# torognes/vsearch

Measured on AMD Instinct MI355X. Metric: GCUPS (useful DP cells/s of the search16 global-alignment path: DP + traceback + CIGAR), higher is better.
Workload: dtype int16

## Files before the change

include/vsx.h:

```cpp
#ifndef VSX_H
#define VSX_H

#include <stddef.h>
#include <stdint.h>

#ifdef __cplusplus
extern "C" {
#endif

#define VSX_API_VERSION 1000
#define VSX_SCORE_SENTINEL 32767

#define VSX_OK         0
#define VSX_EINVAL    -1
#define VSX_ENODEVICE -2
#define VSX_ENOMEM    -3
#define VSX_EHIP      -4

typedef struct vsx_ctx vsx_ctx;
typedef struct vsx_seqset vsx_seqset;
typedef struct vsx_plan vsx_plan;

typedef struct vsx_scoring {
  int64_t match;
  int64_t mismatch;
  int64_t gap_open_query_left;
  int64_t gap_open_target_left;
  int64_t gap_open_query_interior;
  int64_t gap_open_target_interior;
  int64_t gap_open_query_right;
  int64_t gap_open_target_right;
  int64_t gap_ext_query_left;
  int64_t gap_ext_target_left;
  int64_t gap_ext_query_interior;
  int64_t gap_ext_target_interior;
  int64_t gap_ext_query_right;
  int64_t gap_ext_target_right;
  int32_t n_mismatch;
} vsx_scoring;

typedef struct vsx_results {
  uint64_t   n_pairs;
  int16_t  * score;
  uint16_t * aligned;
  uint16_t * matches;
  uint16_t * mismatches;
  uint16_t * gaps;
  uint64_t * cigar_off;
  char     * cigar_blob;
  uint64_t   cigar_bytes;
  uint8_t  * verdict;
} vsx_results;

#define VSX_VERDICT_UNDECIDED 0
#define VSX_VERDICT_ACCEPTED  1
#define VSX_VERDICT_WEAK      2
#define VSX_VERDICT_REJECTED  3
typedef struct vsx_filter {
  int32_t iddef;
  int32_t leftjust, rightjust;
  int32_t pad;
  double  id, weak_id, maxid, mid, query_cov, target_cov;
  int64_t maxsubs, maxgaps, mincols, maxdiffs;
} vsx_filter;
int vsx_plan_set_filter(vsx_plan * plan, const vsx_filter * f);

typedef struct vsx_timing {
  float    forward_ms;
  float    traceback_ms;
  float    total_ms;
  uint32_t forward_launches;
  uint32_t traceback_launches;
  uint64_t cells;
  uint64_t dir_bytes;
} vsx_timing;

typedef struct vsx_plan_info {
  uint64_t tasks;
  uint64_t tasks_tilted;
  uint64_t tasks_tracked;
  uint32_t rows_dominant;
  uint32_t chunks;
  uint64_t tasks_max3;
  uint64_t tasks_sparse;
  uint64_t waves;
  uint64_t tasks_pair;
} vsx_plan_info;

const char * vsx_version_string(void);
int vsx_device_count(void);
const char * vsx_last_error(void);

int vsx_create(vsx_ctx ** out, const vsx_scoring * scoring, int device);
void vsx_destroy(vsx_ctx * ctx);


int vsx_seqset_create(vsx_ctx * ctx, vsx_seqset ** out, uint64_t n,
                      const char * blob, uint64_t blob_bytes,
                      const uint64_t * offsets, const uint32_t * lengths);
int vsx_seqset_create_from_device(vsx_ctx * ctx, vsx_seqset ** out, uint64_t n,
                                  const void * d_blob, uint64_t blob_bytes,
                                  const uint64_t * offsets, const uint32_t * lengths);
int vsx_seqset_create_both_strands(vsx_ctx * ctx, vsx_seqset ** out, uint64_t n,
                                   const char * blob, uint64_t blob_bytes,
                                   const uint64_t * offsets, const uint32_t * lengths);
void vsx_seqset_destroy(vsx_seqset * s);
uint64_t vsx_seqset_count(const vsx_seqset * s);

int vsx_plan_create(vsx_ctx * ctx, vsx_plan ** out,
                    const vsx_seqset * queries, const vsx_seqset * targets,
                    uint64_t n_pairs, const uint32_t * qidx, const uint32_t * tidx,
                    uint64_t dir_budget_bytes);
int vsx_plan_run(vsx_plan * plan);
int vsx_plan_sync(vsx_plan * plan, vsx_timing * timing );
int vsx_plan_fetch(vsx_plan * plan, vsx_results * out);
int vsx_plan_describe(const vsx_plan * plan, vsx_plan_info * info);
#define VSX_HIT_RECORD_BYTES 24
int vsx_plan_export_hits(vsx_plan * plan, void * d_dst, uint64_t dst_bytes);
int vsx_plan_export_runs(vsx_plan * plan, void * d_dst, uint64_t dst_bytes, uint64_t * n_runs);
int64_t vsx_cigar_from_runs(const uint32_t * runs, uint32_t n, char * dst, uint64_t cap);
void vsx_plan_destroy(vsx_plan * plan);

int vsx_align_pairs_filtered(vsx_ctx * ctx, const vsx_seqset * queries, const vsx_seqset * targets,
                             uint64_t n_pairs, const uint32_t * qidx, const uint32_t * tidx,
                             const vsx_filter * filter, vsx_results * out);
int vsx_align_pairs(vsx_ctx * ctx, const vsx_seqset * queries, const vsx_seqset * targets,
                    uint64_t n_pairs, const uint32_t * qidx, const uint32_t * tidx,
                    vsx_results * out);
void vsx_results_free(vsx_results * r);

typedef struct vsx_ranked {
  uint64_t   n_pairs, n_hits;
  uint32_t * pair;
  int16_t  * score;
  uint16_t * aligned, * matches, * mismatches, * gaps;
  uint8_t  * verdict;
  double   * id;
  uint64_t * cigar_off;
  char     * cigar_blob;
  uint64_t   cigar_bytes;
  uint64_t   n_undecided;
  uint32_t * undecided;
} vsx_ranked;
int vsx_align_pairs_ranked(vsx_ctx * ctx, const vsx_seqset * queries, const vsx_seqset * targets,
                           uint64_t n_pairs, const uint32_t * qidx, const uint32_t * tidx,
                           const vsx_filter * filter, int keep_weak, vsx_ranked * out);
void vsx_ranked_free(vsx_ranked * r);

#ifdef __cplusplus
}
#endif
#endif
```

profiles/valu_budget.py:

```python
#!/usr/bin/env python3
import argparse
import collections
import os
import re
import shutil
import subprocess
import sys
import tempfile

LLVM = "/opt/rocm/llvm/bin"
ROOT = os.path.dirname(os.path.dirname(os.path.abspath(__file__)))


def mangled(args):
    a = [x.strip() for x in args.split(",")]
    enc = "".join(("Li%sE" % x) if x.lstrip("-").isdigit() else ("Lb%dE" % (x == "true")) for x in a)
    return "_Z18vsx_forward_kernelI" + enc + "Ev12VsxDevParamsPK7VsxTaskPKhS5_PjP15HIP_vector_typeIjLj2EEP10VsxSlotOutj"


def extract(lib, sym, tmp):
    shutil.copy(lib, os.path.join(tmp, "lib.so"))
    subprocess.run([LLVM + "/llvm-objdump", "--offloading", "lib.so"], cwd=tmp, capture_output=True, check=True)
    for f in sorted(os.listdir(tmp)):
        if "gfx950" not in f:
            continue
        p = os.path.join(tmp, f)
        syms = subprocess.run([LLVM + "/llvm-readelf", "-s", "--wide", p], capture_output=True, text=True).stdout
        if (" " + sym + "\n") in syms:
            return p, syms
    sys.exit("kernel %s not found in %s" % (sym, lib))


def meta(syms, sym):
    out = {}
    for k in ("num_vgpr", "numbered_sgpr", "private_seg_size"):
        m = re.search(r"\s([0-9a-f]+)\s+0\s+NOTYPE\s+LOCAL\s+DEFAULT\s+ABS\s+" + re.escape(sym) + r"\." + k + r"\n", syms)
        out[k] = int(m.group(1), 16) if m else None
    m = re.search(r"\s([0-9a-f]+)\s+(\d+)\s+FUNC\s+\S+\s+\S+\s+\S+\s+" + re.escape(sym) + r"\n", syms)
    out["start"], out["size"] = int(m.group(1), 16), int(m.group(2))
    return out


def disasm(co, sym, start):
    txt = subprocess.run([LLVM + "/llvm-objdump", "-d", "--mcpu=gfx950", "--disassemble-symbols=" + sym, co],
                         capture_output=True, text=True, check=True).stdout
    ins = []
    for line in txt.splitlines():
        m = re.match(r"\s+(\S+)\s*(.*?)\s*//\s*([0-9A-F]+):", line)
        if not m:
            continue
        op, rest, addr = m.group(1), m.group(2), int(m.group(3), 16) - start
        t = re.search(r"<" + re.escape(sym) + r"\+0x([0-9a-f]+)>", line)
        ins.append((addr, op, rest, int(t.group(1), 16) if t else None))
    return ins


def is_valu(op):
    return op.startswith("v_")


def category(op, rest):
    if op in ("v_pk_maximum3_f16", "v_pk_max_u16", "v_subrev_u32_e32", "v_sub_u32_e32", "v_subrev_u32_e64", "v_sub_u32_e64"):
        return "row body"
    if op == "v_mov_b32_dpp":
        return "DPP hand-overs (feed, H, F)"
    if op == "v_add_u32_sdwa":
        return "profile row addresses"
    if op in ("v_pk_ashrrev_i16", "v_bfi_b32"):
        return "leave-column tracking"
    if op in ("v_lshl_add_u32", "v_lshlrev_b32_e32", "v_or_b32_e32", "v_and_or_b32") and "s" in rest.split(",")[1]:
        return "feed-slot addresses"
    if op in ("v_lshl_add_u64", "v_add_co_u32_e32", "v_addc_co_u32_e32", "v_mad_u64_u32"):
        return "checkpoint addresses"
    if op == "v_mov_b32_e32":
        return "register copies"
    return None


def budget(body, R, S):
    c = collections.Counter()
    quota = {"v_perm_b32": R * S, "v_add_u32_e32": R * S}
    npk = sum(1 for op, _ in body if op == "v_pk_sub_i16")
    nashr = sum(1 for op, _ in body if op == "v_pk_ashrrev_i16")
    pk = [("row body", S), ("last row's own e / hf subtractions", 2 * S), ("leave-column tracking", nashr)]
    for op, rest in body:
        if not is_valu(op):
            continue
        k = category(op, rest)
        if k is None and op in quota:
            if op == "v_add_u32_e32" and re.search(r"0x(1|2)000(1|2)\b", rest):
                k = "leave-column tracking"
            elif quota[op] > 0:
                quota[op] -= 1
                k = "row body"
            else:
                k = "checkpoint pack" if op == "v_perm_b32" else "other"
        if k is None and op == "v_pk_sub_i16":
            for i, (name, n) in enumerate(pk):
                if n > 0:
                    pk[i] = (name, n - 1)
                    k = name
                    break
            else:
                k = "checkpoint pack"
        c[k or "other"] += 1
    return c, npk


def main():
    ap = argparse.ArgumentParser()
    ap.add_argument("--lib", default=os.path.join(ROOT, "vsearch_amd", "libvsx.so"))
    ap.add_argument("--kernel", default="16,false,true,true,1,false,true", help="template arguments of vsx_forward_kernel")
    ap.add_argument("--rows", type=int, default=None, help="R (default: the first template argument)")
    ap.add_argument("--loop", type=int, default=None, help="loop index to budget (default: most v_pk_maximum3_f16)")
    ap.add_argument("--ops", action="store_true", help="print the opcode histogram of the loop too")
    a = ap.parse_args()
    R = a.rows or int(a.kernel.split(",")[0])
    sym = mangled(a.kernel)
    tmp = tempfile.mkdtemp(prefix="vsx_budget_")
    try:
        co, syms = extract(a.lib, sym, tmp)
        md = meta(syms, sym)
        ins = disasm(co, sym, md["start"])
    finally:
        shutil.rmtree(tmp, ignore_errors=True)
    print("vsx_forward_kernel<%s>  (%s)" % (a.kernel, os.path.relpath(a.lib, ROOT) if a.lib.startswith(ROOT) else a.lib))
    print("  code %d B, %d instructions, %d VALU;  VGPR %s  SGPR %s  scratch %s B" % (
        md["size"], len(ins), sum(is_valu(op) for _, op, _, _ in ins), md["num_vgpr"], md["numbered_sgpr"], md["private_seg_size"]))
    idx = {addr: k for k, (addr, _, _, _) in enumerate(ins)}
    heads = collections.OrderedDict()
    for k, (addr, op, _, tgt) in enumerate(ins):
        if op.startswith("s_branch") or op.startswith("s_cbranch"):
            if tgt is not None and tgt <= addr and tgt in idx:
                h = idx[tgt]
                heads.setdefault(h, []).append(k)
    loops = []
    for h, bs in heads.items():
        first_back, last = min(bs), max(bs)
        main_path = set(range(h, first_back + 1))
        for k in range(h, first_back + 1):
            addr, op, _, tgt = ins[k]
            if op.startswith("s_cbranch") and tgt is not None and tgt > addr and tgt in idx and idx[tgt] <= first_back + 1:
                for j in range(k + 1, idx[tgt]):
                    main_path.discard(j)
        cond = [j for j in range(h, last + 1) if j not in main_path]
        mp = sorted(main_path)
        loops.append(dict(head=h, end=last, main=mp, cond=cond,
                          max3=sum(1 for j in mp if ins[j][1] == "v_pk_maximum3_f16"),
                          valu_main=sum(1 for j in mp if is_valu(ins[j][1])), valu_cond=sum(1 for j in cond if is_valu(ins[j][1]))))
    print("  loops (offset range: VALU on the always-taken path + in branch-guarded regions, v_pk_maximum3_f16):")
    for n, L in enumerate(loops):
        print("    [%d] +0x%04x..+0x%04x: %4d + %4d VALU, %3d max3" % (n, ins[L["head"]][0], ins[L["end"]][0], L["valu_main"], L["valu_cond"], L["max3"]))
    if not loops:
        return
    n = a.loop if a.loop is not None else max(range(len(loops)), key=lambda i: (loops[i]["max3"], -i))
    L = loops[n]
    S = max(1, round(L["max3"] / R))
    body = [(ins[j][1], ins[j][2]) for j in L["main"]]
    cond = [(ins[j][1], ins[j][2]) for j in L["cond"]]
    cm, _ = budget(body, R, S)
    per_step = L["valu_main"] / S + L["valu_cond"] / 16.0
    print("  loop [%d]: %d steps per iteration (R = %d)" % (n, S, R))
    print("    VALU per two steps, always-taken path: %.1f" % (2.0 * L["valu_main"] / S))
    print("    VALU in branch-guarded regions (once per 16 steps): %d" % L["valu_cond"])
    print("    VALU per 16-step block: %.0f   per step: %.2f   (row body %d per step = %.1f %%)" % (
        16 * per_step, per_step, 6 * R, 100.0 * 6 * R / per_step))
    print("    per step, by category (always-taken path / S, + branch-guarded / 16):")
    order = ["row body", "DPP hand-overs (feed, H, F)", "profile row addresses", "feed-slot addresses", "last row's own e / hf subtractions",
             "leave-column tracking", "checkpoint pack", "checkpoint addresses", "register copies", "other"]
    for k in order:
        v = cm.get(k, 0) / S
        if v:
            print("      %-38s %6.2f" % (k, v))
    if L["valu_cond"]:
        print("      %-38s %6.2f  (%d VALU / 16)" % ("16-step block boundary (guarded)", L["valu_cond"] / 16.0, L["valu_cond"]))
    if a.ops:
        for name, lst in (("always-taken path", body), ("branch-guarded", cond)):
            h = collections.Counter(op for op, _ in lst if is_valu(op))
            print("    %s opcodes: %s" % (name, ", ".join("%s %d" % kv for kv in h.most_common())))


if __name__ == "__main__":
    main()
```

vsearch_amd/_lib.py:

```python
import ctypes as C
import os

HERE = os.path.dirname(os.path.abspath(__file__))
LIB_PATH = os.environ.get("VSX_LIBRARY") or os.path.join(HERE, "libvsx.so")

VSX_OK, VSX_EINVAL, VSX_ENODEVICE, VSX_ENOMEM, VSX_EHIP = 0, -1, -2, -3, -4
SENTINEL = 32767

SYMBOLS = [
    "vsx_version_string", "vsx_device_count", "vsx_last_error", "vsx_create", "vsx_destroy",
    "vsx_seqset_create", "vsx_seqset_create_both_strands", "vsx_seqset_create_from_device", "vsx_seqset_destroy", "vsx_seqset_count",
    "vsx_plan_create", "vsx_plan_run", "vsx_plan_sync", "vsx_plan_fetch", "vsx_plan_export_hits", "vsx_plan_export_runs",
    "vsx_cigar_from_runs", "vsx_plan_destroy",
    "vsx_align_pairs", "vsx_align_pairs_filtered", "vsx_align_pairs_ranked", "vsx_ranked_free", "vsx_plan_set_filter", "vsx_results_free", "vsx_plan_describe",
]
SEARCH_SYMBOLS = ["vsx_search_opts_default", "vsx_searcher_create", "vsx_searcher_destroy", "vsx_searcher_db_text", "vsx_search_batch",
                  "vsx_search_batch_meta", "vsx_searcher_set_meta",
                  "vsx_hits_free", "vsx_search_candidates", "vsx_search_candidates_batch", "vsx_candidates_free", "vsx_lma_align", "vsx_allpairs_block", "vsx_allpairs_rows", "vsx_allpairs_stream", "vsx_cluster_fast", "vsx_cluster_out_free", "vsx_msa", "vsx_msa_out_free",
                  "vsx_msa_device", "vsx_msa_device_batch", "vsx_dust_mask", "vsx_abundance_ratio_cmp",
                  "vsx_multi_searcher_create", "vsx_multi_searcher_destroy", "vsx_multi_searcher_devices", "vsx_multi_searcher_replica",
                  "vsx_multi_search_batch", "vsx_multi_allpairs",
                  "vsx_chimera_opts_default", "vsx_uchime_ref", "vsx_chimera_last_stats",
                  "vsx_chimera_denovo_opts_default", "vsx_uchime_denovo", "vsx_chimera_denovo_last_stats"]


class Candidates(C.Structure):
    _fields_ = [("n_queries", C.c_uint64), ("start", C.POINTER(C.c_uint64)), ("target", C.POINTER(C.c_uint32)),
                ("count", C.POINTER(C.c_uint32)), ("seconds", C.c_double), ("kernel_ms", C.c_double),
                ("index_build_ms", C.c_double), ("index_postings", C.c_uint64), ("postings_streamed", C.c_uint64),
                ("bytes_streamed", C.c_uint64)]


class SearchOpts(C.Structure):
    _fields_ = [("id", C.c_double), ("weak_id", C.c_double), ("maxaccepts", C.c_int64), ("maxrejects", C.c_int64),
                ("wordlength", C.c_int64), ("minwordmatches", C.c_int64), ("iddef", C.c_int32), ("soft_mask", C.c_int32),
                ("maxsubs", C.c_int64), ("maxgaps", C.c_int64), ("mincols", C.c_int64), ("maxdiffs", C.c_int64),
                ("query_cov", C.c_double), ("target_cov", C.c_double), ("maxid", C.c_double), ("mid", C.c_double),
                ("leftjust", C.c_int32), ("rightjust", C.c_int32),
                ("minqt", C.c_double), ("maxqt", C.c_double), ("minsl", C.c_double), ("maxsl", C.c_double),
                ("idprefix", C.c_int64), ("idsuffix", C.c_int64), ("selfid", C.c_int32), ("threads", C.c_int32),
                ("window", C.c_int64), ("gap_infinite", C.c_uint32), ("strand_both", C.c_uint32),
                ("maxqsize", C.c_int64), ("mintsize", C.c_int64), ("minsizeratio", C.c_double), ("maxsizeratio", C.c_double),
                ("self", C.c_int32), ("sizeorder", C.c_int32), ("cluster_unoise", C.c_int32), ("qmask", C.c_int32),
                ("unoise_alpha", C.c_double), ("hardmask", C.c_int32)]


class ChimeraOpts(C.Structure):
    _fields_ = [("search", SearchOpts), ("minh", C.c_double), ("mindiv", C.c_double), ("mindiffs", C.c_int64),
                ("xn", C.c_double), ("dn", C.c_double), ("window", C.c_int64)]


class ChimeraResult(C.Structure):
    _fields_ = [("score", C.c_double), ("parent_a", C.c_uint32), ("parent_b", C.c_uint32), ("closest", C.c_uint32),
                ("status", C.c_int32), ("id_query_model", C.c_double), ("id_query_a", C.c_double), ("id_query_b", C.c_double),
                ("id_a_b", C.c_double), ("id_query_top", C.c_double), ("left_yes", C.c_int32), ("left_no", C.c_int32),
                ("left_abstain", C.c_int32), ("right_yes", C.c_int32), ("right_no", C.c_int32), ("right_abstain", C.c_int32),
                ("divergence", C.c_double), ("flag", C.c_char), ("pad", C.c_char * 7)]


class ChimeraStats(C.Structure):
    _fields_ = [("seconds_search", C.c_double), ("seconds_align", C.c_double), ("seconds_eval", C.c_double),
                ("seconds_total", C.c_double), ("windows", C.c_uint64), ("parts", C.c_uint64), ("pairs_aligned", C.c_uint64),
                ("sentinel_pairs", C.c_uint64), ("queries_kernel", C.c_uint64), ("queries_host", C.c_uint64)]


class ChimeraDenovoOpts(C.Structure):
    _fields_ = [("base", ChimeraOpts), ("variant", C.c_int32), ("abskew", C.c_double)]


class ChimeraDenovoStats(C.Structure):
    _fields_ = [("seconds_rank", C.c_double), ("seconds_members", C.c_double), ("seconds_search", C.c_double),
                ("seconds_align", C.c_double), ("seconds_eval", C.c_double), ("seconds_reconcile", C.c_double),
                ("seconds_total", C.c_double), ("windows", C.c_uint64), ("passes", C.c_uint64), ("passes_max", C.c_uint64),
                ("queries_reevaluated", C.c_uint64), ("parts", C.c_uint64), ("pairs_searched", C.c_uint64),
                ("pairs_aligned", C.c_uint64), ("sentinel_pairs", C.c_uint64), ("queries_kernel", C.c_uint64),
                ("queries_host", C.c_uint64)]


class SeqMeta(C.Structure):
    _fields_ = [("abundance", C.POINTER(C.c_uint64)), ("label", C.POINTER(C.c_char_p))]


class Hit(C.Structure):
    _fields_ = [("query", C.c_uint32), ("target", C.c_uint32), ("count", C.c_uint32),
                ("accepted", C.c_uint8), ("weak", C.c_uint8), ("used_fallback", C.c_uint8), ("strand", C.c_uint8),
                ("nwscore", C.c_int32), ("nwdiff", C.c_int32), ("nwgaps", C.c_int32), ("nwindels", C.c_int32),
                ("nwalignmentlength", C.c_int32), ("matches", C.c_int32), ("mismatches", C.c_int32),
                ("internal_alignmentlength", C.c_int32), ("internal_gaps", C.c_int32), ("internal_indels", C.c_int32),
                ("trim_q_left", C.c_int32), ("trim_q_right", C.c_int32), ("trim_t_left", C.c_int32), ("trim_t_right", C.c_int32),
                ("shortest", C.c_int32), ("longest", C.c_int32),
                ("nwid", C.c_double), ("id", C.c_double), ("id0", C.c_double), ("id1", C.c_double), ("id2", C.c_double),
                ("id3", C.c_double), ("id4", C.c_double), ("cigar_off", C.c_uint64)]


class Hits(C.Structure):
    _fields_ = [("n_queries", C.c_uint64), ("n_hits", C.c_uint64), ("first", C.POINTER(C.c_uint64)),
                ("hit", C.POINTER(Hit)), ("cigar_blob", C.POINTER(C.c_char)), ("cigar_bytes", C.c_uint64),
                ("pairs_aligned", C.c_uint64), ("cells_aligned", C.c_uint64), ("stages", C.c_uint64),
                ("sentinel_pairs", C.c_uint64), ("seconds_kmer", C.c_double), ("seconds_align", C.c_double),
                ("seconds_total", C.c_double)]


class Scoring(C.Structure):
    _fields_ = [(n, C.c_int64) for n in (
        "match", "mismatch", "gap_open_query_left", "gap_open_target_left", "gap_open_query_interior",
        "gap_open_target_interior", "gap_open_query_right", "gap_open_target_right",
        "gap_ext_query_left", "gap_ext_target_left", "gap_ext_query_interior", "gap_ext_target_interior",
        "gap_ext_query_right", "gap_ext_target_right")] + [("n_mismatch", C.c_int32)]


class Results(C.Structure):
    _fields_ = [("n_pairs", C.c_uint64), ("score", C.POINTER(C.c_int16)), ("aligned", C.POINTER(C.c_uint16)),
                ("matches", C.POINTER(C.c_uint16)), ("mismatches", C.POINTER(C.c_uint16)),
                ("gaps", C.POINTER(C.c_uint16)), ("cigar_off", C.POINTER(C.c_uint64)),
                ("cigar_blob", C.POINTER(C.c_char)), ("cigar_bytes", C.c_uint64), ("verdict", C.POINTER(C.c_uint8))]


class Ranked(C.Structure):
    _fields_ = [("n_pairs", C.c_uint64), ("n_hits", C.c_uint64), ("pair", C.POINTER(C.c_uint32)), ("score", C.POINTER(C.c_int16)),
                ("aligned", C.POINTER(C.c_uint16)), ("matches", C.POINTER(C.c_uint16)), ("mismatches", C.POINTER(C.c_uint16)),
                ("gaps", C.POINTER(C.c_uint16)), ("verdict", C.POINTER(C.c_uint8)), ("id", C.POINTER(C.c_double)),
                ("cigar_off", C.POINTER(C.c_uint64)), ("cigar_blob", C.POINTER(C.c_char)), ("cigar_bytes", C.c_uint64),
                ("n_undecided", C.c_uint64), ("undecided", C.POINTER(C.c_uint32))]


class Filter(C.Structure):
    _fields_ = [("iddef", C.c_int32), ("leftjust", C.c_int32), ("rightjust", C.c_int32), ("pad", C.c_int32),
                ("id", C.c_double), ("weak_id", C.c_double), ("maxid", C.c_double), ("mid", C.c_double),
                ("query_cov", C.c_double), ("target_cov", C.c_double),
                ("maxsubs", C.c_int64), ("maxgaps", C.c_int64), ("mincols", C.c_int64), ("maxdiffs", C.c_int64)]


class PlanInfo(C.Structure):
    _fields_ = [("tasks", C.c_uint64), ("tasks_tilted", C.c_uint64), ("tasks_tracked", C.c_uint64),
                ("rows_dominant", C.c_uint32), ("chunks", C.c_uint32), ("tasks_max3", C.c_uint64),
                ("tasks_sparse", C.c_uint64), ("waves", C.c_uint64), ("tasks_pair", C.c_uint64)]


class Timing(C.Structure):
    _fields_ = [("forward_ms", C.c_float), ("traceback_ms", C.c_float), ("total_ms", C.c_float),
                ("forward_launches", C.c_uint32), ("traceback_launches", C.c_uint32),
                ("cells", C.c_uint64), ("dir_bytes", C.c_uint64)]


class ClusterOut(C.Structure):
    _fields_ = [("n", C.c_uint64), ("n_clusters", C.c_uint64), ("clusterno", C.POINTER(C.c_uint32)), ("hits", Hits)]


class MsaOut(C.Structure):
    _fields_ = [("alnlen", C.c_uint64), ("n_rows", C.c_uint64), ("conslen", C.c_uint64), ("rows", C.POINTER(C.c_char)),
                ("consensus", C.POINTER(C.c_char)), ("profile", C.POINTER(C.c_uint64))]


_lib = None


def load():
    global _lib
    if _lib is not None:
        return _lib
    if not os.path.exists(LIB_PATH):
        raise ImportError(
            f"{LIB_PATH} not found: build the HIP extension first (python -c 'import __graft_entry__ as g; "
            "g.build()' or make -C vsearch_amd/csrc). vsearch_amd has no CPU fallback.")
    lib = C.CDLL(LIB_PATH)
    vp = C.c_void_p
    lib.vsx_version_string.restype = C.c_char_p
    lib.vsx_last_error.restype = C.c_char_p
    lib.vsx_device_count.restype = C.c_int
    lib.vsx_create.argtypes = [C.POINTER(vp), C.POINTER(Scoring), C.c_int]
    lib.vsx_destroy.argtypes = [vp]
    lib.vsx_destroy.restype = None
    lib.vsx_seqset_create.argtypes = [vp, C.POINTER(vp), C.c_uint64, vp, C.c_uint64, vp, vp]
    lib.vsx_seqset_create_both_strands.argtypes = [vp, C.POINTER(vp), C.c_uint64, vp, C.c_uint64, vp, vp]
    lib.vsx_seqset_create_from_device.argtypes = [vp, C.POINTER(vp), C.c_uint64, vp, C.c_uint64, vp, vp]
    lib.vsx_seqset_destroy.argtypes = [vp]
    lib.vsx_seqset_destroy.restype = None
    lib.vsx_seqset_count.argtypes = [vp]
    lib.vsx_seqset_count.restype = C.c_uint64
    lib.vsx_plan_create.argtypes = [vp, C.POINTER(vp), vp, vp, C.c_uint64, vp, vp, C.c_uint64]
    lib.vsx_plan_run.argtypes = [vp]
    lib.vsx_plan_sync.argtypes = [vp, C.POINTER(Timing)]
    lib.vsx_plan_fetch.argtypes = [vp, C.POINTER(Results)]
    lib.vsx_plan_export_hits.argtypes = [vp, vp, C.c_uint64]
    lib.vsx_plan_export_runs.argtypes = [vp, vp, C.c_uint64, C.POINTER(C.c_uint64)]
    lib.vsx_cigar_from_runs.argtypes = [vp, C.c_uint32, vp, C.c_uint64]
    lib.vsx_cigar_from_runs.restype = C.c_int64
    lib.vsx_plan_destroy.argtypes = [vp]
    lib.vsx_plan_destroy.restype = None
    lib.vsx_plan_describe.argtypes = [vp, C.POINTER(PlanInfo)]
    lib.vsx_align_pairs.argtypes = [vp, vp, vp, C.c_uint64, vp, vp, C.POINTER(Results)]
    lib.vsx_align_pairs_filtered.argtypes = [vp, vp, vp, C.c_uint64, vp, vp, C.POINTER(Filter), C.POINTER(Results)]
    lib.vsx_align_pairs_ranked.argtypes = [vp, vp, vp, C.c_uint64, vp, vp, C.POINTER(Filter), C.c_int, C.POINTER(Ranked)]
    lib.vsx_ranked_free.argtypes = [C.POINTER(Ranked)]
    lib.vsx_ranked_free.restype = None
    lib.vsx_plan_set_filter.argtypes = [vp, C.POINTER(Filter)]
    lib.vsx_results_free.argtypes = [C.POINTER(Results)]
    lib.vsx_results_free.restype = None
    lib.vsx_search_opts_default.argtypes = [C.POINTER(SearchOpts)]
    lib.vsx_search_opts_default.restype = None
    lib.vsx_searcher_create.argtypes = [vp, C.POINTER(vp), C.POINTER(SearchOpts), C.c_uint64, vp, C.c_uint64, vp, vp]
    lib.vsx_searcher_destroy.argtypes = [vp]
    lib.vsx_searcher_destroy.restype = None
    lib.vsx_search_batch.argtypes = [vp, C.c_uint64, vp, C.c_uint64, vp, vp, C.POINTER(Hits)]
    lib.vsx_search_batch_meta.argtypes = [vp, C.c_uint64, vp, C.c_uint64, vp, vp, C.POINTER(SeqMeta), C.POINTER(Hits)]
    lib.vsx_searcher_set_meta.argtypes = [vp, C.POINTER(SeqMeta)]
    lib.vsx_hits_free.argtypes = [C.POINTER(Hits)]
    lib.vsx_hits_free.restype = None
    lib.vsx_search_candidates.argtypes = [vp, C.c_char_p, C.c_uint32, vp, vp, C.c_uint64]
    lib.vsx_search_candidates.restype = C.c_int64
    lib.vsx_search_candidates_batch.argtypes = [vp, C.c_int32, C.c_uint64, vp, C.c_uint64, vp, vp, C.POINTER(Candidates)]
    lib.vsx_candidates_free.argtypes = [C.POINTER(Candidates)]
    lib.vsx_candidates_free.restype = None
    lib.vsx_allpairs_block.argtypes = [vp, C.c_int32, C.c_uint64, C.c_uint64, C.POINTER(Hits)]
    lib.vsx_allpairs_rows.argtypes = [vp, C.c_int32, vp, C.c_uint64, C.POINTER(Hits)]
    lib.vsx_allpairs_stream.argtypes = [vp, C.c_int32, C.c_uint64, C.c_uint64, C.c_uint64, vp, vp]
    lib.vsx_dust_mask.argtypes = [vp, C.c_uint64, vp, vp, C.c_int32]
    lib.vsx_multi_searcher_create.argtypes = [C.POINTER(vp), vp, vp, C.c_int32, vp, C.c_uint64, vp, C.c_uint64, vp, vp, vp]
    lib.vsx_multi_searcher_destroy.argtypes = [vp]
    lib.vsx_multi_searcher_destroy.restype = None
    lib.vsx_multi_searcher_devices.argtypes = [vp]
    lib.vsx_multi_searcher_devices.restype = C.c_int32
    lib.vsx_multi_searcher_replica.argtypes = [vp, C.c_int32]
    lib.vsx_multi_searcher_replica.restype = vp
    lib.vsx_multi_search_batch.argtypes = [vp, C.c_uint64, vp, C.c_uint64, vp, vp, vp, C.POINTER(Hits)]
    lib.vsx_multi_allpairs.argtypes = [vp, C.c_int32, C.c_uint64, C.c_uint64, C.POINTER(Hits)]
    lib.vsx_abundance_ratio_cmp.argtypes = [C.c_int64, C.c_double, C.c_int64]
    lib.vsx_abundance_ratio_cmp.restype = C.c_int
    lib.vsx_cluster_fast.argtypes = [vp, C.c_uint64, C.POINTER(ClusterOut)]
    lib.vsx_cluster_out_free.argtypes = [C.POINTER(ClusterOut)]
    lib.vsx_cluster_out_free.restype = None
    lib.vsx_msa.argtypes = [C.c_uint32, vp, vp, vp, vp, C.POINTER(MsaOut)]
    lib.vsx_msa_device.argtypes = [vp, C.c_uint32, vp, vp, vp, vp, C.POINTER(MsaOut)]
    lib.vsx_msa_device_batch.argtypes = [vp, C.c_uint32, vp, vp, vp, vp, vp, C.POINTER(MsaOut)]
    lib.vsx_msa_out_free.argtypes = [C.POINTER(MsaOut)]
    lib.vsx_msa_out_free.restype = None
    lib.vsx_lma_align.argtypes = [C.POINTER(Scoring), C.c_char_p, C.c_uint64, C.c_char_p, C.c_uint64] + \
        [C.POINTER(C.c_int64)] * 5 + [C.POINTER(vp)]
    _lib = lib
    return lib


class VsxError(RuntimeError):
    def __init__(self, code, where):
        msg = load().vsx_last_error().decode(errors="replace")
        super().__init__(f"{where}: error {code}: {msg}")
        self.code = code


def check(code, where):
    if code != VSX_OK:
        raise VsxError(code, where)
```

vsearch_amd/csrc/ubench_d16.hip:

```cpp
#include <hip/hip_runtime.h>
#include <cstdio>
#include <cstdlib>

#define CK(x) do { hipError_t e = (x); if (e != hipSuccess) { fprintf(stderr, "%s:%d %s\n", __FILE__, __LINE__, hipGetErrorString(e)); exit(1); } } while (0)

__global__ void k_semantics(unsigned * out)
{
  __shared__ unsigned short tab[256];
  tab[threadIdx.x] = (unsigned short) (0x1100u + threadIdx.x);
  tab[threadIdx.x + 64] = (unsigned short) (0x2200u + threadIdx.x);
  __syncthreads();
  const unsigned addr = (unsigned) (size_t) tab + threadIdx.x * 2u;
  unsigned hi = 0xDEADBEEFu, lo = 0xDEADBEEFu, u16 = 0xDEADBEEFu;
  asm volatile("ds_read_u16_d16_hi %0, %3 offset:128\n"
               "ds_read_u16_d16 %1, %3\n"
               "ds_read_u16 %2, %3\n"
               "s_waitcnt lgkmcnt(0)\n" : "+v"(hi), "+v"(lo), "+v"(u16) : "v"(addr));
  out[threadIdx.x * 3 + 0] = hi;
  out[threadIdx.x * 3 + 1] = lo;
  out[threadIdx.x * 3 + 2] = u16;
}

typedef _Float16 f16x2 __attribute__((ext_vector_type(2)));
typedef unsigned short us2 __attribute__((ext_vector_type(2)));
__device__ __forceinline__ unsigned max3(unsigned a, unsigned b, unsigned c)
{
  const f16x2 x = __builtin_bit_cast(f16x2, a), y = __builtin_bit_cast(f16x2, b), z = __builtin_bit_cast(f16x2, c);
  return __builtin_bit_cast(unsigned, __builtin_elementwise_maximum(__builtin_elementwise_maximum(x, y), z));
}
__device__ __forceinline__ unsigned pmaxu(unsigned a, unsigned b)
{
  return __builtin_bit_cast(unsigned, __builtin_elementwise_max(__builtin_bit_cast(us2, a), __builtin_bit_cast(us2, b)));
}

#define R 16
template <int MODE>
__global__ void __launch_bounds__(64) __attribute__((amdgpu_waves_per_eu(MODE == 2 ? 2 : 4, 8))) k_rows(int steps, unsigned * out, unsigned seed)
{
  __shared__ __attribute__((aligned(16))) short QP[(MODE == 2 ? 2 : 1) * 16 * 16 * R];
  for (int i = threadIdx.x; i < (MODE == 2 ? 2 : 1) * 16 * 16 * R; i += 64) QP[i] = (short) ((i * 7 + (int) seed) & 0xff);
  __syncthreads();
  const int l = threadIdx.x & 15;
  unsigned H[R], H2[R], E[R];
  for (int r = 0; r < R; ++r) { H[r] = 0x3E003E00u + (unsigned) (r * 3 + (int) threadIdx.x); H2[r] = H[r]; E[r] = 0x3E003E00u - (unsigned) (r + (int) seed); }
  unsigned F = 0x3E003E00u, diag = 0x3E003E00u, sym = threadIdx.x * 2654435761u + seed;
  const unsigned go = 0x00120012u;
  auto step = [&](unsigned (&hin)[R], unsigned (&hout)[R]) __attribute__((always_inline)) {
    sym = sym * 1664525u + 1013904223u;
    const unsigned ca = (sym >> 8) & 15u, cb = (sym >> 20) & 15u;
    unsigned Hd = diag;
    if (MODE == 0)
      {
        const short * qa = QP + ca * (16 * R) + l * R;
        const short * qb = QP + cb * (16 * R) + l * R;
        unsigned pa = 0, pb = 0, pa2 = 0, pb2 = 0;
#pragma unroll
        for (int r = 0; r < R; ++r)
          {
            if ((r & 3) == 0)
              {
                const uint2 va = *reinterpret_cast<const uint2 *>(qa + r), vb = *reinterpret_cast<const uint2 *>(qb + r);
                pa = va.x; pb = vb.x; pa2 = va.y; pb2 = vb.y;
              }
            else if ((r & 3) == 2) { pa = pa2; pb = pb2; }
            const unsigned V = (r & 1) ? __builtin_amdgcn_perm(pb, pa, 0x07060302u) : __builtin_amdgcn_perm(pb, pa, 0x05040100u);
            const unsigned h0 = Hd + V;
            const unsigned h2 = max3(h0, F, E[r]);
            Hd = hin[r];
            hout[r] = h2;
            const unsigned he = h2 - go;
            F = pmaxu(F, he);
            E[r] = pmaxu(E[r], he);
          }
      }
    else if (MODE == 2)
      {
        const uint4 * q4 = reinterpret_cast<const uint4 *>(QP) + (((ca & 3u) * 4u + (cb & 3u)) * 16u + (unsigned) l) * (R / 4);
        uint4 v4 = make_uint4(0, 0, 0, 0);
#pragma unroll
        for (int r = 0; r < R; ++r)
          {
            if ((r & 3) == 0) v4 = q4[r >> 2];
            const unsigned V = (r & 3) == 0 ? v4.x : ((r & 3) == 1 ? v4.y : ((r & 3) == 2 ? v4.z : v4.w));
            const unsigned h0 = Hd + V;
            const unsigned h2 = max3(h0, F, E[r]);
            Hd = hin[r];
            hout[r] = h2;
            const unsigned he = h2 - go;
            F = pmaxu(F, he);
            E[r] = pmaxu(E[r], he);
          }
      }
    else
      {
        const unsigned aA = (unsigned) (size_t) QP + (ca * (16 * R) + (unsigned) l * R) * 2u;
        const unsigned aB = (unsigned) (size_t) QP + (cb * (16 * R) + (unsigned) l * R) * 2u;
        unsigned lo[R], hi[R];
#define LOAD2(k) asm volatile("ds_read_u16 %0, %4 offset:%6\n ds_read_u16_d16_hi %1, %5 offset:%6\n ds_read_u16 %2, %4 offset:%7\n ds_read_u16_d16_hi %3, %5 offset:%7\n" \
                              : "=&v"(lo[2 * (k)]), "=&v"(hi[2 * (k)]), "=&v"(lo[2 * (k) + 1]), "=&v"(hi[2 * (k) + 1]) : "v"(aA), "v"(aB), "n"(4 * (k)), "n"(4 * (k) + 2))
#define WAIT2(k, n) asm volatile("s_waitcnt lgkmcnt(" #n ")" : "+v"(lo[2 * (k)]), "+v"(hi[2 * (k)]), "+v"(lo[2 * (k) + 1]), "+v"(hi[2 * (k) + 1]))
        LOAD2(0); LOAD2(1);
#pragma unroll
        for (int k = 0; k < R / 2; ++k)
          {
            if (k + 1 < R / 2) { WAIT2(k, 4); } else { WAIT2(k, 0); }
#pragma unroll
            for (int rr = 0; rr < 2; ++rr)
              {
                const int r = 2 * k + rr;
                const unsigned h0 = Hd + lo[r] + hi[r];
                const unsigned h2 = max3(h0, F, E[r]);
                Hd = hin[r];
                hout[r] = h2;
                const unsigned he = h2 - go;
                F = pmaxu(F, he);
                E[r] = pmaxu(E[r], he);
              }
            if (k + 2 < R / 2)
              {
                switch (k + 2) { case 2: LOAD2(2); break; case 3: LOAD2(3); break; case 4: LOAD2(4); break; case 5: LOAD2(5); break; case 6: LOAD2(6); break; case 7: LOAD2(7); break; }
              }
          }
      }
    diag = hout[R - 1] ^ sym;
  };
  for (int t = 0; t < steps; t += 2) { step(H, H2); step(H2, H); }
  unsigned acc = F;
  for (int r = 0; r < R; ++r) acc ^= H[r] ^ E[r];
  out[blockIdx.x * 64 + threadIdx.x] = acc;
}

template <int MODE> static void run(int waves_per_simd)
{
  const int blocks = 1024 * waves_per_simd, steps = 2000;
  unsigned * out; CK(hipMalloc(&out, (size_t) blocks * 64 * 4));
  hipEvent_t e0, e1; CK(hipEventCreate(&e0)); CK(hipEventCreate(&e1));
  hipLaunchKernelGGL(k_rows<MODE>, dim3(blocks), dim3(64), 0, 0, 20, out, 1u);
  CK(hipDeviceSynchronize());
  CK(hipEventRecord(e0));
  hipLaunchKernelGGL(k_rows<MODE>, dim3(blocks), dim3(64), 0, 0, steps, out, 1u);
  CK(hipEventRecord(e1));
  CK(hipEventSynchronize(e1));
  float ms; CK(hipEventElapsedTime(&ms, e0, e1));
  unsigned h0 = 0;
  CK(hipMemcpy(&h0, out, 4, hipMemcpyDeviceToHost));
  const double cycles = ms * 1e-3 * 2.4e9;
  printf("mode %d (%s) waves/SIMD %d: %8.3f ms, %.1f cycles per lane-row and wave   [check %08x]\n", MODE,
         MODE == 0 ? "b64 loads + perm, 6 VALU per row" : (MODE == 1 ? "u16 loads, add3, 5 VALU per row" : "pair profile, b128 loads, 5 VALU per row"), waves_per_simd, ms,
         cycles / ((double) steps * R * waves_per_simd), h0);
  CK(hipFree(out));
}

int main()
{
  hipDeviceProp_t p; CK(hipGetDeviceProperties(&p, 0));
  printf("device %s  CUs %d  arch %s\n", p.name, p.multiProcessorCount, p.gcnArchName);
  unsigned * out; CK(hipMalloc(&out, 64 * 3 * 4));
  hipLaunchKernelGGL(k_semantics, dim3(1), dim3(64), 0, 0, out);
  unsigned h[12]; CK(hipMemcpy(h, out, sizeof h, hipMemcpyDeviceToHost));
  printf("lane 0: d16_hi into 0xDEADBEEF -> %08x, d16 -> %08x, u16 -> %08x;  lane 1: %08x %08x %08x\n", h[0], h[1], h[2], h[3], h[4], h[5]);
  printf("  (table: lane x holds 0x1100 + x at its address, 0x2200 + x at +128)  d16_hi zeroes the low half: %s\n", (h[0] & 0xffffu) == 0 ? "YES" : "no");
  for (int w = 1; w <= 4; w *= 2) { run<0>(w); run<1>(w); if (w <= 2) run<2>(w); }
  run<0>(3);
  return 0;
}
```

vsearch_amd/csrc/vsx_device.hip:

```cpp
#include <hip/hip_runtime.h>
#include <type_traits>
#include <cstdlib>
#include <atomic>
#include "vsx_internal.h"

typedef unsigned int u32;
typedef unsigned int u32x4 __attribute__((ext_vector_type(4)));
typedef unsigned int u32x3 __attribute__((ext_vector_type(3)));
typedef short s2 __attribute__((ext_vector_type(2)));
typedef unsigned short us2 __attribute__((ext_vector_type(2)));

#define DEV __device__ __forceinline__
struct __attribute__((aligned(4))) Pair2 { unsigned int x, y; };

#define SIGN2 0x80008000u

DEV s2 S2(u32 x) { return __builtin_bit_cast(s2, x); }
DEV us2 U2(u32 x) { return __builtin_bit_cast(us2, x); }
DEV u32 UI(s2 x) { return __builtin_bit_cast(u32, x); }
DEV u32 UI(us2 x) { return __builtin_bit_cast(u32, x); }

DEV u32 sadd(u32 a, u32 b) { return UI(__builtin_elementwise_add_sat(S2(a), S2(b))); }
DEV u32 ssub(u32 a, u32 b) { return UI(__builtin_elementwise_sub_sat(S2(a), S2(b))); }
DEV u32 pmax(u32 a, u32 b) { return UI(__builtin_elementwise_max(S2(a), S2(b))); }
DEV u32 pmin(u32 a, u32 b) { return UI(__builtin_elementwise_min(S2(a), S2(b))); }
DEV u32 pminu(u32 a, u32 b) { return UI(__builtin_elementwise_min(U2(a), U2(b))); }
DEV u32 pmaxu(u32 a, u32 b) { return UI(__builtin_elementwise_max(U2(a), U2(b))); }
DEV u32 psubw(u32 a, u32 b) { return UI((us2) (U2(a) - U2(b))); }
DEV u32 pmad(u32 a, u32 b, u32 c) { return UI((us2) (U2(a) * U2(b) + U2(c))); }
DEV u32 pashr15(u32 a) { return UI((s2) (S2(a) >> (s2){15, 15})); }
DEV u32 bfi(u32 mask, u32 a, u32 b) { return (a & mask) | (b & ~mask); }
DEV u32 a_bfi(u32 mask, u32 a, u32 b) { u32 r; asm("v_bfi_b32 %0, %1, %2, %3" : "=v"(r) : "s"(mask), "v"(a), "v"(b)); return r; }
DEV u32 a_bfi_v(u32 mask, u32 a, u32 b) { u32 r; asm("v_bfi_b32 %0, %1, %2, %3" : "=v"(r) : "v"(mask), "v"(a), "v"(b)); return r; }
DEV u32 a_bfi_vs(u32 mask, u32 a, u32 b) { u32 r; asm("v_bfi_b32 %0, %1, %2, %3" : "=v"(r) : "v"(mask), "v"(a), "s"(b)); return r; }
DEV u32 a_lshr1(u32 a) { u32 r; asm("v_lshrrev_b32 %0, 1, %1" : "=v"(r) : "v"(a)); return r; }
DEV u32 a_pk_ashr15(u32 a) { u32 r; asm("v_pk_ashrrev_i16 %0, 15, %1 op_sel_hi:[0,1]" : "=v"(r) : "v"(a)); return r; }
DEV u32 funnel(u32 acc, u32 d) { return a_bfi(SIGN2, d, a_lshr1(acc)); }
DEV u32 pack16(int v) { const u32 x = (u32) v & 0xffffu; return x | (x << 16); }

DEV u32 dpp_shr1(u32 feed, u32 src) { return (u32) __builtin_amdgcn_update_dpp((int) feed, (int) src, 0x111, 0xF, 0xF, false); }
DEV u32 dpp_rol1(u32 src) { return (u32) __builtin_amdgcn_update_dpp((int) src, (int) src, 0x12F, 0xF, 0xF, false); }


#define VSX_COLCK_G 64
#define VSX_COLCK_DW(R_, lane_, block_) ((((size_t) ((lane_) / VSX_COLCK_G) * (size_t) ((2 * (R_)) / 4) + (size_t) (block_)) * VSX_COLCK_G + (size_t) ((lane_) % VSX_COLCK_G)) * 4)
#define VSX_RB 1
#define VSX_ROWCK_PAIR_DW(TILT_) ((TILT_) ? 192 : 256)
#define VSX_COLCK_NBH(RT_) (((RT_) + ((RT_) + 1) / 2 + 3) / 4)
#define VSX_COLCK_NB(R_, TILT_) ((TILT_) ? (VSX_MID(R_, true) ? 2 * VSX_COLCK_NBH((R_) / 2) : ((R_) + ((R_) + 1) / 2 + 3) / 4) : (2 * (R_)) / 4)
#define VSX_CK_SLOT(TILT_, g_, l_) ((TILT_) ? ((l_) * 4 + (g_)) : ((g_) * 16 + (l_)))
#ifndef VSX_COLCK_CG
#define VSX_COLCK_CG 64
#endif
#define VSX_COLCK_CDW(NB_, lane_, block_) ((((size_t) ((lane_) / VSX_COLCK_CG) * (size_t) (NB_) + (size_t) (block_)) * VSX_COLCK_CG + (size_t) ((lane_) % VSX_COLCK_CG)) * 4)
#ifndef VSX_FWD_WAVES
#define VSX_FWD_WAVES(R_, TILT_) ((R_) <= 16 ? 4 : ((R_) <= 24 ? 3 : 2))
#endif
#ifndef VSX_FWD_WAVES_ONE
#define VSX_FWD_WAVES_ONE(R_, TILT_) ((R_) == 26 ? 3 : VSX_FWD_WAVES(R_, TILT_))
#endif
typedef _Float16 f16x2 __attribute__((ext_vector_type(2)));
DEV u32 pk_max3_bits(u32 a, u32 b, u32 c)
{
  const f16x2 x = __builtin_bit_cast(f16x2, a), y = __builtin_bit_cast(f16x2, b), z = __builtin_bit_cast(f16x2, c);
  return __builtin_bit_cast(u32, __builtin_elementwise_maximum(__builtin_elementwise_maximum(x, y), z));
}
#ifndef VSX_FWD_WAVES_NQ
#define VSX_FWD_WAVES_NQ(R_, NQ_) ((NQ_) == 4 ? 2 : ((R_) <= 24 ? 3 : 2))
#endif
template <int R, bool TRACK, bool TILT = false, bool MAX3 = false, int NQ = 1, bool PAIR = false, bool ONE = false>
__global__ void __launch_bounds__(PAIR ? 256 : 64) __attribute__((amdgpu_waves_per_eu(NQ == 1 ? (ONE ? VSX_FWD_WAVES_ONE(R, TILT) : VSX_FWD_WAVES(R, TILT)) : VSX_FWD_WAVES_NQ(R, NQ), 8)))
vsx_forward_kernel(const VsxDevParams P, const VsxTask * __restrict__ tasks,
                   const uint8_t * __restrict__ qc, const uint8_t * __restrict__ tc,
                   u32 * __restrict__ dir, uint2 * strip, VsxSlotOut * __restrict__ slot_out, const u32 ntasks)
{
  constexpr bool TOPPAD = !TRACK;
  static_assert(!TILT || TOPPAD, "tilted coordinates exist for the TOPPAD class only");
  const int tl = TILT ? P.tilt : 0;
  static_assert(!MAX3 || TILT, "the MAX3 arithmetic is a sub-class of TILT");
  constexpr u32 BIAS16 = MAX3 ? 0x3E00u : (TILT ? 0x8000u : 0u);
  constexpr u32 BIAS = BIAS16 * 0x10001u;
  constexpr u32 CK_REBIAS = 0u;
  auto bpack = [](int v) -> u32 { return pack16(v + (int) BIAS16); };
  auto vadd = [](u32 a, u32 b) -> u32 { return TILT ? a + b : sadd(a, b); };
  auto vsubk = [](u32 a, u32 b) -> u32 { return TILT ? a - b : ssub(a, b); };
  auto vsub = [](u32 a, u32 b) -> u32 { return TILT ? psubw(a, b) : ssub(a, b); };
  auto vmax = [](u32 a, u32 b) -> u32 { return TILT ? pmaxu(a, b) : pmax(a, b); };
  constexpr bool MIDCK = VSX_MID(R, TILT);
  constexpr int RT = MIDCK ? R / 2 : R;
  constexpr bool QPL = TILT;
  constexpr int RP = (R + 3) & ~3;
  static_assert(NQ == 1 || NQ == 2 || NQ == 4, "tasks per wave");
  static_assert(NQ == 1 || TILT, "the sparse-task classes exist for the look-ahead TILT kernels only");
  static_assert(!PAIR || (NQ == 1 && TILT), "the pair-profile classes extend the FEED2 look-ahead kernels");
  constexpr int WPB = PAIR ? 4 : 1;
  constexpr int QPBYTES = 16 * 16 * RP;
  constexpr int RPP = ((RP / 4) & 1) ? RP : RP + 4;
  __shared__ __attribute__((aligned(16))) u32 PPf[PAIR ? 16 * 16 * RPP : 4];
  __shared__ __attribute__((aligned(16))) int16_t QP[!PAIR ? (QPL ? (NQ * QPBYTES) / 2 : 16 * 16 * R) : 8];
  constexpr int FSZ = (TILT ? 2 : 1) * 4 * 16;
  __shared__ uint4 FEED4a[FSZ * WPB];
  __shared__ u32 FEEDFa[FSZ * WPB];
  constexpr bool FEED2 = TILT;
  __shared__ uint2 FEEDBa[FEED2 ? 2 * 4 * 16 * WPB : 1];

  const int wv = PAIR ? __builtin_amdgcn_readfirstlane((int) (threadIdx.x >> 6)) : 0;
  uint4 * const FEED4 = FEED4a + wv * FSZ;
  u32 * const FEEDF = FEEDFa + wv * FSZ;
  uint2 * const FEEDB = FEEDBa + (FEED2 ? wv * FSZ : 0);
  const int lane = PAIR ? (int) (threadIdx.x & 63) : (int) threadIdx.x;
  const int gw = lane >> 4;
  constexpr int GPT = 4 / NQ;
  const int sq = (NQ == 1) ? 0 : gw / GPT;
  const int g = (NQ == 1) ? gw : gw % GPT;
  const int l = lane & 15;
  const u32 tix = PAIR ? blockIdx.x * 4u + (u32) wv : ((NQ == 1) ? blockIdx.x : blockIdx.x * (u32) NQ + (u32) sq);
  const bool sub_on = (NQ == 1 && !PAIR) ? true : (tix < ntasks);
  const VsxTask & T = tasks[sub_on ? tix : ntasks - 1];
  uint8_t * const QPl = reinterpret_cast<uint8_t *>(QP) + ((NQ == 1) ? 0 : sq * QPBYTES);

  const int Q = (int) T.qlen;
  const int total_lanes = (Q + R - 1) / R;
  const int rcnt0 = Q - (total_lanes - 1) * R;
  const int rc0 = __builtin_amdgcn_readfirstlane(rcnt0);
  static_assert(!PAIR || ONE, "the pair-profile classes are planned for single-strip queries only");
  const int nstrips = (NQ == 1 && !ONE) ? (total_lanes + 15) >> 4 : 1;
  const int steps = (NQ == 1) ? (int) T.steps : __builtin_amdgcn_readfirstlane((int) T.steps);

  const int DA = sub_on ? (int) T.tlen[2 * g] : 0;
  const int DB = sub_on ? (int) T.tlen[2 * g + 1] : 0;
  const int DpA = (DA + 3) & ~3;
  const int DpB = (DB + 3) & ~3;
  const int Dpg = DpA > DpB ? DpA : DpB;
  const uint8_t * __restrict__ tA = tc + T.toff[2 * g];
  const uint8_t * __restrict__ tB = tc + T.toff[2 * g + 1];
  const uint8_t * __restrict__ qq = qc + T.qoff;

  const u32 qrt_i_pk = pack16(P.qrt_i);
  u32 hmin = 0, hmax = 0;
  u32 score = 0;
  u32 lv1 = 0xFFFFFFFFu, leave = 0;

  for (int s = 0; s < nstrips; ++s)
    {
      const int L = 16 * s + l;
      const bool lane_on = (L < total_lanes) && (Dpg > 0);
      const bool first = (L == 0);
      const int pad = TOPPAD ? R - rcnt0 : 0;
      const int i0 = first ? -pad : rcnt0 + (L - 1) * R;

        {
          __syncthreads();
          if (PAIR)
            {
              for (int idx = (int) threadIdx.x; idx < 16 * 16 * RP; idx += 256)
                {
                  const int pr = idx / (16 * RP), row = idx % (16 * RP);
                  const int Lr = 16 * s + row / RP, rr = row % RP;
                  int va = 0, vb = 0;
                  if (rr < R)
                    {
                      if (Lr == 0 && rr < pad) va = vb = -P.top_step + 2 * tl;
                      else if (Lr < total_lanes)
                        {
                          const int gi = (Lr == 0) ? rr - pad : rcnt0 + (Lr - 1) * R + rr;
                          const int qs = (int) qq[gi];
                          va = P.matrix[(1 << (pr >> 2)) * 16 + qs];
                          vb = P.matrix[(1 << (pr & 3)) * 16 + qs];
                        }
                    }
                  PPf[(pr * 16 + row / RP) * RPP + rr] = ((u32) va & 0xffu) | (((u32) vb & 0xffu) << 16);
                }
            }
          else if (QPL)
            {
              constexpr int LPT = 64 / NQ;
              for (int idx = (NQ == 1) ? lane : lane % LPT; idx < 16 * 16 * RP; idx += LPT)
                {
                  const int code = idx / (16 * RP), row = idx % (16 * RP);
                  const int Lr = 16 * s + row / RP, rr = row % RP;
                  int v = 0;
                  if (rr < R)
                    {
                      if (Lr == 0 && rr < pad) v = -P.top_step + 2 * tl;
                      else if (Lr < total_lanes)
                        {
                          const int gi = (Lr == 0) ? rr - pad : rcnt0 + (Lr - 1) * R + rr;
                          v = P.matrix[code * 16 + (int) qq[gi]];
                        }
                    }
                  QPl[idx] = (uint8_t) v;
                }
            }
          else
          for (int idx = lane; idx < 16 * 16 * R; idx += 64)
            {
              const int code = idx / (16 * R), row = idx % (16 * R);
              const int Lr = 16 * s + row / R, rr = row % R;
              int v = 0;
              if (TOPPAD && Lr == 0 && rr < pad) v = -P.top_step + 2 * tl;
              else if (Lr < total_lanes && (TOPPAD || !(Lr == 0 && rr >= rcnt0)))
                {
                  const int gi = (Lr == 0) ? rr - pad : rcnt0 + (Lr - 1) * R + rr;
                  v = P.matrix[code * 16 + (int) qq[gi]];
                }
              QP[idx] = (int16_t) v;
            }
          __syncthreads();
        }

      u32 hprev[R];
      u32 hnext[R];
      u32 E[R];
      u32 ac[R];
#pragma unroll
      for (int r = 0; r < R; ++r)
        {
          int i = i0 + r;
          const bool dummy = TOPPAD && first && r < pad;
          if (i > Q - 1) i = Q - 1;
          if (i < 0) i = 0;
          u32 hl = bpack(P.hleft[i]);
          u32 e0 = vsub(hl, (i < Q - 1) ? P.qrq_i_pk : P.qrq_r_pk);
          if (dummy)
            {
              const int sh = (r - pad - 1) * tl;
              hl = bpack(((r == pad - 1) ? 0 : -P.top_open) + sh);
              e0 = vsub(bpack(-P.top_open - P.top_step + sh), P.qrq_i_pk);
            }
          hprev[r] = hl;
          hnext[r] = hl;
          E[r] = e0;
        }
      u32 diag = first ? bpack(((TOPPAD && pad > 0) ? -P.top_open : 0) - (pad + 2) * tl) : bpack(P.hleft[i0 - 1]);
      const bool lastpos = (L == total_lanes - 1);
      const u32 qrq_last = lastpos ? P.qrq_r_pk : P.qrq_i_pk;
      const u32 rq_last = lastpos ? P.rq_r_pk : P.rq_i_pk;

      u32 sym = 0, qrt = 0, rt = 0;
      u32 symf = 0;
      u32 outH = 0, outF = 0;
      u32 f_sym = 0, f_qrt = 0, f_rt = 0, f_H = 0, f_F = 0;
      u32 rawA = 0, rawB = 0;
      int rawH = 0;
      uint2 rawS = make_uint2(0, 0);
      const uint2 * strip_in = strip + T.strip_off + (size_t) (((s + 1) & 1) * 4 + g) * (size_t) steps;
      uint2 * strip_outp = strip + T.strip_off + (size_t) ((s & 1) * 4 + g) * (size_t) steps;

      auto prefetch = [&](int blk) {
        const int c = 16 * blk + l;
        rawA = (c < DA) ? (u32) tA[c] : 0u;
        rawB = (c < DB) ? (u32) tB[c] : 0u;
        if (s == 0) rawH = P.htop[c];
        else if (c < Dpg) rawS = strip_in[c];
      };
      prefetch(0);

      auto build_feed = [&](int blk, auto lean_tag) __attribute__((always_inline)) {
              constexpr bool LEAN = FEED2 && decltype(lean_tag)::value;
              const int c = 16 * blk + l;
              if (LEAN)
                {
                  f_H = (s == 0) ? bpack(rawH - pad * tl) : rawS.x;
                  f_F = (s == 0) ? vsub(f_H, qrt_i_pk) : rawS.y;
                  const u32 f_off = PAIR ? (((rawA >> 1) - (rawA >> 3)) * 4u + ((rawB >> 1) - (rawB >> 3))) * (u32) (16 * RPP * 4)
                                         : (rawA * (u32) (16 * RP) | ((rawB * (u32) (16 * RP)) << 16));
                  FEED4[(blk & 1) * 64 + gw * 16 + l] = make_uint4(f_off, 0u, f_H, f_F);
                  prefetch(blk + 1);
                  return;
                }
              const u32 qA = (u32) ((c < DA - 1) ? P.qrt_i : P.qrt_r) & 0xffffu;
              const u32 qB = (u32) ((c < DB - 1) ? P.qrt_i : P.qrt_r) & 0xffffu;
              const u32 rA = (u32) ((c < DA - 1) ? P.rt_i : P.rt_r) & 0xffffu;
              const u32 rB = (u32) ((c < DB - 1) ? P.rt_i : P.rt_r) & 0xffffu;
              const u32 sA = rawA | ((c == DA - 1) ? 0x100u : 0u) | ((c < DpA) ? 0x200u : 0u);
              const u32 sB = rawB | ((c == DB - 1) ? 0x100u : 0u) | ((c < DpB) ? 0x200u : 0u);
              f_sym = sA | (sB << 16);
              f_qrt = qA | (qB << 16);
              f_rt = rA | (rB << 16);
              if (s == 0)
                {
                  f_H = bpack(rawH - pad * tl);
                  f_F = vsub(f_H, f_qrt);
                }
              else
                {
                  f_H = rawS.x;
                  f_F = rawS.y;
                }
              const int fo = QPL ? (blk & 1) * 64 : 0;
              if (FEED2)
                {
                  const u32 f_off = PAIR ? (((rawA >> 1) - (rawA >> 3)) * 4u + ((rawB >> 1) - (rawB >> 3))) * (u32) (16 * RPP * 4)
                                         : (rawA * (u32) (16 * RP) | ((rawB * (u32) (16 * RP)) << 16));
                  FEED4[fo + gw * 16 + l] = make_uint4(f_off, f_sym, f_H, f_F);
                  FEEDB[fo + gw * 16 + l] = make_uint2(f_qrt, f_rt);
                }
              else
                {
                  FEED4[fo + gw * 16 + l] = make_uint4(f_sym, f_qrt, f_rt, f_H);
                  FEEDF[fo + gw * 16 + l] = f_F;
                }
              prefetch(blk + 1);
      };
      constexpr int PD = RP / 4;
      u32 profA[2][(QPL && !PAIR) ? PD : 1], profB[2][(QPL && !PAIR) ? PD : 1];
      auto load_profile = [&](u32 (&buf)[2][(QPL && !PAIR) ? PD : 1], u32 sy) __attribute__((always_inline)) {
        if (PAIR) return;
        const u32 cd = sy & 0x000F000Fu;
        constexpr int QPA = (RP % 16 == 0) ? 16 : ((RP % 8 == 0) ? 8 : 4);
        if (FEED2)
          {
            const uint8_t * pa = QPl + l * RP + (sy & 0xFFFFu);
            const uint8_t * pb = QPl + l * RP + (sy >> 16);
            constexpr int PDN = (QPL && !PAIR) ? PD : 1;
            if constexpr (PAIR) { }
            else if constexpr (QPA == 16)
              {
#pragma unroll
                for (int k = 0; k < PDN; k += 4)
                  {
                    const uint4 va = *reinterpret_cast<const uint4 *>(pa + 4 * k), vb = *reinterpret_cast<const uint4 *>(pb + 4 * k);
                    buf[0][k] = va.x; buf[0][k + 1] = va.y; buf[0][k + 2] = va.z; buf[0][k + 3] = va.w;
                    buf[1][k] = vb.x; buf[1][k + 1] = vb.y; buf[1][k + 2] = vb.z; buf[1][k + 3] = vb.w;
                  }
              }
            else if constexpr (QPA == 8)
              {
#pragma unroll
                for (int k = 0; k < PDN; k += 2)
                  {
                    const uint2 va = *reinterpret_cast<const uint2 *>(pa + 4 * k), vb = *reinterpret_cast<const uint2 *>(pb + 4 * k);
                    buf[0][k] = va.x; buf[0][k + 1] = va.y;
                    buf[1][k] = vb.x; buf[1][k + 1] = vb.y;
                  }
              }
            else
              {
#pragma unroll
                for (int k = 0; k < PDN; ++k)
                  { buf[0][k] = reinterpret_cast<const u32 *>(pa)[k]; buf[1][k] = reinterpret_cast<const u32 *>(pb)[k]; }
              }
            return;
          }
        const u32 * a = reinterpret_cast<const u32 *>(QPl + (cd & 0xFu) * (16 * RP) + l * RP);
        const u32 * b = reinterpret_cast<const u32 *>(QPl + (cd >> 16) * (16 * RP) + l * RP);
#pragma unroll
        for (int k = 0; k < ((QPL && !PAIR) ? PD : 1); ++k) { buf[0][k] = a[k]; buf[1][k] = b[k]; }
      };
      if (QPL)
        {
          build_feed(0, std::false_type {});
          sym = dpp_shr1(FEED4[gw * 16].x, 0u);
          load_profile(profA, sym);
        }

      const uint4 * const feed4_g = FEED4 + gw * 16;
      const u32 * const feedf_g = FEEDF + gw * 16;
      u32 pendH = 0, pendF = 0;
      u32 pendMH = 0, pendMF = 0, curMH = 0, curMF = 0;
      bool pend_on = false;
      const size_t ck_rowdw = ((((size_t) nstrips * steps + 1) & ~(size_t) 1) >> 1) * VSX_ROWCK_PAIR_DW(TILT);
      const size_t ck_nblk = ((size_t) steps + 15) >> 4;
      constexpr int CK_LANE_DW = TILT ? 3 : 4;
      constexpr size_t CK_COL_DW = TILT ? (size_t) 64 * 4 * VSX_COLCK_NB(R, true) : (size_t) 64 * (2 * R);
      const int ck_slot = VSX_CK_SLOT(TILT, gw, l);
      u32 * const rck_base = dir + T.dir_off + ((((size_t) s * steps) >> 1) * 64 + ck_slot) * CK_LANE_DW;
      u32 * const cck_base = dir + T.dir_off + ck_rowdw + (size_t) s * ck_nblk * CK_COL_DW;
      u32 * const mck_base = dir + T.dir_off + ck_rowdw + (size_t) nstrips * ck_nblk * CK_COL_DW
                             + ((((size_t) s * steps) >> 1) * 64 + ck_slot) * CK_LANE_DW;

      auto step = [&](const int t, u32 (&hin)[R], u32 (&hout)[R], u32 (&pc)[2][(QPL && !PAIR) ? PD : 1], u32 (&pn)[2][(QPL && !PAIR) ? PD : 1],
                      auto interior_tag, auto odd_tag, auto steady_tag) __attribute__((always_inline)) {
          constexpr bool INTERIOR = decltype(interior_tag)::value;
          constexpr bool ODD = decltype(odd_tag)::value;
          constexpr bool STEADY = decltype(steady_tag)::value != 0;
          constexpr bool LEANFEED = decltype(steady_tag)::value == 2;
          u32 symn = 0;
          u32 pp[PAIR ? RP : 1];
          if (PAIR)
            {
              const u32 * ppa = PPf + (sym >> 2) + l * RPP;
#pragma unroll
              for (int k = 0; k < (PAIR ? RP : 0); k += 4)
                {
                  const uint4 v = *reinterpret_cast<const uint4 *>(ppa + k);
                  pp[k] = v.x; pp[k + 1] = v.y; pp[k + 2] = v.z; pp[k + 3] = v.w;
                }
            }
          if (QPL) { if ((t & 15) == 15) build_feed((t >> 4) + 1, std::integral_constant<bool, LEANFEED> {}); }
          else if ((t & 15) == 0) build_feed(t >> 4, std::false_type {});

          const int fo = QPL ? ((t >> 4) & 1) * 64 : 0;
          const u32 fslot = (u32) (fo + (t & 15));
          const uint4 fv = feed4_g[fslot];
          const u32 fF = FEED2 ? fv.w : feedf_g[fslot];
          if (QPL)
            {
              const int t1 = t + 1;
              symn = dpp_shr1(feed4_g[(u32) (((t1 >> 4) & 1) * 64 + (t1 & 15))].x, sym);
              load_profile(pn, symn);
            }
          else sym = dpp_shr1(fv.x, sym);
          if (!INTERIOR)
            {
              if (FEED2)
                {
                  const uint2 fb = FEEDB[fo + gw * 16 + (t & 15)];
                  qrt = dpp_shr1(fb.x, qrt); rt = dpp_shr1(fb.y, rt);
                  symf = dpp_shr1(fv.y, symf);
                }
              else { qrt = dpp_shr1(fv.y, qrt); rt = dpp_shr1(fv.z, rt); }
            }
          const u32 inH = dpp_shr1(FEED2 ? fv.z : fv.w, outH);
          const u32 inF = dpp_shr1(fF, outF);

          const int j = t - l;
          const bool active = STEADY ? true : (lane_on && j >= 0 && j < Dpg);
          if (active)
            {
              const u32 code = sym & 0x000F000Fu;
              const int16_t * qpA = QP + (code & 0xFu) * (16 * R) + l * R;
              const int16_t * qpB = QP + (code >> 16) * (16 * R) + l * R;
              u32 pa = 0, pb = 0;
              u32 Hd = diag;
              u32 F = inF;
              u32 smn = 0x7FFF7FFFu, smx = 0x80008000u;
              u32 h2 = 0;
              u32 capH = 0, capF = 0, capmn = 0, capmx = 0;
              u32 lastL = 0, lastEL = 0;
              u32 midH = 0, midF = 0;
              auto rows = [&](auto shared_tag) __attribute__((always_inline)) {
              constexpr bool SHARED = decltype(shared_tag)::value;
              constexpr bool LASTFAST = MAX3 && SHARED;
#pragma unroll
              for (int r = 0; r < R; ++r)
                {
                  u32 V;
                  if (PAIR) V = pp[r];
                  else if (QPL)
                    {
                      if ((r & 3) == 0) { pa = pc[0][r >> 2]; pb = pc[1][r >> 2]; }
                      V = __builtin_amdgcn_perm(pb, pa, 0x0C040C00u + 0x00010001u * (u32) (r & 3));
                    }
                  else
                    {
                      if (R % 2 == 0)
                        {
                          if ((r & 3) == 0 && r + 3 < R)
                            {
                              typedef typename std::conditional<R % 4 == 0, uint2, Pair2>::type Rows4;
                              const Rows4 va = *reinterpret_cast<const Rows4 *>(qpA + r);
                              const Rows4 vb = *reinterpret_cast<const Rows4 *>(qpB + r);
                              pa = va.x; pb = vb.x;
                              ac[r + 1] = va.y; ac[r + 2] = vb.y;
                            }
                          else if ((r & 3) == 0)
                            {
                              pa = *reinterpret_cast<const u32 *>(qpA + r);
                              pb = *reinterpret_cast<const u32 *>(qpB + r);
                            }
                          else if ((r & 3) == 2) { pa = ac[r - 1]; pb = ac[r]; }
                          V = (r & 1) ? __builtin_amdgcn_perm(pb, pa, 0x07060302u) : __builtin_amdgcn_perm(pb, pa, 0x05040100u);
                        }
                      else V = (u32) (uint16_t) qpA[r] | ((u32) (uint16_t) qpB[r] << 16);
                    }
                  const u32 h0 = vadd(Hd, V);
                  const bool ONE_MAX = MAX3 && (r < R - 1 || LASTFAST);
                  const u32 h1 = ONE_MAX ? 0u : vmax(h0, F);
                  h2 = ONE_MAX ? pk_max3_bits(h0, F, E[r]) : vmax(h1, E[r]);
                  if (TRACK) { smn = pmin(smn, h2); smx = pmax(smx, h2); }
                  Hd = hin[r];
                  hout[r] = h2;
                  const u32 qrq = (r == R - 1) ? qrq_last : P.qrq_i_pk;
                  const u32 rq = (r == R - 1) ? rq_last : P.rq_i_pk;
                  const u32 he = (r < R - 1) ? vsubk(h2, qrq) : vsub(h2, qrq);
                  const u32 hf = (SHARED && r < R - 1) ? he : vsub(h2, qrt);
                  const u32 f = (TILT && INTERIOR) ? F : vsub(F, rt);
                  const u32 e = (TILT && INTERIOR && r < R - 1) ? E[r] : vsub(E[r], rq);
                  if (r == R - 1) { lastL = LASTFAST ? 0u : vsub(h1, E[r]); lastEL = vsub(he, e); }
                  F = vmax(f, hf);
                  E[r] = vmax(e, he);
                  if (MIDCK && r == RT - 1) { midH = h2; midF = F; }
                  if (!TOPPAD && __builtin_expect(rc0 == r + 1, 0)) { capH = h2; capF = F; capmn = smn; capmx = smx; }
                }
              };
              if (INTERIOR) rows(std::true_type {});
              else rows(std::false_type {});
              const u32 hl = (!TOPPAD && first) ? capH : h2;
              F = (!TOPPAD && first) ? capF : F;
              smn = (!TOPPAD && first) ? capmn : smn;
              smx = (!TOPPAD && first) ? capmx : smx;
              outH = hl;
              outF = F;
              diag = inH;
              {
                const u32 jpk = (u32) j | ((u32) j << 16);
                if (!INTERIOR)
                  {
                    const u32 atlast = a_pk_ashr15((FEED2 ? symf : sym) << 7);
                    leave = a_bfi_v(atlast, a_bfi_v(a_pk_ashr15(lastL), lv1, jpk), leave);
                  }
                const u32 lmask = a_pk_ashr15((MAX3 && INTERIOR) ? lastEL : (lastL | lastEL));
                lv1 = STEADY ? a_bfi_vs(lmask, lv1, (u32) t * 0x00010001u) : a_bfi_v(lmask, lv1, jpk);
              }

              if (TRACK)
                {
                  const u32 vm = a_pk_ashr15(sym << 6);
                  hmin = pmin(hmin, a_bfi_v(vm, smn, 0x7FFF7FFFu));
                  hmax = pmax(hmax, a_bfi_v(vm, smx, 0x80008000u));
                }
              if (!INTERIOR)
                {
                  const u32 lm = a_pk_ashr15((FEED2 ? symf : sym) << 7);
                  score = a_bfi_v(lm, hl, score);
                }

              if (!ODD) { pendH = outH; pendF = outF; }
              if (MIDCK) { if (!ODD) { pendMH = midH; pendMF = midF; } else { curMH = midH; curMF = midF; } }
              if (l == 15 && s + 1 < nstrips) strip_outp[j] = make_uint2(outH, outF);
            }
          if (!ODD) pend_on = active;
          else if (pend_on || active)
            {
              if (TILT)
                {
                  const size_t ckp = LEANFEED ? (size_t) ((t & ~15) >> 1) * 192 + (size_t) (((t & 15) >> 1) * 192) : (size_t) (t >> 1) * 192;
                  const u32 dpk = __builtin_amdgcn_perm(psubw(outH, outF), psubw(pendH, pendF), 0x06040200u);
                  __builtin_nontemporal_store((u32x3) {pendH + CK_REBIAS, outH + CK_REBIAS, dpk}, reinterpret_cast<u32x3 *>(rck_base + ckp));
                  if (MIDCK)
                    {
                      const u32 dpm = __builtin_amdgcn_perm(psubw(curMH, curMF), psubw(pendMH, pendMF), 0x06040200u);
                      __builtin_nontemporal_store((u32x3) {pendMH + CK_REBIAS, curMH + CK_REBIAS, dpm}, reinterpret_cast<u32x3 *>(mck_base + ckp));
                    }
                }
              else
                __builtin_nontemporal_store((u32x4) {pendH, pendF, outH, outF}, reinterpret_cast<u32x4 *>(rck_base + (size_t) (t >> 1) * 256));
            }
          if ((t & 15) == 15)
            {
              u32 * cb = cck_base + (size_t) (t >> 4) * CK_COL_DW;
              if (TILT)
                {
                  constexpr int NF = R + (R + 1) / 2;
                  constexpr int NFH = RT + (RT + 1) / 2, ZH = 4 * VSX_COLCK_NBH(RT);
                  auto flatc = [&](int z) -> u32 {
                    if (MIDCK)
                      {
                        const int hh = z / ZH, zz = z % ZH, r00 = hh * RT;
                        if (zz < RT) return hout[r00 + zz] + CK_REBIAS;
                        if (zz < NFH)
                          {
                            const int r0 = r00 + 2 * (zz - RT), r1 = (r0 + 1 < r00 + RT) ? r0 + 1 : r0;
                            return __builtin_amdgcn_perm(psubw(hout[r1], E[r1]), psubw(hout[r0], E[r0]), 0x06040200u);
                          }
                        return 0u;
                      }
                    if (z < R) return hout[z] + CK_REBIAS;
                    if (z < NF)
                      {
                        const int r0 = 2 * (z - R), r1 = r0 + 1 < R ? r0 + 1 : r0;
                        return __builtin_amdgcn_perm(psubw(hout[r1], E[r1]), psubw(hout[r0], E[r0]), 0x06040200u);
                      }
                    return 0u;
                  };
#pragma unroll
                  for (int z = 0; z < 4 * VSX_COLCK_NB(R, true); z += 4)
                    __builtin_nontemporal_store((u32x4) {flatc(z), flatc(z + 1), flatc(z + 2), flatc(z + 3)}, reinterpret_cast<u32x4 *>(cb + VSX_COLCK_CDW(VSX_COLCK_NB(R, true), ck_slot, z >> 2)));
                }
              else if (R % 2 == 0)
                {
                  auto flat = [&](int z) -> u32 { return z < R ? hout[z] : E[z - R]; };
#pragma unroll
                  for (int z = 0; z < 2 * R; z += 4)
                    __builtin_nontemporal_store((u32x4) {flat(z), flat(z + 1), flat(z + 2), flat(z + 3)}, reinterpret_cast<u32x4 *>(cb + VSX_COLCK_DW(R, lane, z >> 2)));
                }
              else
                {
                  u32 * cp = cb + lane * (2 * R);
#pragma unroll
                  for (int x = 0; x < R; ++x) { cp[x] = hout[x]; cp[R + x] = E[x]; }
                }
            }
          if (QPL) sym = symn;
      };
      int t_switch = 0;
      if (P.share_sub)
        {
          int dmin = 0x7fffffff;
          if (DA > 0 && DA < dmin) dmin = DA;
          if (DB > 0 && DB < dmin) dmin = DB;
#pragma unroll
          for (int m = 32; m >= 1; m >>= 1) { const int o = __shfl_xor(dmin, m, 64); dmin = o < dmin ? o : dmin; }
          t_switch = __builtin_amdgcn_readfirstlane(dmin == 0x7fffffff ? 0 : dmin - 1) & ~1;
          if (t_switch > steps) t_switch = steps & ~1;
        }
      int t = 0;
      qrt = qrt_i_pk; rt = pack16(P.rt_i);
      for (; t < t_switch && (TRACK || t < 16); t += 2)
        {
          step(t, hprev, hnext, profA, profB, std::true_type {}, std::false_type {}, std::false_type {});
          step(t + 1, hnext, hprev, profB, profA, std::true_type {}, std::true_type {}, std::false_type {});
        }
      if (!TRACK)
        {
          const u32 lpk = (u32) l * 0x00010001u;
          lv1 = psubw(lv1, psubw(0u, lpk));
          for (; t + 32 <= t_switch; t += 16)
            {
              const int tb = t & ~15;
#pragma unroll
              for (int k = 0; k < 16; k += 2)
                {
                  step(tb + k, hprev, hnext, profA, profB, std::true_type {}, std::false_type {}, std::integral_constant<int, 2> {});
                  step(tb + k + 1, hnext, hprev, profB, profA, std::true_type {}, std::true_type {}, std::integral_constant<int, 2> {});
                }
            }
          for (; t < t_switch; t += 2)
            {
              step(t, hprev, hnext, profA, profB, std::true_type {}, std::false_type {}, std::true_type {});
              step(t + 1, hnext, hprev, profB, profA, std::true_type {}, std::true_type {}, std::true_type {});
            }
          lv1 = psubw(lv1, lpk);
        }
      for (; t < steps; t += 2)
        {
          step(t, hprev, hnext, profA, profB, std::false_type {}, std::false_type {}, std::false_type {});
          step(t + 1, hnext, hprev, profB, profA, std::false_type {}, std::true_type {}, std::false_type {});
        }

      if (s + 1 < nstrips)
        {
          __builtin_amdgcn_fence(__ATOMIC_RELEASE, "agent");
          __builtin_amdgcn_fence(__ATOMIC_ACQUIRE, "agent");
        }
    }

#pragma unroll
  for (int m = 8; m >= 1; m >>= 1)
    {
      hmin = pmin(hmin, (u32) __shfl_xor((int) hmin, m, 16));
      hmax = pmax(hmax, (u32) __shfl_xor((int) hmax, m, 16));
    }
  const int l_last = (total_lanes - 1) & 15;
  score = (u32) __shfl((int) score, l_last, 16);
  leave = (u32) __shfl((int) leave, l_last, 16);
  if (l == 0)
    {
      const int mnA = (int16_t) (hmin & 0xffff), mnB = (int16_t) (hmin >> 16);
      const int mxA = (int16_t) (hmax & 0xffff), mxB = (int16_t) (hmax >> 16);
      VsxSlotOut oA, oB;
      score = psubw(score, BIAS);
      oA.score = (int16_t) ((int) (int16_t) (score & 0xffff) - (DA > 0 ? (Q + DA - 2) * tl : 0));
      oB.score = (int16_t) ((int) (int16_t) (score >> 16) - (DB > 0 ? (Q + DB - 2) * tl : 0));
      oA.leave = (uint16_t) (leave & 0xffff); oB.leave = (uint16_t) (leave >> 16); oA.pad = 0; oB.pad = 0;
      oA.overflow = (mnA <= P.smin || mxA >= 32767) ? 1 : 0;
      oB.overflow = (mnB <= P.smin || mxB >= 32767) ? 1 : 0;
      if (sub_on)
        {
          slot_out[(size_t) tix * VSX_TASK_SLOTS + 2 * g] = oA;
          slot_out[(size_t) tix * VSX_TASK_SLOTS + 2 * g + 1] = oB;
        }
    }
}

DEV u32 half_lo(u32 w, bool hi) { return hi ? (w >> 16) : w; }
DEV int wave_max_i32(int v)
{
#pragma unroll
  for (int m = 32; m >= 1; m >>= 1) { const int o = __shfl_xor(v, m, 64); v = o > v ? o : v; }
  return v;
}

DEV void rank_note(const VsxFilterDev & FL, u32 pid, u32 verdict, int score, double idv)
{
  if (FL.rank_counts == nullptr) return;
  if (verdict == 1u || verdict == 2u)
    {
      const u32 pos = atomicAdd(FL.rank_counts, 1u);
      FL.kept_pair[pos] = pid;
      FL.kept_id[pos] = idv;
    }
  else if (verdict == 0u && score == 32767)
    FL.refused_pair[atomicAdd(FL.rank_counts + 1, 1u)] = pid;
}

template <bool FAST> struct TbOps;
template <> struct TbOps<false>
{
  static DEV u32 in(u32 lo16) { return lo16; }
  static DEV u32 score(int16_t v) { return (u32) (uint16_t) v; }
  static DEV u32 add(u32 a, u32 b) { return sadd(a, b); }
  static DEV u32 sub(u32 a, u32 b) { return ssub(a, b); }
  static DEV u32 max(u32 a, u32 b) { return pmax(a, b); }
  static DEV u32 dif(u32 a, u32 b) { return ssub(a, b); }
  static DEV u32 neg(u32 d) { return (d >> 15) & 1u; }
  static DEV u32 fun(u32 acc, u32 d) { return funnel(acc, d); }
  static DEV u32 one_row_word(u32 acc) { return acc >> 12; }
  static DEV u32 nibble(u32 w, int rows_in_group, int y) { return (w >> (16 - 4 * rows_in_group + 4 * y)) & 15u; }
  static constexpr u32 UP = 1, LEFT = 2, EXT_UP = 4, EXT_LEFT = 8;
};
template <> struct TbOps<true>
{
  static DEV u32 in(u32 lo16) { return (lo16 & 0xffffu) ^ 0x8000u; }
  static DEV u32 score(int16_t v) { return (u32) (int) v; }
  static DEV u32 add(u32 a, u32 b) { return a + b; }
  static DEV u32 sub(u32 a, u32 b) { return a - b; }
  static DEV u32 max(u32 a, u32 b) { return (u32) __builtin_elementwise_max((unsigned short) a, (unsigned short) b); }
  static DEV u32 dif(u32 a, u32 b) { return a - b; }
  static DEV u32 neg(u32 d) { return d >> 31; }
  static DEV u32 fun(u32 acc, u32 d) { return __builtin_amdgcn_alignbit(acc, d, 31); }
  static DEV u32 one_row_word(u32 acc) { return acc << 12; }
  static DEV u32 nibble(u32 w, int rows_in_group, int y) { return (w >> (4 * (rows_in_group - 1 - y))) & 15u; }
  static constexpr u32 UP = 8, LEFT = 4, EXT_UP = 2, EXT_LEFT = 1;
};

typedef u32 u32_unaligned __attribute__((aligned(1)));
typedef unsigned long long u64_unaligned __attribute__((aligned(1)));
struct __attribute__((aligned(4))) Quad { u32 x, y, z, w; };
struct __attribute__((aligned(4))) Trio { u32 x, y, z; };

#include "vsx_accept.h"

#ifndef VSX_TB_STATS
#define VSX_TB_STATS 0
#endif
#if VSX_TB_STATS
__device__ unsigned long long vsx_tb_stats_dev[16];
extern "C" hipError_t vsx_internal_tb_stats(unsigned long long * out8, int reset)
{
  hipError_t e = hipMemcpyFromSymbol(out8, HIP_SYMBOL(vsx_tb_stats_dev), sizeof(unsigned long long) * 16);
  if (e == hipSuccess && reset) { unsigned long long z[16] = {0}; e = hipMemcpyToSymbol(HIP_SYMBOL(vsx_tb_stats_dev), z, sizeof z); }
  return e;
}
#endif

#ifndef VSX_TB_WAVES
#define VSX_TB_WAVES(R_, MID_) ((MID_) ? ((R_) <= 24 ? 4 : 3) : ((R_) <= 12 ? 4 : ((R_) <= 16 ? 3 : 2)))
#endif
template <int R, bool FAST, bool CK8 = false, bool MID = false>
__global__ void __launch_bounds__(128) __attribute__((amdgpu_waves_per_eu(VSX_TB_WAVES(R, MID), 8)))
vsx_traceback_ck_kernel(const VsxDevParams P, const VsxFilterDev FL, const VsxTask * __restrict__ tasks,
                        const u32 * __restrict__ pair_slot, const u32 * __restrict__ pair_ids, u32 npairs,
                        const uint8_t * __restrict__ qc, const uint8_t * __restrict__ tc,
                        const u32 * __restrict__ ck, const VsxSlotOut * __restrict__ slot,
                        u32 * __restrict__ slab, const uint64_t * __restrict__ slab_off,
                        u32 * __restrict__ runs, uint64_t runs_capacity, unsigned long long * cursor,
                        VsxPairOut * __restrict__ out)
{
  typedef TbOps<FAST> A;
  static_assert(VSX_RB == 1, "the tile staging below reads row checkpoints as two-step (16-byte) pairs");
  static_assert(!CK8 || FAST, "compressed checkpoints belong to the TILT class");
  static_assert(!MID || (CK8 && R % 2 == 0), "half-height tiles belong to the TILT class");
  constexpr int RT = MID ? R / 2 : R;
  constexpr int ND = (RT + 3) / 4;
  constexpr bool TOPPAD = FAST;
  typedef typename std::conditional<CK8, uint8_t, int16_t>::type SshT;
  __shared__ SshT Ssh[512];
  __shared__ uint16_t bitsL_all[2 * 16 * ND * 64];
  __shared__ u32 tbL_all[2 * 17 * 64];
  __shared__ uint8_t symL_all[2 * 8 * 64];
  const int tid = (int) (threadIdx.x & 63);
  const int wv = (int) (threadIdx.x >> 6);
  uint16_t * const bitsL = bitsL_all + wv * (16 * ND * 64);
  u32 * const tbL = tbL_all + wv * (17 * 64) - 64;
  uint8_t * const symL = symL_all + wv * (8 * 64);
  for (int x = (int) threadIdx.x; x < 512; x += 128)
    Ssh[x] = (SshT) (((x & 31) < 16) ? P.matrix[(x >> 5) * 16 + (x & 15)] : (int16_t) (-P.top_step + 2 * P.tilt));
  __syncthreads();
// ... 824 lines not shown
                      const u32 h1 = pmax(h0, F);
                      const u32 dL = ssub(h1, ee[x]);
                      const u32 h2 = pmax(h1, ee[x]);
                      Hd = hp[x];
                      hp[x] = FIRST ? bfi(0x0000FFFFu, h2, hp[x]) : h2;
                      const u32 hf = pk_sub(h2, qrt_pk);
                      const u32 f = INT ? F : pk_sub(F, rt_pk);
                      const u32 dEU = ssub(hf, f);
                      F = pmax(f, hf);
                      const bool plain = INT && x != XL;
                      const u32 he = plain ? hf : pk_sub(h2, x == XL ? qrq_pk_x : qrq_pk_i);
                      const u32 e = plain ? ee[x] : pk_sub(ee[x], x == XL ? rq_pk_x : rq_pk_i);
                      const u32 dEL = ssub(he, e);
                      const u32 en = pmax(e, he);
                      ee[x] = FIRST ? bfi(0x0000FFFFu, en, ee[x]) : en;
                      acc = a_bfi(mA[x & 3], __builtin_amdgcn_perm(dL, dU, 0x0B0A0908u), acc);
                      acc = a_bfi(mB[x & 3], __builtin_amdgcn_perm(dEL, dEU, 0x0B0A0908u), acc);
                    }
                bitsL[(it * NG + g4) * 64 + tid] = acc;
              }
          Hd_end = Hd;
          F_end = F;
          tb_prev = tbv;
          cr_prev = cr;
        };
        auto sweep = [&](auto int_tag, auto fast_tag) __attribute__((always_inline)) {
          column(0, int_tag, fast_tag, std::true_type {});
          for (int it = 1; it <= cmax + 1; ++it) column(it, int_tag, fast_tag, std::false_type {});
        };
        if (tile_int) { if (fastV) sweep(std::true_type {}, std::true_type {}); else sweep(std::true_type {}, std::false_type {}); }
        else          { if (fastV) sweep(std::false_type {}, std::true_type {}); else sweep(std::false_type {}, std::false_type {}); }
      };
      auto walk = [&](const int cst) __attribute__((always_inline)) {
        while (r >= r0h && j >= cst && i >= 0)
          {
            const int cw = j - cst;
            const int rv = r - r0h;
            const bool up_half = rv >= HR;
            const int rx = up_half ? rv - HR : rv;
            const u32 w = bitsL[((cw + (up_half ? 1 : 0)) * NG + (rx >> 2)) * 64 + tid] >> ((rx & 3) + (up_half ? 8 : 0));
            ++al;
            const u32 inI = (op == 1) ? 1u : 0u, inD = (op == 2) ? 1u : 0u;
            const u32 c1 = inI & (w >> 20);
            const u32 c2 = (c1 ^ 1u) & inD & (w >> 4);
            const u32 c12 = c1 | c2;
            const u32 c3 = (c12 ^ 1u) & (w >> 16);
            const u32 c4 = ((c12 | c3) ^ 1u) & w;
            const u32 isI = (c1 | c3) & 1u, isD = (c2 | c4) & 1u;
            const int newop = (int) (isI + 2u * isD);
            ga += ((c3 & (inI ^ 1u)) | (c4 & (inD ^ 1u))) & 1u;
            j -= (int) (isD ^ 1u);
            const int di = (int) (isI ^ 1u);
            i -= di; r -= di;
            if (newop != op)
              {
                if (op >= 0) my[nruns++] = (runlen << 2) | (u32) op;
                op = newop;
                runlen = 0;
              }
            ++runlen;
#if VSX_TB_STATS & 1
            atomicAdd(&vsx_tb_stats_dev[3], 1ull);
#endif
          }
      };

#if VSX_TB_STATS & 2
#define TBMARK(k_) do { __builtin_amdgcn_s_waitcnt(0); const unsigned long long now_ = __builtin_readcyclecounter(); tphase[k_] += now_ - tmark; tmark = now_; } while (0)
      unsigned long long tmark = __builtin_readcyclecounter();
#else
#define TBMARK(k_) do { } while (0)
#endif
#pragma unroll 1
      for (int tno = 0; tno < 2; ++tno)
        {
          const bool need = (tno == 0) ? busy : (busy && (m >= 1) && (r >= r0h) && (i >= 0) && (j >= 0) && (j < c0));
          if (tno == 1 && !__any(need)) break;
          const int cst = tno ? c0b : c0;
          TileIn in;
          load_tile(in, cst, tno ? m - 2 : m - 1);
          TBMARK(3 * tno);
          const int rmax_raw = __builtin_amdgcn_readfirstlane(wave_max_i32(need ? r - r0h : 0));
          const int cmax = __builtin_amdgcn_readfirstlane(wave_max_i32(need ? j - cst : 0));
          const bool tile_int = tno ? true : !__any(busy && (c0 + cmax >= D - 1));
          recompute(in, tno ? (m <= 1) : (m == 0), cst, rmax_raw, cmax, tile_int);
          TBMARK(3 * tno + 1);
          if (need) walk(cst);
          TBMARK(3 * tno + 2);
        }
      if (busy && r < 0 && L > 0) { --L; r = R - 1; }
    }
#if VSX_TB_STATS
  if (valid) atomicAdd(&vsx_tb_stats_dev[5], 1ull);
  if (tid == 0)
    {
      atomicAdd(&vsx_tb_stats_dev[15], __builtin_readcyclecounter() - t_kernel0); atomicAdd(&vsx_tb_stats_dev[0], (unsigned long long) n_iter);
      for (int k2 = 0; k2 < 6; ++k2) atomicAdd(&vsx_tb_stats_dev[8 + k2], tphase[k2]);
    }
#endif
  if (!valid) return;

  VsxPairOut o;
  o.pad = 0; o.nruns = 0; o.run_off = 0;
  if (so.overflow)
    {
      o.score = 32767; o.aligned = 0; o.matches = 0; o.mismatches = 0; o.gaps = 0;
      out[pair_ids[k]] = o;
      rank_note(FL, pair_ids[k], 0u, 32767, 0.0);
      return;
    }
  if (i >= 0) { al += (u32) (i + 1); if (op != 2) ++ga; push_n(2, (u32) (i + 1)); }
  if (j >= 0) { al += (u32) (j + 1); if (op != 1) ++ga; push_n(1, (u32) (j + 1)); }
  if (op >= 0) my[nruns++] = (runlen << 2) | (u32) op;

  u32 ma = 0, mi = 0;
  {
    int qi = Q - 1, tj = D - 1;
    for (u32 x = 0; x < nruns; ++x)
      {
        const u32 w = my[x];
        const int len = (int) (w >> 2);
        const u32 o2 = w & 3u;
        if (o2 == 0)
          {
            for (int b = 0; b < len; b += 8)
              {
                const int rem = (len - b < 8) ? len - b : 8;
                const unsigned long long aw = *reinterpret_cast<const u64_unaligned *>(q + (qi - b - 7));
                const unsigned long long cw = *reinterpret_cast<const u64_unaligned *>(d + (tj - b - 7));
                const unsigned long long ones = 0x0101010101010101ull;
                const unsigned long long x2 = aw & cw;
                unsigned long long t = (x2 | (x2 >> 1) | (x2 >> 2) | (x2 >> 3)) & ones;
                if (P.n_mismatch)
                  {
                    const unsigned long long a15 = aw & (aw >> 1) & (aw >> 2) & (aw >> 3);
                    const unsigned long long c15 = cw & (cw >> 1) & (cw >> 2) & (cw >> 3);
                    t &= ~(a15 | c15);
                  }
                t &= ~0ull << (8 * (8 - rem));
                const u32 m8 = (u32) __builtin_popcountll(t);
                ma += m8;
                mi += (u32) rem - m8;
              }
            qi -= len; tj -= len;
          }
        else if (o2 == 1) tj -= len;
        else qi -= len;
      }
  }

  u32 verdict = 0;
  double idv = 0.0;
  if (FL.enabled && nruns > 0) verdict = accept_verdict(FL, Q, D, (int) al, (int) ma, (int) mi, (int) ga, my[nruns - 1], my[0], &idv);
  if (verdict == 3u) nruns = 0;
  rank_note(FL, pair_ids[k], verdict, (int) so.score, idv);

  const unsigned long long base = atomicAdd(cursor, (unsigned long long) nruns);
  if (base + nruns <= runs_capacity)
    for (u32 x = 0; x < nruns; ++x) runs[base + x] = my[x];

  o.score = so.score;
  o.aligned = (uint16_t) al; o.matches = (uint16_t) ma; o.mismatches = (uint16_t) mi; o.gaps = (uint16_t) ga;
  o.pad = (uint16_t) verdict;
  o.nruns = nruns;
  o.run_off = base;
  out[pair_ids[k]] = o;
}

DEV u32 map4(u32 ch)
{
  const u32 c = ch | 0x20u;
  if (((ch | 0x20u) < 'a') || ((ch | 0x20u) > 'z') || ((ch & 0xC0u) != 0x40u)) return 0;
  switch (c)
    {
    case 'a': return 1;  case 'b': return 14; case 'c': return 2;  case 'd': return 13;
    case 'g': return 4;  case 'h': return 11; case 'k': return 12; case 'm': return 3;
    case 'n': return 15; case 'r': return 5;  case 's': return 6;  case 't': return 8;
    case 'u': return 8;  case 'v': return 7;  case 'w': return 9;  case 'y': return 10;
    default: return 0;
    }
}

__global__ void __launch_bounds__(256)
vsx_encode_kernel(const uint8_t * __restrict__ ascii, uint8_t * __restrict__ codes, uint64_t nbytes)
{
  __shared__ uint8_t lut[256];
  lut[threadIdx.x] = (uint8_t) map4(threadIdx.x);
  __syncthreads();
  const uint64_t nvec = nbytes >> 4;
  const uint64_t stride = (uint64_t) gridDim.x * blockDim.x;
  for (uint64_t v = (uint64_t) blockIdx.x * blockDim.x + threadIdx.x; v < nvec; v += stride)
    {
      const uint4 in = reinterpret_cast<const uint4 *>(ascii)[v];
      u32 w[4] = {in.x, in.y, in.z, in.w};
      u32 o[4];
#pragma unroll
      for (int x = 0; x < 4; ++x)
        o[x] = (u32) lut[w[x] & 0xff] | ((u32) lut[(w[x] >> 8) & 0xff] << 8) |
               ((u32) lut[(w[x] >> 16) & 0xff] << 16) | ((u32) lut[w[x] >> 24] << 24);
      reinterpret_cast<uint4 *>(codes)[v] = make_uint4(o[0], o[1], o[2], o[3]);
    }
  if (blockIdx.x == 0 && threadIdx.x < (nbytes & 15))
    {
      const uint64_t p = (nvec << 4) + threadIdx.x;
      codes[p] = lut[ascii[p]];
    }
}

__global__ void __launch_bounds__(256)
vsx_purity_kernel(const uint8_t * __restrict__ codes, const uint64_t * __restrict__ off,
                  const uint32_t * __restrict__ len, uint64_t nseq, uint8_t * __restrict__ impure)
{
  const uint64_t s = (uint64_t) blockIdx.x * 4 + (threadIdx.x >> 6);
  if (s >= nseq) return;
  const int lane = threadIdx.x & 63;
  const uint8_t * p = codes + off[s];
  const uint32_t n = len[s];
  int bad = 0;
  for (uint32_t x = lane; x < n; x += 64)
    {
      const u32 c = p[x];
      bad |= !((c != 0) && ((c & (c - 1)) == 0));
    }
  const unsigned long long any = __ballot(bad);
  if (lane == 0) impure[s] = any ? 1 : 0;
}

__global__ void __launch_bounds__(256)
vsx_max3_selftest_kernel(u32 * bad)
{
  const u32 x = blockIdx.x * 256u + threadIdx.x;
  if (x > 0x7BFFu) return;
  const u32 edge[8] = {0u, 1u, 0x03FFu, 0x0400u, 0x3C00u, 0x3E00u, 0x7BFEu, 0x7BFFu};
  u32 wrong = 0;
  for (u32 k = 0; k < 64; ++k)
    {
      const u32 h = (x * 2654435761u) ^ (k * 0x9E3779B9u);
      const u32 y = (k < 8) ? edge[k] : (h >> 7) % 0x7C00u;
      const u32 z = (k < 16) ? edge[(k + 3) & 7] : (h >> 17) % 0x7C00u;
      const u32 a = x | (y << 16), b = y | (z << 16), c = z | (x << 16);
      const u32 got = pk_max3_bits(a, b, c);
      const u32 m = x > y ? (x > z ? x : z) : (y > z ? y : z);
      if (got != (m | (m << 16))) ++wrong;
      const u32 pa = h ^ (x << 13), pb = (h * 0x85EBCA6Bu) ^ k;
      const u32 pg = __builtin_amdgcn_perm(pa, pb, 0x0B0A0908u);
      const u32 pe = ((pb >> 15) & 1u) * 0xFFu | (((pb >> 31) & 1u) * 0xFFu) << 8 | (((pa >> 15) & 1u) * 0xFFu) << 16 | (((pa >> 31) & 1u) * 0xFFu) << 24;
      if (pg != pe) atomicAdd(bad + 1, 1u);
    }
  if (wrong) atomicAdd(bad, wrong);
}
static std::atomic<int> g_tb_v1_dev[65];
extern "C" void vsx_internal_set_tb_v2(int device, int on) { g_tb_v1_dev[device < 0 || device > 64 ? 64 : device].store(on ? 0 : 1); }
extern "C" hipError_t vsx_launch_max3_selftest(u32 * d_bad, hipStream_t st)
{
  hipLaunchKernelGGL(vsx_max3_selftest_kernel, dim3((0x7C00 + 255) / 256), dim3(256), 0, st, d_bad);
  return hipGetLastError();
}

static const int kRows[] = {1, 4, 8, 10, 12, 14, 16, 18, 20, 22, 24, 26, 28, 32};

extern "C" const int * vsx_supported_rows(int * count)
{
  *count = (int) (sizeof(kRows) / sizeof(kRows[0]));
  return kRows;
}

extern "C" hipError_t vsx_launch_encode(const uint8_t * d_ascii, uint8_t * d_codes, uint64_t nbytes, hipStream_t st)
{
  if (nbytes == 0) return hipSuccess;
  uint64_t blocks = ((nbytes >> 4) + 255) / 256;
  if (blocks < 1) blocks = 1;
  if (blocks > 256 * 8) blocks = 256 * 8;
  hipLaunchKernelGGL(vsx_encode_kernel, dim3((unsigned) blocks), dim3(256), 0, st, d_ascii, d_codes, nbytes);
  return hipGetLastError();
}

extern "C" hipError_t vsx_launch_purity(const uint8_t * d_codes, const uint64_t * d_off, const uint32_t * d_len,
                                        uint64_t nseq, uint8_t * d_impure, hipStream_t st)
{
  if (nseq == 0) return hipSuccess;
  hipLaunchKernelGGL(vsx_purity_kernel, dim3((unsigned) ((nseq + 3) / 4)), dim3(256), 0, st,
                     d_codes, d_off, d_len, nseq, d_impure);
  return hipGetLastError();
}

#define VSX_FWD_GO(GRID_, ...) hipLaunchKernelGGL((vsx_forward_kernel<__VA_ARGS__>), dim3(GRID_), dim3(64), 0, st, P, d_tasks, q, t, dir, strip, slot, ntasks)
#define VSX_FWD_GO4(GRID_, ...) hipLaunchKernelGGL((vsx_forward_kernel<__VA_ARGS__>), dim3(GRID_), dim3(256), 0, st, P, d_tasks, q, t, dir, strip, slot, ntasks)
template <int R>
static hipError_t launch_fwd2(int track, int nq, int one, const VsxDevParams & P, const VsxTask * d_tasks, uint32_t ntasks,
                              const uint8_t * q, const uint8_t * t, uint32_t * dir, uint2 * strip,
                              VsxSlotOut * slot, hipStream_t st)
{
  if (nq == 8)
    {
      if (!(P.tilt != 0 && !track) || (ntasks & 3u)) return hipErrorInvalidValue;
      if constexpr (R >= 4)
        {
          if (!one) return hipErrorInvalidValue;
          if (P.max3) VSX_FWD_GO4(ntasks / 4, R, false, true, true, 1, true, true); else VSX_FWD_GO4(ntasks / 4, R, false, true, false, 1, true, true);
          return hipGetLastError();
        }
      else return hipErrorInvalidValue;
    }
  if (nq != 1)
    {
      if (!(P.tilt != 0 && !track && (nq == 2 || nq == 4))) return hipErrorInvalidValue;
      if constexpr (R >= 4)
        {
          const uint32_t grid = (ntasks + (uint32_t) nq - 1) / (uint32_t) nq;
          if (nq == 2) { if (P.max3) VSX_FWD_GO(grid, R, false, true, true, 2); else VSX_FWD_GO(grid, R, false, true, false, 2); }
          else         { if (P.max3) VSX_FWD_GO(grid, R, false, true, true, 4); else VSX_FWD_GO(grid, R, false, true, false, 4); }
          return hipGetLastError();
        }
      else return hipErrorInvalidValue;
    }
  if (P.tilt != 0)
    {
      if (track) return hipErrorInvalidValue;
      if constexpr (R >= 4)
        {
          if (one)
            {
              if (P.max3) VSX_FWD_GO(ntasks, R, false, true, true, 1, false, true);
              else VSX_FWD_GO(ntasks, R, false, true, false, 1, false, true);
              return hipGetLastError();
            }
        }
      if (P.max3) VSX_FWD_GO(ntasks, R, false, true, true);
      else VSX_FWD_GO(ntasks, R, false, true);
    }
  else if (track) VSX_FWD_GO(ntasks, R, true);
  else VSX_FWD_GO(ntasks, R, false);
  return hipGetLastError();
}
#undef VSX_FWD_GO
#undef VSX_FWD_GO4

extern "C" hipError_t vsx_launch_forward(int rows, int track, int nq, int one, VsxDevParams P, const VsxTask * d_tasks, uint32_t ntasks,
                                         const uint8_t * q, const uint8_t * t, uint32_t * dir, uint2 * strip,
                                         VsxSlotOut * slot, hipStream_t st)
{
  if (ntasks == 0) return hipSuccess;
#define FWDR(RR) case RR: return launch_fwd2<RR>(track, nq, one, P, d_tasks, ntasks, q, t, dir, strip, slot, st)
  switch (rows)
    {
    FWDR(1); FWDR(4); FWDR(8); FWDR(10); FWDR(12); FWDR(14); FWDR(16); FWDR(18); FWDR(20); FWDR(22); FWDR(24); FWDR(26); FWDR(28); FWDR(32);
    default: return hipErrorInvalidValue;
    }
#undef FWDR
}

template <int R, bool MID>
static hipError_t launch_tbtilt(const VsxDevParams & P, const VsxFilterDev & F, const VsxTask * d_tasks, const uint32_t * d_pair_slot,
                                const uint32_t * d_pair_ids, uint32_t npairs, const uint8_t * q, const uint8_t * t,
                                const uint32_t * ck, const VsxSlotOut * slot, uint32_t * slab, const uint64_t * slab_off,
                                uint32_t * runs, uint64_t cap, unsigned long long * cursor, VsxPairOut * out, hipStream_t st)
{
  if constexpr (R >= 4)
    hipLaunchKernelGGL((vsx_traceback_tilt_kernel<R, MID>), dim3((npairs + 63) / 64), dim3(64), 0, st,
                       P, F, d_tasks, d_pair_slot, d_pair_ids, npairs, q, t, ck, slot, slab, slab_off, runs, cap, cursor, out);
  return hipGetLastError();
}

template <int R, bool FAST, bool CK8 = false, bool MID = false>
static hipError_t launch_tbck(const VsxDevParams & P, const VsxFilterDev & F, const VsxTask * d_tasks, const uint32_t * d_pair_slot,
                              const uint32_t * d_pair_ids, uint32_t npairs, const uint8_t * q, const uint8_t * t,
                              const uint32_t * ck, const VsxSlotOut * slot, uint32_t * slab, const uint64_t * slab_off,
                              uint32_t * runs, uint64_t cap, unsigned long long * cursor, VsxPairOut * out, hipStream_t st)
{
  hipLaunchKernelGGL((vsx_traceback_ck_kernel<R, FAST, CK8, MID>), dim3((npairs + 127) / 128), dim3(128), 0, st,
                     P, F, d_tasks, d_pair_slot, d_pair_ids, npairs, q, t, ck, slot, slab, slab_off, runs, cap, cursor, out);
  return hipGetLastError();
}

extern "C" hipError_t vsx_launch_traceback_ck(int rows, int fast16, VsxDevParams P, VsxFilterDev F, const VsxTask * d_tasks, const uint32_t * d_pair_slot,
                                              const uint32_t * d_pair_ids, uint32_t npairs,
                                              const uint8_t * q, const uint8_t * t,
                                              const uint32_t * ck, const VsxSlotOut * slot,
                                              uint32_t * slab, const uint64_t * slab_off,
                                              uint32_t * runs, uint64_t runs_capacity, unsigned long long * cursor,
                                              VsxPairOut * out, hipStream_t st)
{
  if (npairs == 0) return hipSuccess;
  static const bool v1_env = std::getenv("VSX_TB_V1") != nullptr;
  int dev_now = 0;
  if (hipGetDevice(&dev_now) != hipSuccess) { (void) hipGetLastError(); dev_now = 64; }
  const bool v2 = g_tb_v1_dev[dev_now < 0 || dev_now > 64 ? 64 : dev_now].load(std::memory_order_relaxed) == 0 && !v1_env;
#define TBCK(RR) case RR: return (fast16 && P.tilt != 0 && v2 && RR >= 4) ? launch_tbtilt<RR, VSX_MID(RR, true)>(P, F, d_tasks, d_pair_slot, d_pair_ids, npairs, q, t, ck, slot, slab, slab_off, runs, runs_capacity, cursor, out, st) \
                                 : (fast16 && P.tilt != 0) ? launch_tbck<RR, true, true, VSX_MID(RR, true)>(P, F, d_tasks, d_pair_slot, d_pair_ids, npairs, q, t, ck, slot, slab, slab_off, runs, runs_capacity, cursor, out, st) \
                                 : fast16 ? launch_tbck<RR, true>(P, F, d_tasks, d_pair_slot, d_pair_ids, npairs, q, t, ck, slot, slab, slab_off, runs, runs_capacity, cursor, out, st) \
                                        : launch_tbck<RR, false>(P, F, d_tasks, d_pair_slot, d_pair_ids, npairs, q, t, ck, slot, slab, slab_off, runs, runs_capacity, cursor, out, st)
  switch (rows)
    {
    TBCK(1); TBCK(4); TBCK(8); TBCK(10); TBCK(12); TBCK(14); TBCK(16); TBCK(18); TBCK(20); TBCK(22); TBCK(24); TBCK(26); TBCK(28); TBCK(32);
    default: return hipErrorInvalidValue;
    }
#undef TBCK
}

extern "C" uint64_t vsx_ckpt_dwords(uint64_t nstrips, uint64_t steps, uint64_t rows, int tilt)
{
  const uint64_t nblk = (steps + 15) >> 4;
  const uint64_t rowck = (((nstrips * steps) + 1) >> 1) * VSX_ROWCK_PAIR_DW(tilt != 0);
  if (tilt)
    {
      const bool mid = VSX_MID(rows, true);
      const uint64_t rt = mid ? rows / 2 : rows;
      const uint64_t nbh = (rt + (rt + 1) / 2 + 3) / 4;
      const uint64_t nb = mid ? 2 * nbh : nbh;
      return rowck + nstrips * nblk * 64 * 4 * nb + (mid ? rowck : 0);
    }
  return rowck + nstrips * nblk * 64 * 2 * rows;
}
```

vsearch_amd/csrc/vsx_host.cpp:

```cpp
#include "../../include/vsx.h"
#include "vsx_internal.h"

#include <hip/hip_runtime.h>
#include <cstdlib>
extern "C" uint64_t vsx_internal_memory_pressure(int device);
extern "C" void vsx_internal_poison(void * p, size_t bytes)
{
  static const bool on = std::getenv("VSX_POISON") != nullptr;
  if (on && p && bytes) { (void) hipMemset(p, 0xA5, bytes); (void) hipDeviceSynchronize(); }
}

#include <algorithm>
#include <cinttypes>
#include <cstdarg>
#include <cstdio>
#include <cstdlib>
#include <cstring>
#include <sched.h>
#include <thread>
#include <atomic>
#include <condition_variable>
#include <mutex>
#include <chrono>
#include <deque>
// ... 817 lines not shown
                                   const uint64_t * offsets, const uint32_t * lengths)
{
  return seqset_common(ctx, out, n, blob, false, blob_bytes, offsets, lengths, true);
}

int vsx_internal_seqset_create_cased(vsx_ctx * ctx, vsx_seqset ** out, uint64_t n, const char * blob, uint64_t blob_bytes,
                                     const uint64_t * offsets, const uint32_t * lengths, int mode)
{
  if (mode != 1 && mode != 2) return fail(VSX_EINVAL, "vsx_internal_seqset_create_cased: mode must be 1 (soft) or 2 (dust)");
  return seqset_common(ctx, out, n, blob, false, blob_bytes, offsets, lengths, false, mode);
}
const uint8_t * vsx_internal_seqset_lower(const vsx_seqset * s) { return s ? s->d_lower.p : nullptr; }
int vsx_internal_seqset_lower_download(const vsx_seqset * s, uint8_t * dst, uint64_t nbytes)
{
  if (!s || !s->d_lower.p || nbytes > s->lower_bytes) return fail(VSX_EINVAL, "vsx_internal_seqset_lower_download: no case bitmap of that size");
  HIPCHK(hipSetDevice(s->device));
  if (nbytes) HIPCHK(hipMemcpy(dst, s->d_lower.p, nbytes, hipMemcpyDeviceToHost));
  return VSX_OK;
}

int vsx_internal_mask_bits(vsx_ctx * ctx, uint64_t n, const char * blob, uint64_t blob_bytes, const uint64_t * offsets,
                           const uint32_t * lengths, int mode, uint8_t * bits_out)
{
  vsx_seqset * s = nullptr;
  int rc = vsx_internal_seqset_create_cased(ctx, &s, n, blob, blob_bytes, offsets, lengths, mode);
  if (rc != VSX_OK) return rc;
  rc = vsx_internal_seqset_lower_download(s, bits_out, (blob_bytes + 7) / 8);
  vsx_seqset_destroy(s);
  return rc;
}

int vsx_seqset_create_from_device(vsx_ctx * ctx, vsx_seqset ** out, uint64_t n, const void * d_blob,
                                  uint64_t blob_bytes, const uint64_t * offsets, const uint32_t * lengths)
{
  return seqset_common(ctx, out, n, d_blob, true, blob_bytes, offsets, lengths);
}

void vsx_seqset_destroy(vsx_seqset * s)
{
  if (!s) return;
  (void) hipSetDevice(s->device);
  delete s;
}

uint64_t vsx_seqset_count(const vsx_seqset * s) { return s ? s->n : 0; }

static int ensure_impure(const vsx_seqset * s)
{
  std::lock_guard<std::mutex> lk(s->impure_mu);
  if (s->have_impure) return VSX_OK;
  vsx_ctx * ctx = s->ctx;
  HIPCHK(hipSetDevice(ctx->device));
  PoolBuf<uint8_t> d_flags;
  HIPCHK(d_flags.alloc(s->pool_ref ? s->pool_ref.get() : nullptr, s->n));
  HIPCHK(vsx_launch_purity(s->codes(), s->d_off.p, s->d_len.p, s->n, d_flags.p, ctx->stream));
  s->impure.assign(s->n, 0);
  if (s->n) HIPCHK(hipMemcpyAsync(s->impure.data(), d_flags.p, s->n, hipMemcpyDeviceToHost, ctx->stream));
  HIPCHK(hipStreamSynchronize(ctx->stream));
  s->have_impure = true;
  return VSX_OK;
}

static bool no_overflow_possible(const vsx_ctx * ctx, int64_t Q, int64_t D)
{
  int64_t B = std::max<int64_t>(std::llabs(ctx->P.match), std::llabs(ctx->P.mismatch));
  int64_t G = 0;
  for (int k = 0; k < 12; ++k)
    {
      if (ctx->pen[k] < 0) return false;
      if (k < 6) G = std::max<int64_t>(G, ctx->pen[k]); else B = std::max<int64_t>(B, ctx->pen[k]);
    }
  if (ctx->pen[2] + ctx->pen[8] < ctx->pen[6] || ctx->pen[8] < ctx->pen[6]) return false;
  const int64_t Dp = (D + 3) & ~3ll;
  return 4 * G + (Q + Dp + 16) * B < 32000;
}

static int tilt_possible(const vsx_ctx * ctx, int64_t Q, int64_t D)
{
  if (ctx->Pt.tilt == 0) return 0;
  static const bool max3_off = std::getenv("VSX_MAX3") && std::strcmp(std::getenv("VSX_MAX3"), "0") == 0;
  int64_t B = std::max<int64_t>(std::llabs(ctx->P.match), std::llabs(ctx->P.mismatch));
  int64_t G = 0;
  for (int k = 0; k < 12; ++k)
    if (k < 6) G = std::max<int64_t>(G, ctx->pen[k]); else B = std::max<int64_t>(B, ctx->pen[k]);
  const int64_t Dp = (D + 3) & ~3ll;
  const int64_t reach = 4 * G + 2 * (Q + Dp + 64) * B;
  if (reach < 15800 && !max3_off && ctx->pen[4] > 0 &&
      ctx->device < 64 && g_max3_state[ctx->device].load(std::memory_order_relaxed) == 1) return 2;
  return reach < 32000 ? 1 : 0;
}

static int pick_rows(int Q)
{
  static const int forced = std::getenv("VSX_ROWS") ? std::atoi(std::getenv("VSX_ROWS")) : 0;
  if (forced > 0 && Q >= forced) return forced;
  int cnt = 0;
  const int * rows = vsx_supported_rows(&cnt);
  int idx = cnt - 1;
  for (int k = 0; k < cnt; ++k)
    if (16 * rows[k] >= Q) { idx = k; break; }
  while (idx > 0 && Q < rows[idx]) --idx;
  return rows[idx];
}

int vsx_plan_create(vsx_ctx * ctx, vsx_plan ** out, const vsx_seqset * queries, const vsx_seqset * targets,
                    uint64_t n_pairs, const uint32_t * qidx, const uint32_t * tidx, uint64_t dir_budget_bytes)
{
  if (!ctx || !out || !queries || !targets || (n_pairs && (!qidx || !tidx)))
    return fail(VSX_EINVAL, "vsx_plan_create: null argument");
  *out = nullptr;
  if (queries->device != ctx->device || targets->device != ctx->device)
    return fail(VSX_EINVAL, "vsx_plan_create: seqset lives on another device");
  if (n_pairs > 0xffffffffull / 8) return fail(VSX_EINVAL, "vsx_plan_create: too many pairs for one plan");
  static const bool timing = std::getenv("VSX_DEBUG_TIMING") != nullptr;
  auto now = []() { return std::chrono::duration<double>(std::chrono::steady_clock::now().time_since_epoch()).count(); };
  const double tc0 = now();
  const int nthc = (int) std::max<uint64_t>(1, std::min<uint64_t>((uint64_t) vsx_internal_usable_cpus(), n_pairs / 32768));
  {
    std::vector<uint64_t> bad((size_t) nthc, UINT64_MAX);
    auto check = [&](int t) {
      const uint64_t lo = n_pairs * (uint64_t) t / (uint64_t) nthc, hi = n_pairs * (uint64_t) (t + 1) / (uint64_t) nthc;
      for (uint64_t k = lo; k < hi; ++k)
        if (qidx[k] >= queries->n || tidx[k] >= targets->n) { bad[(size_t) t] = k; return; }
    };
    run_threads(nthc, check);
    for (int t = 0; t < nthc; ++t)
      if (bad[(size_t) t] != UINT64_MAX)
        return fail(VSX_EINVAL, "vsx_plan_create: pair %" PRIu64 " references a sequence out of range", bad[(size_t) t]);
  }
  HIPCHK(hipSetDevice(ctx->device));
  static const bool pair_env = std::getenv("VSX_PAIRPROF") ? std::strcmp(std::getenv("VSX_PAIRPROF"), "0") != 0 : (VSX_PAIRPROF_DEFAULT != 0);
  const bool pair_try = pair_env && n_pairs >= 32;

  std::unique_ptr<vsx_plan> pl(new vsx_plan);
  pl->ctx = ctx; pl->Q = queries; pl->T = targets; pl->n_pairs = n_pairs;
  {
    std::lock_guard<std::mutex> lk(ctx->slot_mu);
    const unsigned seq = ctx->plan_seq.fetch_add(1);
    int pick = -1;
    for (int k = 0; k < 3; ++k)
      if (ctx->slot_refs[k] == 0 && (pick < 0 || ctx->shared_dir[k].bytes() > ctx->shared_dir[pick].bytes())) pick = k;
    if (pick < 0)
      for (int k = 0; k < 3; ++k)
        if (pick < 0 || (int) (seq - ctx->slot_stamp[k]) > (int) (seq - ctx->slot_stamp[pick])) pick = k;
    ++ctx->slot_refs[pick];
    ctx->slot_stamp[pick] = seq;
    pl->dir_slot = pick;
    pl->slot_held = true;
  }

  std::vector<uint32_t> gpu_pairs;
  {
    std::vector<std::vector<uint32_t>> gp((size_t) nthc), special((size_t) nthc);
    std::vector<uint64_t> pcells((size_t) nthc, 0);
    auto classify = [&](int t) {
      const uint64_t lo = n_pairs * (uint64_t) t / (uint64_t) nthc, hi = n_pairs * (uint64_t) (t + 1) / (uint64_t) nthc;
      gp[(size_t) t].reserve(hi - lo);
      uint64_t cells = 0;
      for (uint64_t k = lo; k < hi; ++k)
        {
          const int64_t Q = queries->len[qidx[k]], D = targets->len[tidx[k]];
          if (ctx->force_fallback || Q == 0 || D == 0 || !fits(Q, D)) { special[(size_t) t].push_back((uint32_t) k); continue; }
          gp[(size_t) t].push_back((uint32_t) k);
          cells += (uint64_t) Q * (uint64_t) D;
        }
      pcells[(size_t) t] = cells;
    };
    run_threads(nthc, classify);
    size_t total = 0;
    for (auto & v : gp) total += v.size();
    gpu_pairs.resize(total);
    {
      std::vector<size_t> base((size_t) nthc);
      size_t acc = 0;
      for (int t = 0; t < nthc; ++t) { base[(size_t) t] = acc; acc += gp[(size_t) t].size(); pl->cells += pcells[(size_t) t]; }
      auto place = [&](int t) { if (!gp[(size_t) t].empty()) std::memcpy(gpu_pairs.data() + base[(size_t) t], gp[(size_t) t].data(), gp[(size_t) t].size() * 4); };
      run_threads(nthc, place);
    }
    for (int t = 0; t < nthc; ++t)
      for (uint32_t k : special[(size_t) t])
        {
          const int64_t Q = queries->len[qidx[k]], D = targets->len[tidx[k]];
          pl->host_pairs.push_back(k);
          pl->host_out.emplace_back();
          VsxPairOut & o = pl->host_out.back();
          auto sentinel = [&]() { o = VsxPairOut {}; o.score = 32767; };
          if (ctx->force_fallback) { sentinel(); continue; }
          if (Q == 0)
            {
              if (!fits(0, D)) { sentinel(); continue; }
              o = VsxPairOut {};
              o.aligned = (uint16_t) D; o.gaps = (uint16_t) D;
              if (D > 0)
                {
                  const int64_t a = -(int64_t) ctx->pen[1] - D * (int64_t) ctx->pen[7];
                  const int64_t b = -(int64_t) ctx->pen[5] - D * (int64_t) ctx->pen[11];
                  o.score = (int16_t) (uint16_t) (std::max(a, b) & 0xffff);
                  pl->host_cigar.push_back(std::to_string(D) + "I");
                  pl->host_cigar_pair.push_back(k);
                  pl->host_cigar_run.push_back(((uint32_t) D << 2) | 1u);
                }
              continue;
            }
          sentinel();
        }
  }
  const double tc1 = now();

  auto by_query = [&](uint32_t a, uint32_t b) { return qidx[a] < qidx[b]; };
  if (!std::is_sorted(gpu_pairs.begin(), gpu_pairs.end(), by_query)) std::stable_sort(gpu_pairs.begin(), gpu_pairs.end(), by_query);
  struct ProtoTask { uint32_t q; int rows; int track; int tilt; int nq; uint32_t n; uint32_t pair[8]; };
  static const bool sparse_on = !(std::getenv("VSX_SPARSE") && std::strcmp(std::getenv("VSX_SPARSE"), "0") == 0);
  std::vector<size_t> group_begin;
  for (size_t b = 0; b < gpu_pairs.size();)
    {
      group_begin.push_back(b);
      const uint32_t q = qidx[gpu_pairs[b]];
      size_t e = b;
      while (e < gpu_pairs.size() && qidx[gpu_pairs[e]] == q) ++e;
      b = e;
    }
  group_begin.push_back(gpu_pairs.size());
  const size_t ngroups = group_begin.size() - 1;
  const int nth = (int) std::max<size_t>(1, std::min<size_t>((size_t) vsx_internal_usable_cpus(), gpu_pairs.size() / 16384));
  std::vector<std::vector<ProtoTask>> part((size_t) nth);
  std::vector<std::vector<std::pair<size_t, size_t>>> pair_cand((size_t) nth);
  auto work = [&](int t) {
    const size_t p_lo = gpu_pairs.size() * (size_t) t / (size_t) nth, p_hi = gpu_pairs.size() * (size_t) (t + 1) / (size_t) nth;
    const size_t g_lo = (size_t) (std::lower_bound(group_begin.begin(), group_begin.end() - 1, p_lo) - group_begin.begin());
    const size_t g_hi = (t == nth - 1) ? ngroups : (size_t) (std::lower_bound(group_begin.begin(), group_begin.end() - 1, p_hi) - group_begin.begin());
    std::vector<ProtoTask> & outp = part[(size_t) t];
    for (size_t g = g_lo; g < g_hi; ++g)
      {
        const size_t b = group_begin[g], e = group_begin[g + 1];
        const uint32_t q = qidx[gpu_pairs[b]];
        std::stable_sort(gpu_pairs.begin() + (long) b, gpu_pairs.begin() + (long) e,
                         [&](uint32_t x, uint32_t y) { return targets->len[tidx[x]] > targets->len[tidx[y]]; });
        const int rows = pick_rows((int) queries->len[q]);
        const size_t first_of_query = outp.size();
        for (size_t x = b; x < e; x += VSX_TASK_SLOTS)
          {
            ProtoTask pt {};
            pt.q = q; pt.rows = rows;
            pt.n = (uint32_t) std::min<size_t>(VSX_TASK_SLOTS, e - x);
            uint32_t dmax = 0;
            for (uint32_t sidx = 0; sidx < pt.n; ++sidx)
              {
                pt.pair[sidx] = gpu_pairs[x + sidx];
                dmax = std::max(dmax, targets->len[tidx[pt.pair[sidx]]]);
              }
            pt.track = (!ctx->tb_packed && no_overflow_possible(ctx, queries->len[q], dmax)) ? 0 : 1;
            pt.tilt = (pt.track == 0) ? tilt_possible(ctx, queries->len[q], dmax) : 0;
            pt.nq = 1;
            if (sparse_on && pt.tilt && rows >= 4 && pt.n <= 4 && (int64_t) queries->len[q] <= 16ll * rows)
              pt.nq = pt.n <= 2 ? 4 : 2;
            outp.push_back(pt);
          }
        if (pair_try && rows >= 4 && outp.size() - first_of_query >= 4 && (int64_t) queries->len[q] <= 16ll * rows)
          {
            size_t eligible = 0;
            for (size_t k = first_of_query; k < outp.size(); ++k) eligible += (outp[k].nq == 1 && outp[k].tilt) ? 1 : 0;
            if (eligible >= 4) pair_cand[(size_t) t].emplace_back(first_of_query, outp.size());
          }
      }
  };
  run_threads(nth, work);
  bool any_pair_cand = false;
  for (const auto & v : pair_cand) any_pair_cand = any_pair_cand || !v.empty();
  if (any_pair_cand)
    {
      int rc = ensure_impure(queries);
      if (rc == VSX_OK) rc = ensure_impure(targets);
      if (rc != VSX_OK) return rc;
    }
  auto mark_pairs = [&](int t) {
    std::vector<ProtoTask> & outp = part[(size_t) t];
    for (const std::pair<size_t, size_t> & range : pair_cand[(size_t) t])
      {
        const size_t first_of_query = range.first, end_of_query = range.second;
        if (queries->impure[outp[first_of_query].q]) continue;
          {
            std::vector<size_t> ok;
            for (size_t k = first_of_query; k < end_of_query; ++k)
              {
                ProtoTask & pt = outp[k];
                if (pt.nq != 1 || !pt.tilt) continue;
                bool pure = true;
                for (uint32_t sidx = 0; sidx < pt.n && pure; ++sidx) pure = !targets->impure[tidx[pt.pair[sidx]]];
                if (pure) ok.push_back(k);
              }
            size_t i0 = 0;
            while (i0 < ok.size())
              {
                size_t i1 = i0;
                while (i1 < ok.size() && outp[ok[i1]].tilt == outp[ok[i0]].tilt) ++i1;
                const size_t whole = (i1 - i0) / 4 * 4;
                for (size_t k = i0; k < i0 + whole; ++k) outp[ok[k]].nq = 8;
                i0 = i1;
              }
          }
      }
  };
  if (any_pair_cand) run_threads(nth, mark_pairs);
  std::vector<ProtoTask> protos;
  {
    size_t total = 0;
    for (auto & v : part) total += v.size();
    protos.reserve(total);
    for (auto & v : part) protos.insert(protos.end(), v.begin(), v.end());
  }
  {
    static const bool no_promote = std::getenv("VSX_NO_PROMOTE") != nullptr;
    struct Cls { int rows, track, tilt, nq; size_t count; };
    std::vector<Cls> cls;
    for (const ProtoTask & pt : protos)
      {
        bool found = false;
        for (Cls & c : cls) if (c.rows == pt.rows && c.track == pt.track && c.tilt == pt.tilt && c.nq == pt.nq) { ++c.count; found = true; break; }
        if (!found) cls.push_back(Cls {pt.rows, pt.track, pt.tilt, pt.nq, 1});
      }
    std::vector<std::pair<size_t, int>> move;
    for (size_t a = 0; a < cls.size() && !no_promote; ++a)
      {
        int best = 0;
        for (const Cls & c : cls)
          if (c.track == cls[a].track && c.tilt == cls[a].tilt && c.nq == cls[a].nq && c.rows > cls[a].rows &&
              c.count >= 32 * cls[a].count && (best == 0 || c.rows < best))
            best = c.rows;
        if (best && cls[a].count < 4096) move.emplace_back(a, best);
      }
    for (auto & mv : move)
      for (int hop = 0; hop < 4; ++hop)
        for (const auto & other : move)
          {
            const Cls & a = cls[mv.first], & o = cls[other.first];
            if (o.rows == mv.second && o.track == a.track && o.tilt == a.tilt && o.nq == a.nq) { mv.second = other.second; break; }
          }
    if (!move.empty())
      for (ProtoTask & pt : protos)
        for (const auto & mv : move)
          {
            const Cls & c = cls[mv.first];
            if (pt.rows == c.rows && pt.track == c.track && pt.tilt == c.tilt && pt.nq == c.nq)
              {
                if ((int) queries->len[pt.q] > mv.second) pt.rows = mv.second;
                break;
              }
          }
  }
  if (sparse_on)
    {
      static const size_t sparse_min = std::getenv("VSX_SPARSE_MIN") ? (size_t) std::atoll(std::getenv("VSX_SPARSE_MIN")) : 4096;
      struct Key { int rows, track, tilt, nq; size_t count; };
      std::vector<Key> ks;
      for (const ProtoTask & pt : protos)
        {
          if (pt.nq != 2 && pt.nq != 4) continue;
          bool found = false;
          for (Key & c : ks) if (c.rows == pt.rows && c.track == pt.track && c.tilt == pt.tilt && c.nq == pt.nq) { ++c.count; found = true; break; }
          if (!found) ks.push_back(Key {pt.rows, pt.track, pt.tilt, pt.nq, 1});
        }
      bool any = false;
      for (const Key & c : ks) any = any || c.count < sparse_min;
      if (any)
        for (ProtoTask & pt : protos)
          if (pt.nq == 2 || pt.nq == 4)
            for (const Key & c : ks)
              if (c.count < sparse_min && pt.nq == c.nq && pt.rows == c.rows && pt.track == c.track && pt.tilt == c.tilt) { pt.nq = 1; break; }
    }
  auto by_class = [](const ProtoTask & a, const ProtoTask & b) {
    if (a.rows != b.rows) return a.rows < b.rows;
    if (a.track != b.track) return a.track < b.track;
    if (a.tilt != b.tilt) return a.tilt < b.tilt;
    return a.nq < b.nq;
  };
  if (!std::is_sorted(protos.begin(), protos.end(), by_class)) std::stable_sort(protos.begin(), protos.end(), by_class);

  double t_budget = 0;
  if (dir_budget_bytes == 0)
    {
      size_t free_b = 0, total_b = 0;
      const double tb0 = now();
      HIPCHK(hipMemGetInfo(&free_b, &total_b));
      t_budget = now() - tb0;
      free_b += ctx->pool.idle_bytes() + ctx->shared_dir[pl->dir_slot].bytes();
      dir_budget_bytes = std::min<uint64_t>((uint64_t) (free_b * 0.4), 128ull << 30);
      const uint64_t have = ctx->shared_dir[pl->dir_slot].bytes();
      if (have >= dir_budget_bytes / 2) dir_budget_bytes = have;
    }
  const uint64_t budget_dwords = std::max<uint64_t>(dir_budget_bytes / 4, 1);

  const double tc2 = now();
  const size_t NT = protos.size();
  pl->tasks.resize(NT);
  pl->pair_slot.resize(gpu_pairs.size());
  pl->pair_ids.resize(gpu_pairs.size());
  pl->slab_off.resize(gpu_pairs.size());
  std::vector<uint64_t> t_dwords(NT), t_slab(NT), t_pair0(NT);
  const int ntt = (int) std::max<size_t>(1, std::min<size_t>((size_t) vsx_internal_usable_cpus(), NT / 4096));
  run_threads(ntt, [&](int th) {
    const size_t lo = NT * (size_t) th / (size_t) ntt, hi = NT * (size_t) (th + 1) / (size_t) ntt;
    for (size_t x = lo; x < hi; ++x)
      {
        const ProtoTask & pt = protos[x];
        VsxTask t {};
        t.qoff = queries->off[pt.q];
        t.qlen = queries->len[pt.q];
        t.rows = (uint32_t) pt.rows;
        uint32_t dmax = 0;
        uint64_t slab = 0;
        for (uint32_t sl = 0; sl < pt.n; ++sl)
          {
            const uint32_t ti = tidx[pt.pair[sl]];
            t.toff[sl] = targets->off[ti];
            t.tlen[sl] = targets->len[ti];
            dmax = std::max(dmax, (targets->len[ti] + 3u) & ~3u);
            slab += (uint64_t) t.qlen + t.tlen[sl] + 1;
          }
        t.steps = dmax + 16;
        const uint64_t total_lanes = (t.qlen + pt.rows - 1) / pt.rows;
        const uint64_t nstrips = (total_lanes + 15) / 16;
        t_dwords[x] = vsx_ckpt_dwords(nstrips, t.steps, (uint64_t) pt.rows, pt.tilt);
        t.strip_off = nstrips > 1 ? 2ull * 4 * t.steps : 0;
        t_slab[x] = slab;
        pl->tasks[x] = t;
      }
  });
  size_t np_out = 0;
  Chunk cur;
  auto close_chunk = [&]() {
    if (cur.task_count) pl->chunks.push_back(cur);
    Chunk nc;
    nc.task_first = cur.task_first + cur.task_count;
    nc.pair_first = cur.pair_first + cur.pair_count;
    cur = nc;
  };
  uint32_t wave_left = 0, wave_steps = 0, wave_group = 0, pair_left = 0;
  uint64_t wave_off = 0;
  auto same_class = [&](size_t a, size_t b) {
    return protos[a].rows == protos[b].rows && protos[a].track == protos[b].track &&
           protos[a].tilt == protos[b].tilt && protos[a].nq == protos[b].nq;
  };
  for (size_t x = 0; x < NT; ++x)
    {
      const ProtoTask & pt = protos[x];
      VsxTask & t = pl->tasks[x];
      uint64_t dwords = t_dwords[x];
      const uint64_t strip = t.strip_off;
      const bool sparse_task = pt.nq == 2 || pt.nq == 4;
      if (pt.nq == 8)
        {
          if (pair_left == 0)
            {
              pair_left = 4;
              uint64_t gsum = 0;
              for (size_t y = x; y < std::min(NT, x + 4); ++y) gsum += t_dwords[y];
              if (cur.task_count && cur.dir_dwords + gsum + VSX_CK_SLACK_DW > budget_dwords) close_chunk();
            }
          --pair_left;
        }
      else if (sparse_task && wave_left == 0)
        {
          uint32_t smax = t.steps, members = 1;
          while (members < (uint32_t) pt.nq && x + members < NT && same_class(x, x + members)) { smax = std::max(smax, pl->tasks[x + members].steps); ++members; }
          wave_left = members; wave_steps = smax; wave_group = 0;
          dwords = vsx_ckpt_dwords(1, smax, (uint64_t) pt.rows, pt.tilt);
          if (cur.task_count && cur.dir_dwords + dwords + VSX_CK_SLACK_DW > budget_dwords) close_chunk();
          wave_off = cur.dir_dwords;
        }
      else if (sparse_task) dwords = 0;
      else if (cur.task_count && cur.dir_dwords + dwords + VSX_CK_SLACK_DW > budget_dwords) close_chunk();
      if (sparse_task)
        {
          t.dir_off = wave_off;
          t.steps = wave_steps;
          t.group0 = wave_group;
          wave_group += 4u / (uint32_t) pt.nq;
          --wave_left;
        }
      else t.dir_off = cur.dir_dwords;
      t.strip_off = cur.strip_elems;
      cur.dir_dwords += dwords;
      cur.strip_elems += strip;
      pl->dir_bytes_total += dwords * 4;
      if (cur.launches.empty() || cur.launches.back().rows != pt.rows ||
          cur.launches.back().track != pt.track || cur.launches.back().tilt != pt.tilt || cur.launches.back().nq != pt.nq)
        cur.launches.push_back(Launch {pt.rows, pt.track, pt.tilt, pt.nq, (uint32_t) x, 0, cur.pair_first + cur.pair_count, 0});
      cur.launches.back().count++;
      if (strip != 0) cur.launches.back().multi = true;
      cur.launches.back().pair_count += pt.n;
      t_pair0[x] = np_out;
      np_out += pt.n;
      const uint64_t slab = t_slab[x];
      t_slab[x] = cur.slab_words;
      cur.slab_words += slab;
      cur.pair_count += pt.n;
      cur.task_count++;
    }
  run_threads(ntt, [&](int th) {
    const size_t lo = NT * (size_t) th / (size_t) ntt, hi = NT * (size_t) (th + 1) / (size_t) ntt;
    for (size_t x = lo; x < hi; ++x)
      {
        const ProtoTask & pt = protos[x];
        const VsxTask & t = pl->tasks[x];
        uint64_t slab = t_slab[x];
        for (uint32_t sl = 0; sl < pt.n; ++sl)
          {
            const size_t o = (size_t) t_pair0[x] + sl;
            pl->pair_slot[o] = (uint32_t) x * VSX_TASK_SLOTS + sl;
            pl->pair_ids[o] = pt.pair[sl];
            pl->slab_off[o] = slab;
            slab += (uint64_t) t.qlen + t.tlen[sl] + 1;
          }
      }
  });
  close_chunk();
  const double tc3 = now();

  uint64_t max_dir = 1, max_strip = 1, max_slab = 1, worst_runs = 0;
  for (const Chunk & c : pl->chunks)
    {
      max_dir = std::max(max_dir, c.dir_dwords + VSX_CK_SLACK_DW);
      max_strip = std::max(max_strip, c.strip_elems);
      max_slab = std::max(max_slab, c.slab_words);
      worst_runs += c.slab_words;
    }
  const size_t ngp = pl->pair_ids.size();
  pl->runs_capacity = std::min<uint64_t>(worst_runs, std::max<uint64_t>(16ull << 20, 48ull * ngp)) + 1;
  HIPCHK(pl->d_tasks.alloc(&ctx->pool, pl->tasks.size()));
  HIPCHK(pl->d_pair_slot.alloc(&ctx->pool, ngp));
  HIPCHK(pl->d_pair_ids.alloc(&ctx->pool, ngp));
  HIPCHK(pl->d_slab_off.alloc(&ctx->pool, ngp));
  HIPCHK(pl->d_slot.alloc(&ctx->pool, pl->tasks.size() * VSX_TASK_SLOTS));
  HIPCHK(pl->d_out.alloc(&ctx->pool, n_pairs));
  HIPCHK(pl->d_cursor.alloc(&ctx->pool, 2));
  {
    const uint64_t np = std::max<uint64_t>(n_pairs, 1);
    const uint64_t width[7] = {2, 2, 2, 2, 2, 1, 8};
    uint64_t at = 0;
    for (int x = 0; x < 7; ++x) { pl->soa_off[x] = at; at += (np * width[x] + 15) & ~15ull; }
    pl->soa_bytes = at;
    HIPCHK(pl->d_soa.alloc(&ctx->pool, at));
    uint8_t * b = pl->d_soa.p;
    pl->soa.score = reinterpret_cast<int16_t *>(b + pl->soa_off[0]);
    pl->soa.aligned = reinterpret_cast<uint16_t *>(b + pl->soa_off[1]);
    pl->soa.matches = reinterpret_cast<uint16_t *>(b + pl->soa_off[2]);
    pl->soa.mismatches = reinterpret_cast<uint16_t *>(b + pl->soa_off[3]);
    pl->soa.gaps = reinterpret_cast<uint16_t *>(b + pl->soa_off[4]);
    pl->soa.verdict = b + pl->soa_off[5];
    pl->soa.text_off = reinterpret_cast<uint64_t *>(b + pl->soa_off[6]);
  }
  {
    std::lock_guard<std::mutex> lk(ctx->stage_mu);
    if (!ctx->cursor_slots.empty()) { pl->h_cursor = ctx->cursor_slots.back(); ctx->cursor_slots.pop_back(); }
  }
  if (!pl->h_cursor) HIPCHK(hipHostMalloc(reinterpret_cast<void **>(&pl->h_cursor), 64, hipHostMallocDefault));
  for (int k = 0; k < 2; ++k)
    {
      const uint64_t need = (k == 0 ? max_dir : max_slab) * 4;
      uint64_t seen = ctx->req_hwm[k].load();
      while (need > seen && !ctx->req_hwm[k].compare_exchange_weak(seen, need)) { }
    }
  HIPCHK(pl->d_dir[0].alloc(ctx->shared_dir[pl->dir_slot], &ctx->pool, max_dir));
  HIPCHK(pl->d_strip.alloc(&ctx->pool, max_strip));
  HIPCHK(pl->d_slab.alloc(ctx->shared_slab, &ctx->pool, max_slab));
  HIPCHK(pl->d_runs.alloc(&ctx->pool, pl->runs_capacity));
  pl->text_capacity = std::min<uint64_t>(6 * worst_runs + 8 * (uint64_t) ngp, std::max<uint64_t>(32ull << 20, 128ull * ngp)) + 16;
  HIPCHK(pl->d_text.alloc(&ctx->pool, pl->text_capacity));
  if (!pl->tasks.empty())
    HIPCHK(hipMemcpyAsync(pl->d_tasks.p, pl->tasks.data(), pl->tasks.size() * sizeof(VsxTask), hipMemcpyHostToDevice, ctx->stream_up));
  if (ngp)
    {
      HIPCHK(hipMemcpyAsync(pl->d_pair_slot.p, pl->pair_slot.data(), ngp * 4, hipMemcpyHostToDevice, ctx->stream_up));
      HIPCHK(hipMemcpyAsync(pl->d_pair_ids.p, pl->pair_ids.data(), ngp * 4, hipMemcpyHostToDevice, ctx->stream_up));
      HIPCHK(hipMemcpyAsync(pl->d_slab_off.p, pl->slab_off.data(), ngp * 8, hipMemcpyHostToDevice, ctx->stream_up));
    }
  HIPCHK(hipEventCreate(&pl->ev_begin));
  HIPCHK(hipEventCreate(&pl->ev_end));
  for (Chunk & c : pl->chunks)
    {
      HIPCHK(hipEventCreate(&c.e0));
      HIPCHK(hipEventCreate(&c.e1));
      HIPCHK(hipEventCreate(&c.e1b));
      HIPCHK(hipEventCreate(&c.e2));
    }
  HIPCHK(hipStreamSynchronize(ctx->stream_up));
  if (timing)
    std::fprintf(stderr, "vsx_plan_create: %llu pairs, %zu tasks: classify %.2f ms, group %.2f ms (budget query %.2f), tasks %.2f ms, device buffers + upload %.2f ms\n",
                 (unsigned long long) n_pairs, pl->tasks.size(), (tc1 - tc0) * 1e3, (tc2 - tc1) * 1e3, t_budget * 1e3, (tc3 - tc2) * 1e3, (now() - tc3) * 1e3);
  *out = pl.release();
  return VSX_OK;
}

int vsx_plan_set_filter(vsx_plan * pl, const vsx_filter * f)
{
  if (!pl) return fail(VSX_EINVAL, "vsx_plan_set_filter: null plan");
  pl->filter = VsxFilterDev {};
  if (!f) return VSX_OK;
  if (f->iddef < 0 || f->iddef > 4) return fail(VSX_EINVAL, "vsx_plan_set_filter: iddef must be 0..4");
  VsxFilterDev & d = pl->filter;
  d.enabled = 1; d.iddef = f->iddef; d.leftjust = f->leftjust; d.rightjust = f->rightjust;
  d.id = f->id; d.weak_id = f->weak_id; d.maxid = f->maxid; d.mid = f->mid; d.query_cov = f->query_cov; d.target_cov = f->target_cov;
  d.maxsubs = f->maxsubs; d.maxgaps = f->maxgaps; d.mincols = f->mincols; d.maxdiffs = f->maxdiffs;
  pl->ran = false;
  return VSX_OK;
}

static int plan_set_ranked(vsx_plan * pl)
{
  if (!pl->filter.enabled) return VSX_OK;
  vsx_ctx * ctx = pl->ctx;
  const size_t n = (size_t) pl->n_pairs;
  HIPCHK(hipSetDevice(ctx->device));
  HIPCHK(pl->d_rank_counts.alloc(&ctx->pool, 2));
  HIPCHK(pl->d_kept_pair.alloc(&ctx->pool, n + 1));
  HIPCHK(pl->d_kept_id.alloc(&ctx->pool, n + 1));
  HIPCHK(pl->d_refused_pair.alloc(&ctx->pool, n + 1));
  pl->filter.rank_counts = pl->d_rank_counts.p;
  pl->filter.kept_pair = pl->d_kept_pair.p;
  pl->filter.kept_id = pl->d_kept_id.p;
  pl->filter.refused_pair = pl->d_refused_pair.p;
  return VSX_OK;
}

int vsx_plan_run(vsx_plan * pl)
{
  if (!pl) return fail(VSX_EINVAL, "vsx_plan_run: null plan");
  vsx_ctx * ctx = pl->ctx;
  HIPCHK(hipSetDevice(ctx->device));
  hipStream_t st = pl->alt_fwd ? ctx->stream_b : ctx->stream, st2 = ctx->stream2;
  const int slot = pl->dir_slot;
  HIPCHK(hipMemsetAsync(pl->d_cursor.p, 0, 2 * sizeof(unsigned long long), st));
  if (pl->filter.rank_counts) HIPCHK(hipMemsetAsync(pl->d_rank_counts.p, 0, 2 * sizeof(uint32_t), st));
  HIPCHK(hipEventRecord(pl->ev_begin, st));
  for (size_t k = 0; k < pl->chunks.size(); ++k)
    {
      Chunk & c = pl->chunks[k];
      uint32_t * dir = pl->d_dir[0].p;
      if (k >= 1) HIPCHK(hipStreamWaitEvent(st, pl->chunks[k - 1].e2, 0));
      else if (ctx->ev_tb_used[slot]) HIPCHK(hipStreamWaitEvent(st, ctx->ev_tb[slot], 0));
      HIPCHK(hipEventRecord(c.e0, st));
      for (const Launch & L : c.launches)
        {
          VsxDevParams Pf = L.tilt ? ctx->Pt : ctx->P;
          Pf.max3 = (L.tilt == 2) ? 1 : 0;
          static const bool one_off = std::getenv("VSX_ONESTRIP") && std::strcmp(std::getenv("VSX_ONESTRIP"), "0") == 0;
          HIPCHK(vsx_launch_forward(L.rows, L.track, L.nq, (L.multi || (one_off && L.nq != 8)) ? 0 : 1, Pf, pl->d_tasks.p + L.first, L.count,
                                    pl->Q->codes(), pl->T->codes(), dir, pl->d_strip.p,
                                    pl->d_slot.p + (size_t) L.first * VSX_TASK_SLOTS, st));
        }
      HIPCHK(hipEventRecord(c.e1, st));
      HIPCHK(hipStreamWaitEvent(st2, c.e1, 0));
      HIPCHK(hipEventRecord(c.e1b, st2));
      for (size_t li = 0; li < c.launches.size();)
        {
          const Launch & L = c.launches[li];
          uint32_t pair_count = L.pair_count;
          size_t lj = li + 1;
          while (lj < c.launches.size() && c.launches[lj].rows == L.rows &&
                 c.launches[lj].track == L.track && c.launches[lj].tilt == L.tilt) { pair_count += c.launches[lj].pair_count; ++lj; }
          VsxDevParams Pb = L.tilt ? ctx->Pt : ctx->P;
          Pb.max3 = (L.tilt == 2) ? 1 : 0;
          HIPCHK(vsx_launch_traceback_ck(L.rows, L.track == 0 ? 1 : 0, Pb, pl->filter, pl->d_tasks.p, pl->d_pair_slot.p + L.pair_first,
                                         pl->d_pair_ids.p + L.pair_first, pair_count, pl->Q->codes(), pl->T->codes(),
                                         dir, pl->d_slot.p, pl->d_slab.p, pl->d_slab_off.p + L.pair_first,
                                         pl->d_runs.p, pl->runs_capacity, pl->d_cursor.p, pl->d_out.p, st2));
          li = lj;
        }
      HIPCHK(hipEventRecord(c.e2, st2));
    }
  if (pl->chunks.empty()) HIPCHK(hipStreamWaitEvent(st2, pl->ev_begin, 0));
  HIPCHK(hipEventRecord(ctx->ev_tb[slot], st2));
  ctx->ev_tb_used[slot] = true;
  HIPCHK(vsx_launch_cigar_text(pl->d_out.p, pl->d_pair_ids.p, (uint32_t) pl->pair_ids.size(), pl->d_runs.p, pl->runs_capacity,
                               pl->d_text.p, pl->text_capacity, pl->d_cursor.p + 1, pl->soa, st2));
  HIPCHK(hipMemcpyAsync(pl->h_cursor, pl->d_cursor.p, 2 * sizeof(unsigned long long), hipMemcpyDeviceToHost, st2));
  HIPCHK(hipEventRecord(pl->ev_end, st2));
  pl->ran = true;
  pl->host_patched = false;
  return VSX_OK;
}

int vsx_plan_sync(vsx_plan * pl, vsx_timing * tm)
{
  if (!pl) return fail(VSX_EINVAL, "vsx_plan_sync: null plan");
  if (!pl->ran) return fail(VSX_EINVAL, "vsx_plan_sync: plan has not been run");
  HIPCHK(hipSetDevice(pl->ctx->device));
  HIPCHK(hipEventSynchronize(pl->ev_end));
  if (tm)
    {
      *tm = vsx_timing {};
      for (Chunk & c : pl->chunks)
        {
          float a = 0, b = 0;
          HIPCHK(hipEventElapsedTime(&a, c.e0, c.e1));
          HIPCHK(hipEventElapsedTime(&b, c.e1b, c.e2));
          tm->forward_ms += a;
          tm->traceback_ms += b;
          tm->forward_launches += (uint32_t) c.launches.size();
          tm->traceback_launches += 1;
        }
      HIPCHK(hipEventElapsedTime(&tm->total_ms, pl->ev_begin, pl->ev_end));
      tm->cells = pl->cells;
      tm->dir_bytes = pl->dir_bytes_total;
    }
  return VSX_OK;
}

int vsx_plan_describe(const vsx_plan * pl, vsx_plan_info * info)
{
  if (!pl || !info) return fail(VSX_EINVAL, "vsx_plan_describe: null argument");
  *info = vsx_plan_info {};
  info->tasks = pl->tasks.size();
  info->chunks = (uint32_t) pl->chunks.size();
  uint64_t best = 0;
  for (const Chunk & c : pl->chunks)
    for (const Launch & L : c.launches)
      {
        if (L.nq == 2 || L.nq == 4) info->tasks_sparse += L.count;
        if (L.nq == 8) info->tasks_pair += L.count;
        info->waves += (L.nq == 2 || L.nq == 4) ? (L.count + (uint32_t) L.nq - 1) / (uint32_t) L.nq : L.count;
        if (L.tilt) info->tasks_tilted += L.count;
        if (L.tilt == 2) info->tasks_max3 += L.count;
        if (L.track) info->tasks_tracked += L.count;
        if (L.count > best) { best = L.count; info->rows_dominant = (uint32_t) L.rows; }
      }
  return VSX_OK;
}

static void append_cigar(std::string & s, const uint32_t * runs, uint32_t n)
{
  static const char ops[4] = {'M', 'I', 'D', '?'};
  char buf[16];
  for (uint32_t k = n; k-- > 0;)
    {
      const uint32_t len = runs[k] >> 2;
      if (len > 1) { int w = snprintf(buf, sizeof buf, "%u", len); s.append(buf, (size_t) w); }
      s.push_back(ops[runs[k] & 3]);
    }
}

struct FetchDest {
  int16_t * score; uint16_t * aligned, * matches, * mismatches, * gaps; uint64_t * cigar_off; uint8_t * verdict;
  char ** blob; uint64_t * blob_used;
};

static int settle(vsx_plan * pl, unsigned long long & used, unsigned long long & text_used)
{
  vsx_ctx * ctx = pl->ctx;
  if (!pl->ran) { int rc = vsx_plan_run(pl); if (rc != VSX_OK) return rc; }
  int rc = vsx_plan_sync(pl, nullptr);
  if (rc != VSX_OK) return rc;
  HIPCHK(hipSetDevice(ctx->device));
  hipStream_t st = ctx->stream;
  used = pl->h_cursor[0]; text_used = pl->h_cursor[1];
  if (used > pl->runs_capacity)
    {
      pl->runs_capacity = used + 1;
      HIPCHK(pl->d_runs.alloc(&pl->ctx->pool, pl->runs_capacity));
      if ((rc = vsx_plan_run(pl)) != VSX_OK) return rc;
      if ((rc = vsx_plan_sync(pl, nullptr)) != VSX_OK) return rc;
      used = pl->h_cursor[0]; text_used = pl->h_cursor[1];
      if (used > pl->runs_capacity) return fail(VSX_EHIP, "vsx_plan_fetch: run buffer overflow after resize");
    }
  if (text_used > pl->text_capacity)
    {
      pl->text_capacity = text_used + 16;
      HIPCHK(pl->d_text.alloc(&pl->ctx->pool, pl->text_capacity));
      HIPCHK(hipMemsetAsync(pl->d_cursor.p + 1, 0, sizeof(unsigned long long), st));
      HIPCHK(vsx_launch_cigar_text(pl->d_out.p, pl->d_pair_ids.p, (uint32_t) pl->pair_ids.size(), pl->d_runs.p, pl->runs_capacity,
                                   pl->d_text.p, pl->text_capacity, pl->d_cursor.p + 1, pl->soa, st));
      HIPCHK(hipMemcpyAsync(pl->h_cursor, pl->d_cursor.p, 2 * sizeof(unsigned long long), hipMemcpyDeviceToHost, st));
      HIPCHK(hipStreamSynchronize(st));
      text_used = pl->h_cursor[1];
      if (text_used > pl->text_capacity) return fail(VSX_EHIP, "vsx_plan_fetch: text buffer overflow after resize");
    }
  return VSX_OK;
}

static int stage_reserve(vsx_ctx * ctx, uint64_t need)
{
  if (need <= ctx->stage_bytes) return VSX_OK;
  if (ctx->stage) { (void) hipHostFree(ctx->stage); ctx->stage = nullptr; ctx->stage_bytes = 0; }
  const uint64_t want = need + need / 4 + (1u << 20);
  if (hipHostMalloc(reinterpret_cast<void **>(&ctx->stage), want, hipHostMallocDefault) != hipSuccess)
    { (void) hipGetLastError(); return fail(VSX_ENOMEM, "vsx_plan_fetch: pinned staging allocation failed"); }
  ctx->stage_bytes = want;
  return VSX_OK;
}

static int fetch_core(vsx_plan * pl, const FetchDest & D)
{
  vsx_ctx * ctx = pl->ctx;
  unsigned long long used = 0, text_used = 0;
  int rc = settle(pl, used, text_used);
  if (rc != VSX_OK) return rc;

  const uint64_t n = pl->n_pairs;
  uint64_t tail = 0;
  for (size_t h = 0, hc = 0; h < pl->host_pairs.size(); ++h)
    {
      ++tail;
      if (hc < pl->host_cigar_pair.size() && pl->host_cigar_pair[hc] == pl->host_pairs[h]) tail += pl->host_cigar[hc++].size();
    }
  const uint64_t base = *D.blob_used;
  {
    char * nb = (char *) std::realloc(*D.blob, std::max<uint64_t>(base + text_used + tail, 1));
    if (!nb) return fail(VSX_ENOMEM, "vsx_plan_fetch: host allocation failed");
    *D.blob = nb;
  }
  char * const blob = *D.blob;

  {
    std::lock_guard<std::mutex> lk(ctx->stage_mu);
    if ((rc = stage_reserve(ctx, pl->soa_bytes + ((text_used + 15) & ~15ull))) != VSX_OK) return rc;
    hipError_t e = hipSuccess;
    if (n) e = hipMemcpyAsync(ctx->stage, pl->d_soa.p, pl->soa_bytes, hipMemcpyDeviceToHost, ctx->stream_dn);
    if (e == hipSuccess && text_used) e = hipMemcpyAsync(ctx->stage + pl->soa_bytes, pl->d_text.p, text_used, hipMemcpyDeviceToHost, ctx->stream_dn);
    if (e == hipSuccess) e = hipStreamSynchronize(ctx->stream_dn);
    if (e != hipSuccess) return fail(VSX_EHIP, "vsx_plan_fetch: %s", hipGetErrorString(e));
    const uint8_t * sg = ctx->stage;
    const int nth = copy_threads(n * 19 + text_used);
    run_threads(nth, [&](int t) {
      const uint64_t lo = n * (uint64_t) t / (uint64_t) nth, hi = n * (uint64_t) (t + 1) / (uint64_t) nth;
      if (hi > lo)
        {
          std::memcpy(D.score + lo, sg + pl->soa_off[0] + 2 * lo, 2 * (hi - lo));
          std::memcpy(D.aligned + lo, sg + pl->soa_off[1] + 2 * lo, 2 * (hi - lo));
          std::memcpy(D.matches + lo, sg + pl->soa_off[2] + 2 * lo, 2 * (hi - lo));
          std::memcpy(D.mismatches + lo, sg + pl->soa_off[3] + 2 * lo, 2 * (hi - lo));
          std::memcpy(D.gaps + lo, sg + pl->soa_off[4] + 2 * lo, 2 * (hi - lo));
          if (D.verdict) std::memcpy(D.verdict + lo, sg + pl->soa_off[5] + lo, hi - lo);
          const uint64_t * so = reinterpret_cast<const uint64_t *>(sg + pl->soa_off[6]);
          for (uint64_t k = lo; k < hi; ++k) D.cigar_off[k] = so[k] + base;
        }
      const uint64_t blo = text_used * (uint64_t) t / (uint64_t) nth, bhi = text_used * (uint64_t) (t + 1) / (uint64_t) nth;
      if (bhi > blo) std::memcpy(blob + base + blo, sg + pl->soa_bytes + blo, bhi - blo);
    });
  }
  uint64_t at = base + text_used;
  for (size_t h = 0, hc = 0; h < pl->host_pairs.size(); ++h)
    {
      const uint32_t k = pl->host_pairs[h];
      const VsxPairOut & o = pl->host_out[h];
      D.score[k] = o.score; D.aligned[k] = o.aligned; D.matches[k] = o.matches;
      D.mismatches[k] = o.mismatches; D.gaps[k] = o.gaps;
      if (D.verdict) D.verdict[k] = (uint8_t) VSX_VERDICT_UNDECIDED;
      D.cigar_off[k] = at;
      if (hc < pl->host_cigar_pair.size() && pl->host_cigar_pair[hc] == k)
        {
          std::memcpy(blob + at, pl->host_cigar[hc].data(), pl->host_cigar[hc].size());
          at += pl->host_cigar[hc++].size();
        }
      blob[at++] = '\0';
    }
  *D.blob_used = at;
  return VSX_OK;
}

struct RankedSink {
  std::vector<uint32_t> pair, undecided;
  std::vector<int16_t> score;
  std::vector<uint16_t> aligned, matches, mismatches, gaps;
  std::vector<uint8_t> verdict;
  std::vector<double> id;
  std::vector<uint64_t> cigar_off;
  char * blob = nullptr;
  uint64_t blob_used = 0;
  int keep_weak = 0;
  ~RankedSink() { std::free(blob); }
};

static int fetch_ranked_lists(vsx_plan * pl, uint64_t first, const uint32_t * qkey, RankedSink & S, unsigned long long text_used)
{
  vsx_ctx * ctx = pl->ctx;
  hipStream_t st = ctx->stream_dn;
  const uint64_t n = pl->n_pairs;
  uint32_t counts[2] = {0, 0};
  HIPCHK(hipMemcpyAsync(counts, pl->d_rank_counts.p, sizeof counts, hipMemcpyDeviceToHost, st));
  HIPCHK(hipStreamSynchronize(st));
  const uint32_t kept = counts[0], n_refused = counts[1];
  if (kept > n || n_refused > n) return fail(VSX_EHIP, "vsx_align_pairs_ranked: the kept / refused lists are corrupt");
  if (n_refused)
    {
      std::vector<uint32_t> rf(n_refused);
      HIPCHK(hipMemcpy(rf.data(), pl->d_refused_pair.p, (size_t) n_refused * 4, hipMemcpyDeviceToHost));
      std::sort(rf.begin(), rf.end());
      for (uint32_t k : rf) S.undecided.push_back((uint32_t) (first + k));
    }
  if (!kept) return VSX_OK;
  const uint64_t width[9] = {4, 8, 8, 2, 2, 2, 2, 2, 1};
  uint64_t off[9], at = 0;
  for (int x = 0; x < 9; ++x) { off[x] = at; at += ((uint64_t) kept * width[x] + 15) & ~15ull; }
  const uint64_t rank_bytes = at;
  PoolBuf<uint8_t> d_rank;
  HIPCHK(d_rank.alloc(&ctx->pool, rank_bytes));
  VsxRankedOut R;
  R.pair = reinterpret_cast<uint32_t *>(d_rank.p + off[0]);
  R.id = reinterpret_cast<double *>(d_rank.p + off[1]);
  R.text_off = reinterpret_cast<uint64_t *>(d_rank.p + off[2]);
  R.score = reinterpret_cast<int16_t *>(d_rank.p + off[3]);
  R.aligned = reinterpret_cast<uint16_t *>(d_rank.p + off[4]);
  R.matches = reinterpret_cast<uint16_t *>(d_rank.p + off[5]);
  R.mismatches = reinterpret_cast<uint16_t *>(d_rank.p + off[6]);
  R.gaps = reinterpret_cast<uint16_t *>(d_rank.p + off[7]);
  R.verdict = d_rank.p + off[8];
  HIPCHK(vsx_rank_gather_list(pl->d_kept_pair.p, pl->d_kept_id.p, kept, pl->d_out.p, pl->soa.text_off, R, st));
  std::lock_guard<std::mutex> lk(ctx->stage_mu);
  int rc = stage_reserve(ctx, rank_bytes + ((text_used + 15) & ~15ull));
  if (rc != VSX_OK) return rc;
  HIPCHK(hipMemcpyAsync(ctx->stage, d_rank.p, rank_bytes, hipMemcpyDeviceToHost, st));
  if (text_used) HIPCHK(hipMemcpyAsync(ctx->stage + rank_bytes, pl->d_text.p, text_used, hipMemcpyDeviceToHost, st));
  HIPCHK(hipStreamSynchronize(st));
  const uint8_t * sg = ctx->stage;
  const char * text = reinterpret_cast<const char *>(sg + rank_bytes);
  const uint32_t * h_pair = reinterpret_cast<const uint32_t *>(sg + off[0]);
  const double * h_id = reinterpret_cast<const double *>(sg + off[1]);
  const uint64_t * h_toff = reinterpret_cast<const uint64_t *>(sg + off[2]);
  const int16_t * h_score = reinterpret_cast<const int16_t *>(sg + off[3]);
  const uint16_t * h_al = reinterpret_cast<const uint16_t *>(sg + off[4]), * h_ma = reinterpret_cast<const uint16_t *>(sg + off[5]);
  const uint16_t * h_mi = reinterpret_cast<const uint16_t *>(sg + off[6]), * h_ga = reinterpret_cast<const uint16_t *>(sg + off[7]);
  const uint8_t * h_vd = sg + off[8];
  std::vector<uint32_t> order;
  order.reserve(kept);
  for (uint32_t j = 0; j < kept; ++j)
    {
      if (h_pair[j] >= n) return fail(VSX_EHIP, "vsx_align_pairs_ranked: a kept pair is out of range");
      if (h_vd[j] == 1u || (S.keep_weak && h_vd[j] == 2u)) order.push_back(j);
    }
  std::vector<uint32_t> seg((size_t) n);
  for (uint64_t k = 1; k < n; ++k) seg[k] = seg[k - 1] + (qkey[k] != qkey[k - 1] ? 1u : 0u);
  std::sort(order.begin(), order.end(), [&](uint32_t a, uint32_t b) {
    const uint32_t pa = h_pair[a], pb = h_pair[b];
    if (seg[pa] != seg[pb]) return seg[pa] < seg[pb];
    if (h_id[a] != h_id[b]) return h_id[a] > h_id[b];
    return pa < pb;
  });
  const size_t m = order.size(), base = S.pair.size();
  S.pair.resize(base + m); S.id.resize(base + m); S.cigar_off.resize(base + m);
  S.score.resize(base + m); S.aligned.resize(base + m); S.matches.resize(base + m);
  S.mismatches.resize(base + m); S.gaps.resize(base + m); S.verdict.resize(base + m);
  uint64_t need = 0;
  std::vector<uint32_t> slen(m);
  for (size_t x = 0; x < m; ++x) { slen[x] = (uint32_t) std::strlen(text + h_toff[order[x]]) + 1; need += slen[x]; }
  char * nb = (char *) std::realloc(S.blob, std::max<uint64_t>(S.blob_used + need, 1));
  if (!nb) return fail(VSX_ENOMEM, "vsx_align_pairs_ranked: host allocation failed");
  S.blob = nb;
  for (size_t x = 0; x < m; ++x)
    {
      const uint32_t j = order[x];
      S.pair[base + x] = (uint32_t) (first + h_pair[j]);
      S.id[base + x] = h_id[j];
      S.score[base + x] = h_score[j]; S.aligned[base + x] = h_al[j]; S.matches[base + x] = h_ma[j];
      S.mismatches[base + x] = h_mi[j]; S.gaps[base + x] = h_ga[j]; S.verdict[base + x] = h_vd[j];
      S.cigar_off[base + x] = S.blob_used;
      std::memcpy(S.blob + S.blob_used, text + h_toff[j], slen[x]);
      S.blob_used += slen[x];
    }
  return VSX_OK;
}

static int fetch_ranked_core(vsx_plan * pl, uint64_t first, const uint32_t * qkey, RankedSink & S)
{
  unsigned long long used = 0, text_used = 0;
  int rc = settle(pl, used, text_used);
  if (rc != VSX_OK) return rc;
  const uint64_t n = pl->n_pairs;
  for (uint32_t k : pl->host_pairs) S.undecided.push_back((uint32_t) (first + k));
  if (n == 0) return VSX_OK;
  if (!pl->filter.rank_counts) return fail(VSX_EINVAL, "vsx_align_pairs_ranked: the plan has no ranking lists");
  return fetch_ranked_lists(pl, first, qkey, S, text_used);
}

static int results_alloc(vsx_results * out, uint64_t n, bool with_verdict)
{
  std::memset(out, 0, sizeof *out);
  const uint64_t n1 = std::max<uint64_t>(n, 1);
  out->n_pairs = n;
  out->score = (int16_t *) std::malloc(n1 * 2);
  out->aligned = (uint16_t *) std::malloc(n1 * 2);
  out->matches = (uint16_t *) std::malloc(n1 * 2);
  out->mismatches = (uint16_t *) std::malloc(n1 * 2);
  out->gaps = (uint16_t *) std::malloc(n1 * 2);
  out->cigar_off = (uint64_t *) std::malloc(n1 * 8);
  out->verdict = with_verdict ? (uint8_t *) std::malloc(n1) : nullptr;
  out->cigar_blob = (char *) std::malloc(1);
  if (!out->score || !out->aligned || !out->matches || !out->mismatches || !out->gaps || !out->cigar_off || !out->cigar_blob ||
      (with_verdict && !out->verdict))
    { vsx_results_free(out); return fail(VSX_ENOMEM, "vsx_plan_fetch: host allocation failed"); }
  return VSX_OK;
}

static FetchDest dest_at(vsx_results * out, uint64_t first)
{
  return FetchDest {out->score + first, out->aligned + first, out->matches + first, out->mismatches + first, out->gaps + first,
                    out->cigar_off + first, out->verdict ? out->verdict + first : nullptr, &out->cigar_blob, &out->cigar_bytes};
}

int vsx_plan_fetch(vsx_plan * pl, vsx_results * out)
{
  if (!pl || !out) return fail(VSX_EINVAL, "vsx_plan_fetch: null argument");
  int rc = results_alloc(out, pl->n_pairs, pl->filter.enabled != 0);
  if (rc != VSX_OK) return rc;
  rc = fetch_core(pl, dest_at(out, 0));
  if (rc != VSX_OK) { const std::string keep = g_err; vsx_results_free(out); g_err = keep; }
  return rc;
}

int vsx_plan_export_hits(vsx_plan * pl, void * d_dst, uint64_t dst_bytes)
{
  static_assert(sizeof(VsxPairOut) == VSX_HIT_RECORD_BYTES, "hit record layout");
  if (!pl || !d_dst) return fail(VSX_EINVAL, "vsx_plan_export_hits: null argument");
  if (!pl->ran) return fail(VSX_EINVAL, "vsx_plan_export_hits: plan has not been run");
  if (dst_bytes < pl->n_pairs * sizeof(VsxPairOut)) return fail(VSX_EINVAL, "vsx_plan_export_hits: destination too small");
  HIPCHK(hipSetDevice(pl->ctx->device));
  hipStream_t st = pl->ctx->stream;
  HIPCHK(hipEventSynchronize(pl->ev_end));
  if (!pl->host_patched)
    {
      HIPCHK(hipEventSynchronize(pl->ev_end));
      const uint64_t used = pl->h_cursor[0];
      for (size_t h = 0, hc = 0; h < pl->host_pairs.size(); ++h)
        {
// ... 271 lines not shown
```

vsearch_amd/csrc/vsx_internal.h:

```cpp
#ifndef VSX_INTERNAL_H
#define VSX_INTERNAL_H

#include <stdint.h>
#include <hip/hip_runtime_api.h>

#define VSX_TASK_SLOTS 8
#define VSX_GROUP_LANES 16
#define VSX_MAX_SEQLEN_SUM 65535LL
#define VSX_MAX_SEQLEN_PRODUCT 25000000LL
#define VSX_TABLE_LEN (65536 + 64)
#define VSX_CODE_SLACK 64
#define VSX_CK_SLACK_DW 4096
#ifndef VSX_MID_MIN_ROWS
#define VSX_MID_MIN_ROWS 18
#endif
#define VSX_MID(R_, TILT_) ((TILT_) && (R_) >= VSX_MID_MIN_ROWS)

struct VsxDevParams {
  uint32_t match_pk;
  uint32_t qrq_i_pk, rq_i_pk;
  uint32_t qrq_r_pk, rq_r_pk;
  int32_t  qrt_i, rt_i;
  int32_t  qrt_r, rt_r;
  int32_t  match, mismatch;
  int32_t  smin;
  int32_t  n_mismatch;
  int32_t  share_sub;
  int32_t  top_open, top_step;
  int32_t  tilt;
  int32_t  max3;
  const int16_t * htop;
  const int16_t * hleft;
  const int16_t * matrix;
};

struct VsxTask {
  uint64_t qoff;
  uint64_t toff[VSX_TASK_SLOTS];
  uint64_t dir_off;
  uint64_t strip_off;
  uint32_t tlen[VSX_TASK_SLOTS];
  uint32_t qlen;
  uint32_t steps;
  uint32_t rows;
  uint32_t group0;
};

struct VsxFilterDev {
  int32_t enabled, iddef, leftjust, rightjust;
  double  id, weak_id, maxid, mid, query_cov, target_cov;
  int64_t maxsubs, maxgaps, mincols, maxdiffs;
  uint32_t * rank_counts;
  uint32_t * kept_pair;
  double   * kept_id;
  uint32_t * refused_pair;
};

struct VsxSlotOut {
  int16_t  score;
  uint16_t overflow;
  uint16_t leave;
  uint16_t pad;
};

struct VsxPairOut {
  int16_t  score;
  uint16_t aligned, matches, mismatches, gaps;
  uint16_t pad;
  uint32_t nruns;
  uint64_t run_off;
};

struct VsxSoaOut {
  int16_t  * score;
  uint16_t * aligned, * matches, * mismatches, * gaps;
  uint8_t  * verdict;
  uint64_t * text_off;
};

struct VsxRankedOut {
  uint32_t * pair;
  int16_t  * score;
  uint16_t * aligned, * matches, * mismatches, * gaps;
  uint8_t  * verdict;
  double   * id;
  uint64_t * text_off;
};

#define VSX_CHIM_MAXCAND 16
struct VsxChimItem {
  uint32_t q;
  uint32_t ncand;
  uint32_t pair0;
  uint32_t out;
  uint32_t cand[VSX_CHIM_MAXCAND];
};
struct VsxChimParams {
  double minh, mindiv, xn, dn;
  int64_t mindiffs;
  int32_t variant;
  int32_t pad;
};

#ifdef __cplusplus
extern "C" {
#endif

hipError_t vsx_launch_chimera_eval(const VsxChimItem * d_items, uint32_t nitems, const uint8_t * qcodes, const uint64_t * qoff,
                                   const uint32_t * qlen, const uint8_t * tcodes, const uint64_t * toff, const uint32_t * tlen,
                                   const VsxPairOut * d_hits, const uint32_t * d_runs, uint64_t n_runs, VsxChimParams P,
                                   void * d_out, hipStream_t st);

hipError_t vsx_rank_gather_list(const uint32_t * d_kept_pair, const double * d_kept_id, uint32_t kept, const VsxPairOut * d_out,
                                const uint64_t * d_text_off, VsxRankedOut r, hipStream_t st);

hipError_t vsx_launch_cigar_text(const VsxPairOut * d_out, const uint32_t * d_pair_ids, uint32_t npairs,
                                 const uint32_t * d_runs, uint64_t runs_capacity,
                                 uint8_t * d_text, uint64_t text_capacity, unsigned long long * d_text_cursor,
                                 VsxSoaOut soa, hipStream_t st);

hipError_t vsx_launch_revcomp(uint8_t * d_codes, const uint64_t * d_src_off, const uint64_t * d_dst_off,
                              const uint32_t * d_len, uint64_t nseq, hipStream_t st);

hipError_t vsx_launch_encode(const uint8_t * d_ascii, uint8_t * d_codes, uint64_t nbytes, hipStream_t st);
hipError_t vsx_launch_purity(const uint8_t * d_codes, const uint64_t * d_off, const uint32_t * d_len,
                             uint64_t nseq, uint8_t * d_impure, hipStream_t st);
hipError_t vsx_launch_forward(int rows, int track, int nq, int one , VsxDevParams P, const VsxTask * d_tasks, uint32_t ntasks,
                              const uint8_t * d_qcodes, const uint8_t * d_tcodes,
                              uint32_t * d_dir, uint2 * d_strip, VsxSlotOut * d_slot, hipStream_t st);
hipError_t vsx_launch_traceback_ck(int rows, int fast16, VsxDevParams P, VsxFilterDev F, const VsxTask * d_tasks, const uint32_t * d_pair_slot,
                                   const uint32_t * d_pair_ids, uint32_t npairs,
                                   const uint8_t * d_qcodes, const uint8_t * d_tcodes,
                                   const uint32_t * d_ck, const VsxSlotOut * d_slot,
                                   uint32_t * d_slab, const uint64_t * d_slab_off,
                                   uint32_t * d_runs, uint64_t runs_capacity, unsigned long long * d_cursor,
                                   VsxPairOut * d_out, hipStream_t st);
hipError_t vsx_launch_max3_selftest(uint32_t * d_bad , hipStream_t st);
void vsx_internal_set_tb_v2(int device, int on);
uint64_t vsx_ckpt_dwords(uint64_t nstrips, uint64_t steps, uint64_t rows, int tilt );
const int * vsx_supported_rows(int * count);

hipError_t vsx_kmer_launch_sweep(int fill, const uint8_t * codes, const uint64_t * off, const uint32_t * len,
                                 const uint32_t * seq_list, uint32_t nseq, int w, uint32_t ntiles, uint32_t * bucket_count,
                                 const uint64_t * bucket_start, uint32_t * postings, const uint8_t * lower_bits, hipStream_t st);
hipError_t vsx_kmer_launch_case_bits(const uint8_t * d_ascii, uint64_t nbytes, uint8_t * d_bits , int fold_case,
                                     hipStream_t st);
hipError_t vsx_launch_dust(const uint8_t * d_codes, const uint64_t * d_off, const uint32_t * d_len, uint64_t nseq, uint8_t * d_bits,
                           hipStream_t st);
hipError_t vsx_kmer_launch_ranges(const uint64_t * bucket_start, uint32_t ntiles, const uint64_t * qk_start, const uint32_t * qk,
                                  const uint32_t * minmatch, const uint32_t * qlist, uint32_t nslots, void * ranges, hipStream_t st);
hipError_t vsx_kmer_launch_count(int bits, int tagged, const uint32_t * postings, const uint64_t * bucket_start, const void * ranges,
                                 uint32_t ntiles, uint32_t nseq, uint32_t nslots, uint32_t slot_base, const uint64_t * qk_start,
                                 const uint32_t * qk, const uint32_t * minmatch, const uint32_t * qlist, void * rec, uint32_t subcap,
                                 uint32_t * tile_count, hipStream_t st);
hipError_t vsx_kmer_tagged_tile(int fill, const uint8_t * codes, const uint64_t * off, const uint32_t * len, uint32_t first_seq,
                                uint32_t nseq_tile, int w, const uint8_t * lower_bits, const uint64_t * slot_of , uint64_t n_slots,
                                uint64_t * keys_a, uint64_t * keys_b, void * temp, size_t * temp_bytes, uint32_t tile, uint32_t ntiles,
                                uint32_t * bucket_count, const uint64_t * bucket_start, uint32_t * postings, hipStream_t st);
hipError_t vsx_kmer_launch_select(const void * rec, uint32_t subcap, uint32_t ntiles, const uint32_t * tile_count, uint32_t nslots,
                                  uint32_t keep, void * dense, unsigned long long * cursor, uint64_t capacity,
                                  void * sel_m_n, uint64_t * sel_off, hipStream_t st);
uint32_t vsx_kmer_tile_shift(void);

#ifdef __cplusplus
}
#endif
#endif
```

Baseline: 8197.

## Add ACGT-target forward kernel class using pk_mad profile lookup

Adds a new forward-kernel specialization for tasks whose targets are all pure ACGT and whose query fits one strip. It builds a 4-code target-indexed profile in LDS packed as (score,1) pairs, so one b128 load covers four rows. Each row's substitution score plus diagonal is then formed with a single v_pk_mad_u16 instead of a perm plus add. The host marks eligible tasks (nq=16) after an impurity check on targets, and adds plan-info and profiling support. This trims one VALU per row cell but adds LDS loads inside the row loop, an extra host pass, and more kernel instantiations.

```diff
diff --git a/include/vsx.h b/include/vsx.h
--- a/include/vsx.h
+++ b/include/vsx.h
@@ -85,6 +85,7 @@
   uint64_t tasks_sparse;
   uint64_t waves;
   uint64_t tasks_pair;
+  uint64_t tasks_acgt;
 } vsx_plan_info;
 
 const char * vsx_version_string(void);
diff --git a/profiles/valu_budget.py b/profiles/valu_budget.py
--- a/profiles/valu_budget.py
+++ b/profiles/valu_budget.py
@@ -60,7 +60,7 @@
 
 
 def category(op, rest):
-    if op in ("v_pk_maximum3_f16", "v_pk_max_u16", "v_subrev_u32_e32", "v_sub_u32_e32", "v_subrev_u32_e64", "v_sub_u32_e64"):
+    if op in ("v_pk_maximum3_f16", "v_pk_max_u16", "v_pk_mad_u16", "v_subrev_u32_e32", "v_sub_u32_e32", "v_subrev_u32_e64", "v_sub_u32_e64"):
         return "row body"
     if op == "v_mov_b32_dpp":
         return "DPP hand-overs (feed, H, F)"
@@ -79,7 +79,8 @@
 
 def budget(body, R, S):
     c = collections.Counter()
-    quota = {"v_perm_b32": R * S, "v_add_u32_e32": R * S}
+    mad = any(op == "v_pk_mad_u16" for op, _ in body)
+    quota = {"v_perm_b32": 0 if mad else R * S, "v_add_u32_e32": 0 if mad else R * S}
     npk = sum(1 for op, _ in body if op == "v_pk_sub_i16")
     nashr = sum(1 for op, _ in body if op == "v_pk_ashrrev_i16")
     pk = [("row body", S), ("last row's own e / hf subtractions", 2 * S), ("leave-column tracking", nashr)]
@@ -110,7 +111,7 @@
 def main():
     ap = argparse.ArgumentParser()
     ap.add_argument("--lib", default=os.path.join(ROOT, "vsearch_amd", "libvsx.so"))
-    ap.add_argument("--kernel", default="16,false,true,true,1,false,true", help="template arguments of vsx_forward_kernel")
+    ap.add_argument("--kernel", default="16,false,true,true,1,false,true,true", help="template arguments of vsx_forward_kernel")
     ap.add_argument("--rows", type=int, default=None, help="R (default: the first template argument)")
     ap.add_argument("--loop", type=int, default=None, help="loop index to budget (default: most v_pk_maximum3_f16)")
     ap.add_argument("--ops", action="store_true", help="print the opcode histogram of the loop too")
@@ -160,11 +161,12 @@
     cond = [(ins[j][1], ins[j][2]) for j in L["cond"]]
     cm, _ = budget(body, R, S)
     per_step = L["valu_main"] / S + L["valu_cond"] / 16.0
+    rb = (5 if any(ins[j][1] == "v_pk_mad_u16" for j in L["main"]) else 6) * R
     print("  loop [%d]: %d steps per iteration (R = %d)" % (n, S, R))
     print("    VALU per two steps, always-taken path: %.1f" % (2.0 * L["valu_main"] / S))
     print("    VALU in branch-guarded regions (once per 16 steps): %d" % L["valu_cond"])
     print("    VALU per 16-step block: %.0f   per step: %.2f   (row body %d per step = %.1f %%)" % (
-        16 * per_step, per_step, 6 * R, 100.0 * 6 * R / per_step))
+        16 * per_step, per_step, rb, 100.0 * rb / per_step))
     print("    per step, by category (always-taken path / S, + branch-guarded / 16):")
     order = ["row body", "DPP hand-overs (feed, H, F)", "profile row addresses", "feed-slot addresses", "last row's own e / hf subtractions",
              "leave-column tracking", "checkpoint pack", "checkpoint addresses", "register copies", "other"]
diff --git a/vsearch_amd/_lib.py b/vsearch_amd/_lib.py
--- a/vsearch_amd/_lib.py
+++ b/vsearch_amd/_lib.py
@@ -134,7 +134,7 @@
 class PlanInfo(C.Structure):
     _fields_ = [("tasks", C.c_uint64), ("tasks_tilted", C.c_uint64), ("tasks_tracked", C.c_uint64),
                 ("rows_dominant", C.c_uint32), ("chunks", C.c_uint32), ("tasks_max3", C.c_uint64),
-                ("tasks_sparse", C.c_uint64), ("waves", C.c_uint64), ("tasks_pair", C.c_uint64)]
+                ("tasks_sparse", C.c_uint64), ("waves", C.c_uint64), ("tasks_pair", C.c_uint64), ("tasks_acgt", C.c_uint64)]
 
 
 class Timing(C.Structure):
diff --git a/vsearch_amd/csrc/ubench_d16.hip b/vsearch_amd/csrc/ubench_d16.hip
--- a/vsearch_amd/csrc/ubench_d16.hip
+++ b/vsearch_amd/csrc/ubench_d16.hip
@@ -37,19 +37,83 @@
 template <int MODE>
 __global__ void __launch_bounds__(64) __attribute__((amdgpu_waves_per_eu(MODE == 2 ? 2 : 4, 8))) k_rows(int steps, unsigned * out, unsigned seed)
 {
-  __shared__ __attribute__((aligned(16))) short QP[(MODE == 2 ? 2 : 1) * 16 * 16 * R];
-  for (int i = threadIdx.x; i < (MODE == 2 ? 2 : 1) * 16 * 16 * R; i += 64) QP[i] = (short) ((i * 7 + (int) seed) & 0xff);
+  constexpr int QPN = MODE <= 2 ? (MODE == 2 ? 2 : 1) * 16 * 16 * R : 8;
+  constexpr int TDN = MODE == 3 ? 4 * 16 * R : (MODE == 4 ? 8 * 16 * R : (MODE == 5 ? 16 * 16 * R / 4 : 4));
+  __shared__ __attribute__((aligned(16))) short QP[QPN];
+  __shared__ __attribute__((aligned(16))) unsigned TD[TDN];
+  for (int i = threadIdx.x; i < QPN; i += 64) QP[i] = (short) ((i * 7 + (int) seed) & 0xff);
+  for (int i = threadIdx.x; i < TDN; i += 64)
+    {
+      const unsigned v = (unsigned) (i * 7 + (int) seed) & 0xffu;
+      TD[i] = MODE == 3 ? (v | 1u << 16) : (MODE == 4 ? (i < 4 * 16 * R ? v : v << 16) : v * 0x01010101u);
+    }
   __syncthreads();
+  const uint4 * T4 = reinterpret_cast<const uint4 *>(TD);
   const int l = threadIdx.x & 15;
   unsigned H[R], H2[R], E[R];
   for (int r = 0; r < R; ++r) { H[r] = 0x3E003E00u + (unsigned) (r * 3 + (int) threadIdx.x); H2[r] = H[r]; E[r] = 0x3E003E00u - (unsigned) (r + (int) seed); }
   unsigned F = 0x3E003E00u, diag = 0x3E003E00u, sym = threadIdx.x * 2654435761u + seed;
   const unsigned go = 0x00120012u;
+  auto quad = [&](unsigned c, int k) { return (c * (R / 4) + (unsigned) k) * 16u + (unsigned) l; };
+  auto sym_next = [](unsigned s) { return s * 1664525u + 1013904223u; };
+  uint4 na = make_uint4(0, 0, 0, 0), nb = make_uint4(0, 0, 0, 0);
+  {
+    const unsigned s1 = sym_next(sym);
+    if (MODE == 3 || MODE == 4) { na = T4[quad((s1 >> 8) & 3u, 0)]; nb = T4[quad((MODE == 4 ? 4u : 0u) + ((s1 >> 20) & 3u), 0)]; }
+    if (MODE == 5) { na = T4[((s1 >> 8) & 15u) * 16u + (unsigned) l]; nb = T4[((s1 >> 20) & 15u) * 16u + (unsigned) l]; }
+  }
   auto step = [&](unsigned (&hin)[R], unsigned (&hout)[R]) __attribute__((always_inline)) {
-    sym = sym * 1664525u + 1013904223u;
+    sym = sym_next(sym);
     const unsigned ca = (sym >> 8) & 15u, cb = (sym >> 20) & 15u;
     unsigned Hd = diag;
-    if (MODE == 0)
+    if (MODE == 3 || MODE == 4)
+      {
+        const unsigned s1 = sym_next(sym);
+        const unsigned cA = ca & 3u, cB = (MODE == 4 ? 4u : 0u) + (cb & 3u);
+        const unsigned nA = (s1 >> 8) & 3u, nB = (MODE == 4 ? 4u : 0u) + ((s1 >> 20) & 3u);
+#pragma unroll
+        for (int k = 0; k < R / 4; ++k)
+          {
+            const uint4 xa = na, xb = nb;
+            if (k + 1 < R / 4) { na = T4[quad(cA, k + 1)]; nb = T4[quad(cB, k + 1)]; }
+            else { na = T4[quad(nA, 0)]; nb = T4[quad(nB, 0)]; }
+            const unsigned va[4] = {xa.x, xa.y, xa.z, xa.w}, vb[4] = {xb.x, xb.y, xb.z, xb.w};
+#pragma unroll
+            for (int q = 0; q < 4; ++q)
+              {
+                const int r = 4 * k + q;
+                unsigned h0;
+                if (MODE == 3) asm("v_pk_mad_u16 %0, %1, %2, %3 op_sel:[0,1,0] op_sel_hi:[1,0,1]" : "=v"(h0) : "v"(va[q]), "v"(vb[q]), "v"(Hd));
+                else h0 = va[q] + vb[q] + Hd;
+                const unsigned h2 = max3(h0, F, E[r]);
+                Hd = hin[r];
+                hout[r] = h2;
+                const unsigned he = h2 - go;
+                F = pmaxu(F, he);
+                E[r] = pmaxu(E[r], he);
+              }
+          }
+      }
+    else if (MODE == 5)
+      {
+        const unsigned s1 = sym_next(sym);
+        const uint4 xa = na, xb = nb;
+        na = T4[((s1 >> 8) & 15u) * 16u + (unsigned) l]; nb = T4[((s1 >> 20) & 15u) * 16u + (unsigned) l];
+        const unsigned va[4] = {xa.x, xa.y, xa.z, xa.w}, vb[4] = {xb.x, xb.y, xb.z, xb.w};
+#pragma unroll
+        for (int r = 0; r < R; ++r)
+          {
+            const unsigned V = __builtin_amdgcn_perm(vb[r >> 2], va[r >> 2], 0x0C040C00u + 0x00010001u * (unsigned) (r & 3));
+            const unsigned h0 = Hd + V;
+            const unsigned h2 = max3(h0, F, E[r]);
+            Hd = hin[r];
+            hout[r] = h2;
+            const unsigned he = h2 - go;
+            F = pmaxu(F, he);
+            E[r] = pmaxu(E[r], he);
+          }
+      }
+    else if (MODE == 0)
       {
         const short * qa = QP + ca * (16 * R) + l * R;
         const short * qb = QP + cb * (16 * R) + l * R;
@@ -145,13 +209,15 @@
   unsigned h0 = 0;
   CK(hipMemcpy(&h0, out, 4, hipMemcpyDeviceToHost));
   const double cycles = ms * 1e-3 * 2.4e9;
-  printf("mode %d (%s) waves/SIMD %d: %8.3f ms, %.1f cycles per lane-row and wave   [check %08x]\n", MODE,
-         MODE == 0 ? "b64 loads + perm, 6 VALU per row" : (MODE == 1 ? "u16 loads, add3, 5 VALU per row" : "pair profile, b128 loads, 5 VALU per row"), waves_per_simd, ms,
+  static const char * what[] = {"b64 loads + perm, 6 VALU per row", "u16 loads, add3, 5 VALU per row", "pair profile, b128 loads, 5 VALU per row",
+                                "ACGT (S',1) profile, b128 per 4 rows, pk_mad, 5 VALU per row", "ACGT (S',0)/(0,S') profiles, b128 per 4 rows, add3, 5 VALU per row",
+                                "byte profile, b128 per 16 rows, perm + add, 6 VALU per row"};
+  printf("mode %d (%s) waves/SIMD %d: %8.3f ms, %.1f cycles per lane-row and wave   [check %08x]\n", MODE, what[MODE], waves_per_simd, ms,
          cycles / ((double) steps * R * waves_per_simd), h0);
   CK(hipFree(out));
 }
 
-int main()
+int main(int argc, char ** argv)
 {
   hipDeviceProp_t p; CK(hipGetDeviceProperties(&p, 0));
   printf("device %s  CUs %d  arch %s\n", p.name, p.multiProcessorCount, p.gcnArchName);
@@ -160,6 +226,11 @@
   unsigned h[12]; CK(hipMemcpy(h, out, sizeof h, hipMemcpyDeviceToHost));
   printf("lane 0: d16_hi into 0xDEADBEEF -> %08x, d16 -> %08x, u16 -> %08x;  lane 1: %08x %08x %08x\n", h[0], h[1], h[2], h[3], h[4], h[5]);
   printf("  (table: lane x holds 0x1100 + x at its address, 0x2200 + x at +128)  d16_hi zeroes the low half: %s\n", (h[0] & 0xffffu) == 0 ? "YES" : "no");
+  if (argc > 1 && argv[1][0] == 'a')
+    {
+      for (int w = 2; w <= 4; ++w) { run<0>(w); run<5>(w); run<3>(w); run<4>(w); }
+      return 0;
+    }
   for (int w = 1; w <= 4; w *= 2) { run<0>(w); run<1>(w); if (w <= 2) run<2>(w); }
   run<0>(3);
   return 0;
diff --git a/vsearch_amd/csrc/vsx_device.hip b/vsearch_amd/csrc/vsx_device.hip
--- a/vsearch_amd/csrc/vsx_device.hip
+++ b/vsearch_amd/csrc/vsx_device.hip
@@ -35,6 +35,7 @@
 DEV u32 a_bfi_vs(u32 mask, u32 a, u32 b) { u32 r; asm("v_bfi_b32 %0, %1, %2, %3" : "=v"(r) : "v"(mask), "v"(a), "s"(b)); return r; }
 DEV u32 a_lshr1(u32 a) { u32 r; asm("v_lshrrev_b32 %0, 1, %1" : "=v"(r) : "v"(a)); return r; }
 DEV u32 a_pk_ashr15(u32 a) { u32 r; asm("v_pk_ashrrev_i16 %0, 15, %1 op_sel_hi:[0,1]" : "=v"(r) : "v"(a)); return r; }
+DEV u32 a_pk_mad_x(u32 a, u32 b, u32 c) { u32 r; asm("v_pk_mad_u16 %0, %1, %2, %3 op_sel:[0,1,0] op_sel_hi:[1,0,1]" : "=v"(r) : "v"(a), "v"(b), "v"(c)); return r; }
 DEV u32 funnel(u32 acc, u32 d) { return a_bfi(SIGN2, d, a_lshr1(acc)); }
 DEV u32 pack16(int v) { const u32 x = (u32) v & 0xffffu; return x | (x << 16); }
 
@@ -68,7 +69,7 @@
 #ifndef VSX_FWD_WAVES_NQ
 #define VSX_FWD_WAVES_NQ(R_, NQ_) ((NQ_) == 4 ? 2 : ((R_) <= 24 ? 3 : 2))
 #endif
-template <int R, bool TRACK, bool TILT = false, bool MAX3 = false, int NQ = 1, bool PAIR = false, bool ONE = false>
+template <int R, bool TRACK, bool TILT = false, bool MAX3 = false, int NQ = 1, bool PAIR = false, bool ONE = false, bool ACGT = false>
 __global__ void __launch_bounds__(PAIR ? 256 : 64) __attribute__((amdgpu_waves_per_eu(NQ == 1 ? (ONE ? VSX_FWD_WAVES_ONE(R, TILT) : VSX_FWD_WAVES(R, TILT)) : VSX_FWD_WAVES_NQ(R, NQ), 8)))
 vsx_forward_kernel(const VsxDevParams P, const VsxTask * __restrict__ tasks,
                    const uint8_t * __restrict__ qc, const uint8_t * __restrict__ tc,
@@ -96,8 +97,10 @@
   constexpr int WPB = PAIR ? 4 : 1;
   constexpr int QPBYTES = 16 * 16 * RP;
   constexpr int RPP = ((RP / 4) & 1) ? RP : RP + 4;
+  static_assert(!ACGT || (MAX3 && ONE && NQ == 1 && !PAIR), "the ACGT-target classes extend the single-strip MAX3 whole-wave kernels");
   __shared__ __attribute__((aligned(16))) u32 PPf[PAIR ? 16 * 16 * RPP : 4];
-  __shared__ __attribute__((aligned(16))) int16_t QP[!PAIR ? (QPL ? (NQ * QPBYTES) / 2 : 16 * 16 * R) : 8];
+  __shared__ __attribute__((aligned(16))) u32 TPf[ACGT ? 4 * 16 * RP : 4];
+  __shared__ __attribute__((aligned(16))) int16_t QP[(!PAIR && !ACGT) ? (QPL ? (NQ * QPBYTES) / 2 : 16 * 16 * R) : 8];
   constexpr int FSZ = (TILT ? 2 : 1) * 4 * 16;
   __shared__ uint4 FEED4a[FSZ * WPB];
   __shared__ u32 FEEDFa[FSZ * WPB];
@@ -172,6 +175,25 @@
                   PPf[(pr * 16 + row / RP) * RPP + rr] = ((u32) va & 0xffu) | (((u32) vb & 0xffu) << 16);
                 }
             }
+          else if (ACGT)
+            {
+              for (int idx = lane; idx < 4 * 16 * RP; idx += 64)
+                {
+                  const int code = idx / (16 * RP), row = idx % (16 * RP);
+                  const int Lr = 16 * s + row / RP, rr = row % RP;
+                  int v = 0;
+                  if (rr < R)
+                    {
+                      if (Lr == 0 && rr < pad) v = -P.top_step + 2 * tl;
+                      else if (Lr < total_lanes)
+                        {
+                          const int gi = (Lr == 0) ? rr - pad : rcnt0 + (Lr - 1) * R + rr;
+                          v = P.matrix[(1 << code) * 16 + (int) qq[gi]];
+                        }
+                    }
+                  TPf[((code * (RP / 4) + (rr >> 2)) * 16 + row / RP) * 4 + (rr & 3)] = ((u32) v & 0xffu) | 0x10000u;
+                }
+            }
           else if (QPL)
             {
               constexpr int LPT = 64 / NQ;
@@ -255,6 +277,12 @@
         else if (c < Dpg) rawS = strip_in[c];
       };
       prefetch(0);
+      auto profile_off = [&]() -> u32 {
+        const u32 ia = (rawA >> 1) - (rawA >> 3), ib = (rawB >> 1) - (rawB >> 3);
+        if (PAIR) return (ia * 4u + ib) * (u32) (16 * RPP * 4);
+        if (ACGT) return ia * (u32) (16 * RP * 4) | ((ib * (u32) (16 * RP * 4)) << 16);
+        return rawA * (u32) (16 * RP) | ((rawB * (u32) (16 * RP)) << 16);
+      };
 
       auto build_feed = [&](int blk, auto lean_tag) __attribute__((always_inline)) {
               constexpr bool LEAN = FEED2 && decltype(lean_tag)::value;
@@ -263,8 +291,7 @@
                 {
                   f_H = (s == 0) ? bpack(rawH - pad * tl) : rawS.x;
                   f_F = (s == 0) ? vsub(f_H, qrt_i_pk) : rawS.y;
-                  const u32 f_off = PAIR ? (((rawA >> 1) - (rawA >> 3)) * 4u + ((rawB >> 1) - (rawB >> 3))) * (u32) (16 * RPP * 4)
-                                         : (rawA * (u32) (16 * RP) | ((rawB * (u32) (16 * RP)) << 16));
+                  const u32 f_off = profile_off();
                   FEED4[(blk & 1) * 64 + gw * 16 + l] = make_uint4(f_off, 0u, f_H, f_F);
                   prefetch(blk + 1);
                   return;
@@ -291,8 +318,7 @@
               const int fo = QPL ? (blk & 1) * 64 : 0;
               if (FEED2)
                 {
-                  const u32 f_off = PAIR ? (((rawA >> 1) - (rawA >> 3)) * 4u + ((rawB >> 1) - (rawB >> 3))) * (u32) (16 * RPP * 4)
-                                         : (rawA * (u32) (16 * RP) | ((rawB * (u32) (16 * RP)) << 16));
+                  const u32 f_off = profile_off();
                   FEED4[fo + gw * 16 + l] = make_uint4(f_off, f_sym, f_H, f_F);
                   FEEDB[fo + gw * 16 + l] = make_uint2(f_qrt, f_rt);
                 }
@@ -304,16 +330,27 @@
               prefetch(blk + 1);
       };
       constexpr int PD = RP / 4;
-      u32 profA[2][(QPL && !PAIR) ? PD : 1], profB[2][(QPL && !PAIR) ? PD : 1];
-      auto load_profile = [&](u32 (&buf)[2][(QPL && !PAIR) ? PD : 1], u32 sy) __attribute__((always_inline)) {
+      constexpr int PBN = (QPL && !PAIR) ? (ACGT ? 4 : PD) : 1;
+      u32 profA[2][PBN], profB[2][PBN];
+      auto load_chunk = [&](u32 (&buf)[2][PBN], u32 sy, int k) __attribute__((always_inline)) {
+        if constexpr (ACGT)
+          {
+            const uint8_t * tp = reinterpret_cast<const uint8_t *>(TPf) + l * 16 + k * 256;
+            const uint4 va = *reinterpret_cast<const uint4 *>(tp + (sy & 0xFFFFu)), vb = *reinterpret_cast<const uint4 *>(tp + (sy >> 16));
+            buf[0][0] = va.x; buf[0][1] = va.y; buf[0][2] = va.z; buf[0][3] = va.w;
+            buf[1][0] = vb.x; buf[1][1] = vb.y; buf[1][2] = vb.z; buf[1][3] = vb.w;
+          }
+      };
+      auto load_profile = [&](u32 (&buf)[2][PBN], u32 sy) __attribute__((always_inline)) {
         if (PAIR) return;
+        if (ACGT) { load_chunk(buf, sy, 0); return; }
         const u32 cd = sy & 0x000F000Fu;
         constexpr int QPA = (RP % 16 == 0) ? 16 : ((RP % 8 == 0) ? 8 : 4);
         if (FEED2)
           {
             const uint8_t * pa = QPl + l * RP + (sy & 0xFFFFu);
             const uint8_t * pb = QPl + l * RP + (sy >> 16);
-            constexpr int PDN = (QPL && !PAIR) ? PD : 1;
+            constexpr int PDN = PBN;
             if constexpr (PAIR) { }
             else if constexpr (QPA == 16)
               {
@@ -346,7 +383,7 @@
         const u32 * a = reinterpret_cast<const u32 *>(QPl + (cd & 0xFu) * (16 * RP) + l * RP);
         const u32 * b = reinterpret_cast<const u32 *>(QPl + (cd >> 16) * (16 * RP) + l * RP);
 #pragma unroll
-        for (int k = 0; k < ((QPL && !PAIR) ? PD : 1); ++k) { buf[0][k] = a[k]; buf[1][k] = b[k]; }
+        for (int k = 0; k < PBN; ++k) { buf[0][k] = a[k]; buf[1][k] = b[k]; }
       };
       if (QPL)
         {
@@ -370,7 +407,7 @@
       u32 * const mck_base = dir + T.dir_off + ck_rowdw + (size_t) nstrips * ck_nblk * CK_COL_DW
                              + ((((size_t) s * steps) >> 1) * 64 + ck_slot) * CK_LANE_DW;
 
-      auto step = [&](const int t, u32 (&hin)[R], u32 (&hout)[R], u32 (&pc)[2][(QPL && !PAIR) ? PD : 1], u32 (&pn)[2][(QPL && !PAIR) ? PD : 1],
+      auto step = [&](const int t, u32 (&hin)[R], u32 (&hout)[R], u32 (&pc)[2][PBN], u32 (&pn)[2][PBN],
                       auto interior_tag, auto odd_tag, auto steady_tag) __attribute__((always_inline)) {
           constexpr bool INTERIOR = decltype(interior_tag)::value;
           constexpr bool ODD = decltype(odd_tag)::value;
@@ -399,7 +436,7 @@
             {
               const int t1 = t + 1;
               symn = dpp_shr1(feed4_g[(u32) (((t1 >> 4) & 1) * 64 + (t1 & 15))].x, sym);
-              load_profile(pn, symn);
+              if (!ACGT || !STEADY) load_profile(pn, symn);
             }
           else sym = dpp_shr1(fv.x, sym);
           if (!INTERIOR)
@@ -423,6 +460,7 @@
               const int16_t * qpA = QP + (code & 0xFu) * (16 * R) + l * R;
               const int16_t * qpB = QP + (code >> 16) * (16 * R) + l * R;
               u32 pa = 0, pb = 0;
+              u32 xa[4] = {}, xb[4] = {}, tq[2][PBN];
               u32 Hd = diag;
               u32 F = inF;
               u32 smn = 0x7FFF7FFFu, smx = 0x80008000u;
@@ -436,8 +474,19 @@
 #pragma unroll
               for (int r = 0; r < R; ++r)
                 {
-                  u32 V;
-                  if (PAIR) V = pp[r];
+                  u32 V = 0;
+                  if constexpr (ACGT)
+                    {
+                      if ((r & 3) == 0)
+                        {
+                          const int k = r >> 2;
+#pragma unroll
+                          for (int q = 0; q < 4; ++q) { xa[q] = k == 0 ? pc[0][q] : tq[0][q]; xb[q] = k == 0 ? pc[1][q] : tq[1][q]; }
+                          if (k + 1 < PD) load_chunk(tq, sym, k + 1);
+                          else if (STEADY) load_profile(pn, symn);
+                        }
+                    }
+                  else if (PAIR) V = pp[r];
                   else if (QPL)
                     {
                       if ((r & 3) == 0) { pa = pc[0][r >> 2]; pb = pc[1][r >> 2]; }
@@ -465,7 +514,7 @@
                         }
                       else V = (u32) (uint16_t) qpA[r] | ((u32) (uint16_t) qpB[r] << 16);
                     }
-                  const u32 h0 = vadd(Hd, V);
+                  const u32 h0 = ACGT ? a_pk_mad_x(xa[r & 3], xb[r & 3], Hd) : vadd(Hd, V);
                   const bool ONE_MAX = MAX3 && (r < R - 1 || LASTFAST);
                   const u32 h1 = ONE_MAX ? 0u : vmax(h0, F);
                   h2 = ONE_MAX ? pk_max3_bits(h0, F, E[r]) : vmax(h1, E[r]);
@@ -1896,6 +1945,16 @@
         }
       else return hipErrorInvalidValue;
     }
+  if (nq == 16)
+    {
+      if (!(P.tilt != 0 && P.max3 && !track && one)) return hipErrorInvalidValue;
+      if constexpr (VSX_ACGT_ROWS(R))
+        {
+          VSX_FWD_GO(ntasks, R, false, true, true, 1, false, true, true);
+          return hipGetLastError();
+        }
+      else return hipErrorInvalidValue;
+    }
   if (nq != 1)
     {
       if (!(P.tilt != 0 && !track && (nq == 2 || nq == 4))) return hipErrorInvalidValue;
diff --git a/vsearch_amd/csrc/vsx_host.cpp b/vsearch_amd/csrc/vsx_host.cpp
--- a/vsearch_amd/csrc/vsx_host.cpp
+++ b/vsearch_amd/csrc/vsx_host.cpp
@@ -1143,6 +1143,30 @@
       }
   };
   if (any_pair_cand) run_threads(nth, mark_pairs);
+  {
+    static const bool one_off = std::getenv("VSX_ONESTRIP") && std::strcmp(std::getenv("VSX_ONESTRIP"), "0") == 0;
+    auto acgt_cand = [&](const ProtoTask & pt) {
+      return !one_off && pt.nq == 1 && pt.tilt == 2 && VSX_ACGT_ROWS(pt.rows) && (int64_t) queries->len[pt.q] <= 16ll * pt.rows;
+    };
+    bool any = false;
+    for (const auto & v : part)
+      for (const ProtoTask & pt : v)
+        if (acgt_cand(pt)) { any = true; break; }
+    if (any)
+      {
+        const int rc = ensure_impure(targets);
+        if (rc != VSX_OK) return rc;
+        run_threads(nth, [&](int t) {
+          for (ProtoTask & pt : part[(size_t) t])
+            {
+              if (!acgt_cand(pt)) continue;
+              bool pure = true;
+              for (uint32_t sidx = 0; sidx < pt.n && pure; ++sidx) pure = !targets->impure[tidx[pt.pair[sidx]]];
+              if (pure) pt.nq = 16;
+            }
+        });
+      }
+  }
   std::vector<ProtoTask> protos;
   {
     size_t total = 0;
@@ -1486,7 +1510,7 @@
           VsxDevParams Pf = L.tilt ? ctx->Pt : ctx->P;
           Pf.max3 = (L.tilt == 2) ? 1 : 0;
           static const bool one_off = std::getenv("VSX_ONESTRIP") && std::strcmp(std::getenv("VSX_ONESTRIP"), "0") == 0;
-          HIPCHK(vsx_launch_forward(L.rows, L.track, L.nq, (L.multi || (one_off && L.nq != 8)) ? 0 : 1, Pf, pl->d_tasks.p + L.first, L.count,
+          HIPCHK(vsx_launch_forward(L.rows, L.track, L.nq, (L.multi || (one_off && L.nq != 8 && L.nq != 16)) ? 0 : 1, Pf, pl->d_tasks.p + L.first, L.count,
                                     pl->Q->codes(), pl->T->codes(), dir, pl->d_strip.p,
                                     pl->d_slot.p + (size_t) L.first * VSX_TASK_SLOTS, st));
         }
@@ -1560,6 +1584,7 @@
       {
         if (L.nq == 2 || L.nq == 4) info->tasks_sparse += L.count;
         if (L.nq == 8) info->tasks_pair += L.count;
+        if (L.nq == 16) info->tasks_acgt += L.count;
         info->waves += (L.nq == 2 || L.nq == 4) ? (L.count + (uint32_t) L.nq - 1) / (uint32_t) L.nq : L.count;
         if (L.tilt) info->tasks_tilted += L.count;
         if (L.tilt == 2) info->tasks_max3 += L.count;
diff --git a/vsearch_amd/csrc/vsx_internal.h b/vsearch_amd/csrc/vsx_internal.h
--- a/vsearch_amd/csrc/vsx_internal.h
+++ b/vsearch_amd/csrc/vsx_internal.h
@@ -15,6 +15,7 @@
 #define VSX_MID_MIN_ROWS 18
 #endif
 #define VSX_MID(R_, TILT_) ((TILT_) && (R_) >= VSX_MID_MIN_ROWS)
+#define VSX_ACGT_ROWS(R_) ((R_) == 10 || (R_) == 16 || (R_) == 20 || (R_) == 26)
 
 struct VsxDevParams {
   uint32_t match_pk;
```

Result: faster. 8317, median of 6 (+1.5%).
